# opensensor/thingino-accel

Hardware: AMD Instinct MI355X
Metric: images/sec yolov5s_int8 640x640 batch256 (higher is better)
Workload: dtype int8

## Files before the change

thingino-accel_amd/csrc/hip/conv_i8.hip:

```cpp
#include "conv_i8_common.hpp"

#ifndef I8M_ABL
#define I8M_ABL 0
#endif
template <int BPX, int BN, int STAGES, int KS = 1, int NW = 4>
__global__ __launch_bounds__(NW * 64) void conv_i8_mfma(const mhip_conv_i8_t p, const long total_pix, const int k64,
                                                         const int8_t *__restrict__ zeros, const unsigned noc,
                                                         const unsigned nblk, const int lg_inc, const unsigned kw_magic,
                                                         const fastdiv_t dhw, const fastdiv_t dow, const int bufmode,
                                                         const unsigned in_bytes) {
    ANAT_BEGIN();
    const bool POW2 = lg_inc >= 0;
    const bool masked = p.kh * p.kw <= 32;
    constexpr int SLICE = (BPX + BN) * BK;
    constexpr int STAGE = KS * SLICE;
    constexpr int NWN = BN == 128 ? 2 : 1;
    constexpr int NWM = NW / NWN;
    constexpr int WPX = BPX / NWM / 16;
    constexpr int WOC = BN / NWN / 16;
    constexpr int XROWS = BPX / NW;
    constexpr int XI = XROWS / 16;
    constexpr int LW = (BN / 16 + NW - 1) / NW;
    constexpr int L = XI + LW;
    static_assert(XI >= 1 && XROWS % 16 == 0, "every wave fetches whole 16-row pieces of the pixel tile");
// ... 1039 lines not shown
    if (v.patch) return conv_i8_launch_patch(p, k64, v.patch);
    const int bn = p->oc_pad % 128 == 0 ? 128 : (p->oc_pad % 64 == 0 ? 64 : 32);
    const bool b16 = v.persist && v.stages == 2 && bn16_ok(p);
    if (v.bpx == 256) {
        if (bn == 128) return launch_variant_t<256, 128>(p, total_pix, k64, v);
        if (bn == 64) return launch_variant_t<256, 64>(p, total_pix, k64, v);
        if (b16) return launch_variant_t<256, 16>(p, total_pix, k64, v);
        return launch_variant_t<256, 32>(p, total_pix, k64, v);
    }
    if (bn == 128) return launch_variant_t<128, 128>(p, total_pix, k64, v);
    if (bn == 64) return launch_variant_t<128, 64>(p, total_pix, k64, v);
    if (b16) return launch_variant_t<128, 16>(p, total_pix, k64, v);
    return launch_variant_t<128, 32>(p, total_pix, k64, v);
}

template <int BPX, int BN>
static int launch_pair_t(const mhip_conv_i8_t *a, const mhip_conv_i8_t *b, long total_pix, int k64, int lg, unsigned magic,
                         int wres) {
    if (a->nseg > 1) return -2;
    return launch_persist_t<BPX, BN, 2, true, false, true>(a, total_pix, k64, lg, magic, b, wres);
}
extern "C" int mhip_conv_i8_pair(const mhip_conv_i8_t *a, const mhip_conv_i8_t *b) {
    if (!a || !b || !tune().persist || tune().variant) return -2;
    if (a->in != b->in || a->in_stride != b->in_stride || a->frames != b->frames || a->in_h != b->in_h || a->in_w != b->in_w ||
        a->in_c != b->in_c || a->out_h != b->out_h || a->out_w != b->out_w || a->kh != b->kh || a->kw != b->kw ||
        a->stride_h != b->stride_h || a->stride_w != b->stride_w || a->pad_top != b->pad_top || a->pad_left != b->pad_left ||
        a->row_pad != b->row_pad || a->nseg != b->nseg || a->seg_up != b->seg_up || !a->lut || !b->lut || a->add || b->add ||
        a->out_nchw || b->out_nchw)
        return -2;
    for (int i = 0; i < a->nseg; i++)
        if (a->seg_in[i] != b->seg_in[i] || a->seg_c[i] != b->seg_c[i] || a->seg_stride[i] != b->seg_stride[i]) return -2;
    if ((a->in_c % 16) != 0 || mhip_conv_i8_small_c(a->in_c, a->kw, a->out_c) || mhip_conv_i8_small_c(b->in_c, b->kw, b->out_c))
        return -2;
    if (a->nseg > 1 && (!seg_valid(a) || !seg_valid(b))) return -2;
    if (!persist_eligible(a) || !persist_eligible(b)) return -2;
    const int bn = a->oc_pad % 128 == 0 ? 128 : (a->oc_pad % 64 == 0 ? 64 : 32);
    const int bnb = b->oc_pad % 128 == 0 ? 128 : (b->oc_pad % 64 == 0 ? 64 : 32);
    if (bn != bnb || !mhip_zero_page()) return -2;
    const long total_pix = (long)a->frames * a->out_h * a->out_w;
    const int k64 = (a->kh * a->row_pad + BK - 1) / BK * BK, nks = k64 / BK;
    if (total_pix <= 0 || total_pix > 0x7fffffffL) return -2;
    int lg = 0;
    while ((1 << lg) < a->in_c) lg++;
    const unsigned magic = ((65536u + (unsigned)a->kw - 1u) / (unsigned)a->kw);
    const variant_t dv = default_variant(a, nks);
    const int bpx = dv.bpx ? dv.bpx : 128, wres = dv.persist && dv.wres && (tune().wres & 2);
    const bool b16 = bn16_ok(a) && bn16_ok(b);
    if (bpx == 256) {
        if (bn == 128) return launch_pair_t<256, 128>(a, b, total_pix, k64, lg, magic, wres);
        if (bn == 64) return launch_pair_t<256, 64>(a, b, total_pix, k64, lg, magic, wres);
        if (b16) return launch_pair_t<256, 16>(a, b, total_pix, k64, lg, magic, wres);
        return launch_pair_t<256, 32>(a, b, total_pix, k64, lg, magic, wres);
    }
    if (bn == 128) return launch_pair_t<128, 128>(a, b, total_pix, k64, lg, magic, wres);
    if (bn == 64) return launch_pair_t<128, 64>(a, b, total_pix, k64, lg, magic, wres);
    if (b16) return launch_pair_t<128, 16>(a, b, total_pix, k64, lg, magic, wres);
    return launch_pair_t<128, 32>(a, b, total_pix, k64, lg, magic, wres);
}

extern "C" int mhip_conv_i8_seg_ok(const mhip_conv_i8_t *p) {
    return p && (p->in_c % 16) == 0 && !mhip_conv_i8_small_c(p->in_c, p->kw, p->out_c) && seg_valid(p) && persist_eligible(p);
}

extern "C" int mhip_conv_i8_variants(const mhip_conv_i8_t *p, int *codes, int max) {
    if (!p || (p->in_c % 16) != 0 || mhip_conv_i8_small_c(p->in_c, p->kw, p->out_c)) return 0;
    const int k64 = (p->kh * p->row_pad + BK - 1) / BK * BK, nks = k64 / BK;
    int n = 0;
    if (p->pre_w) {
        const int first = conv_i8_pre_tile_rows(p);
        for (int th : {first, 16, 8, 4})
            if (th && n < max && conv_i8_patch_ok(p, th, nullptr)) {
                const int code = th == 16 ? 10 : (th == 8 ? 9 : 11);
                bool seen = false;
                for (int i = 0; i < n; i++) seen |= codes[i] == code;
                if (!seen) codes[n++] = code;
            }
        return n;
    }
    if (p->post_w) {
        for (int th : {16, 8, 4})
            if (n < max && conv_i8_patch_ok(p, th, nullptr)) codes[n++] = th == 16 ? 10 : (th == 8 ? 9 : 11);
        return n;
    }
    if (p->nseg > 1) {
        const int bn = p->oc_pad % 128 == 0 ? 128 : (p->oc_pad % 64 == 0 ? 64 : 32);
        const variant_t dv = default_variant(p, nks);
        const int dflt = dv.persist && dv.wres ? (dv.bpx == 256 ? 15 : 14) : (dv.bpx == 256 ? 4 : 2);
        if (n < max) codes[n++] = dflt;
        if (n < max && dflt != 2) codes[n++] = 2;
        if (n < max && dflt != 4) codes[n++] = 4;
        if (n < max && dflt != 14 && LUTB + 2 * (size_t)128 * BK + (size_t)nks * bn * BK <= 80 * 1024) codes[n++] = 14;
        if (n < max && dflt != 15 && LUTB + 2 * (size_t)256 * BK + (size_t)nks * bn * BK <= 80 * 1024) codes[n++] = 15;
        return n;
    }
    const int dflt = variant_code(default_variant(p, nks));
    if (n < max) codes[n++] = dflt;
    for (int code = 1; code <= NVARIANTS; code++) {
        const variant_t v = variant_of(code);
        if (code == dflt) continue;
        if (v.patch && !conv_i8_patch_ok(p, v.patch, nullptr)) continue;
        if (v.persist && !persist_eligible(p)) continue;
        if (v.ks2 && ((nks & 1) || nks < 4 || p->oc_pad % 64 != 0)) continue;
        if (v.w8 && (p->oc_pad % 128 != 0 || nks < 3)) continue;
        if (v.persist < 0) continue;
        if (v.r128 && !r128_ok(p)) continue;
        if (v.rows && !conv_i8_rows_ok(p)) continue;
        if (v.wres) {
            const int bn = p->oc_pad % 128 == 0 ? 128 : (p->oc_pad % 64 == 0 ? 64 : 32);
            if (LUTB + 2 * (size_t)v.bpx * BK + (size_t)nks * bn * BK > 80 * 1024) continue;
        }
        if (!v.persist && v.stages == 3 && nks <= 2) continue;
        if (n < max) codes[n++] = code;
    }
    return n;
}

template <int BN>
static int launch_generic(const mhip_conv_i8_t *p, long total_pix, int k64) {
    dim3 grid((unsigned)((total_pix + BP - 1) / BP), (unsigned)(p->oc_pad / BN));
    hipLaunchKernelGGL((conv_i8_generic<BN>), grid, dim3(NTHREADS), 0, mhip_stream_native(), *p, total_pix, k64,
                       make_fastdiv((unsigned)(p->out_h * p->out_w)));
    return mhip_check(hipGetLastError(), "conv_i8_generic launch");
}

extern "C" int mhip_conv_i8(const mhip_conv_i8_t *p) {
    if (!p || !p->in || (!p->out && !(p->post_w && p->post_out)) || !p->w) return -1;
    if (p->out_pix_stride < 0 || p->out_ch_off < 0 || (p->out_nchw && (p->out_pix_stride || p->out_ch_off)) ||
        (p->out_pix_stride && p->out_pix_stride < p->out_ch_off + p->out_c))
        return -1;
    if (p->frames <= 0 || p->in_h <= 0 || p->in_w <= 0 || p->in_c <= 0 || p->out_h <= 0 || p->out_w <= 0 ||
        p->out_c <= 0 || p->kh <= 0 || p->kw <= 0 || p->stride_h < 0 || p->stride_w < 0)
        return -1;
    int row_pad, oc_pad;
    mhip_conv_i8_pack_geom(p->in_c, p->kw, p->out_c, &row_pad, &oc_pad, nullptr);
    if (row_pad != p->row_pad || oc_pad != p->oc_pad) return -1;
    if (p->add && (!p->safe || p->out_nchw || ((p->out_c | p->out_pix_stride | p->out_ch_off) & 15) || (p->in_c % 16) != 0 ||
                   mhip_conv_i8_small_c(p->in_c, p->kw, p->out_c) || p->nseg > 1))
        return -1;
    const long total_pix = (long)p->frames * p->out_h * p->out_w;
    const int k64 = (p->kh * p->row_pad + BK - 1) / BK * BK;
    if (total_pix <= 0 || total_pix > 0x7fffffffL || (total_pix + BP - 1) / BP * (oc_pad / 32) > 0x7fffffffL) return -1;
    if (p->in_planar) {
        if (p->in_planar > 4 || p->in_c != 4 || p->in_w < 4 || p->stride_h < 1 || p->stride_w < 1 || p->add || p->nseg > 1 ||
            !mhip_conv_i8_small_c(p->in_c, p->kw, p->out_c))
            return -2;
        return conv_i8_try_smallc(p, k64);
    }
    if (mhip_conv_i8_small_c(p->in_c, p->kw, p->out_c)) {
        if (p->stride_h >= 1 && p->stride_w >= 1) {
            int rc = conv_i8_try_rgb(p, k64);
            if (rc == -2) rc = conv_i8_try_smallc(p, k64);
            if (rc != -2) return rc;
        }
        if (p->add || p->nseg > 1) return -1;
        if (oc_pad % 64 == 0) return launch_generic<64>(p, total_pix, k64);
        return launch_generic<32>(p, total_pix, k64);
    }
    if (p->pre_w) {
        if (!mhip_zero_page() || !mhip_conv_i8_pre_ok(p)) return -1;
        int th = conv_i8_pre_tile_rows(p);
        const int code = p->variant ? p->variant : tune().variant;
        if (code >= 9 && code <= 11) {
            const int want = code == 10 ? 16 : (code == 9 ? 8 : 4);
            if (conv_i8_patch_ok(p, want, nullptr)) th = want;
        } else if (tune().small_batch && conv_i8_patch_ok(p, 4, nullptr) &&
                   ((long)p->frames * p->out_h * p->out_w + 255) / 256 * ((p->oc_pad + 127) / 128) < 256) {
            th = 4;
        }
        return conv_i8_launch_patch(p, k64, th);
    }
    if (p->post_w) {
        if (!mhip_zero_page() || (p->in_c % 16) != 0 || !mhip_conv_i8_post_ok(p)) return -1;
        int th = conv_i8_post_tile_rows(p);
        const int code = p->variant ? p->variant : tune().variant;
        if (code >= 9 && code <= 11) {
            const int want = code == 10 ? 16 : (code == 9 ? 8 : 4);
            if (conv_i8_patch_ok(p, want, nullptr)) th = want;
        } else if (tune().small_batch && conv_i8_patch_ok(p, 4, nullptr) &&
                   ((long)p->frames * p->out_h * p->out_w + 255) / 256 * ((p->oc_pad + 127) / 128) < tune().few_wgs) {
            th = 4;
        }
        return conv_i8_launch_patch(p, k64, th);
    }
    if ((p->in_c % 16) == 0) {
        if (!mhip_zero_page()) return -1;
        const int nks = k64 / BK;
        if (p->variant < 0 || p->variant > NVARIANTS) return -1;
        int code = p->variant;
        if (p->nseg > 1) {
            if (!seg_valid(p) || !persist_eligible(p)) return -1;
            if (!code && tune().variant) {
                int codes[NVARIANTS];
                const int n = mhip_conv_i8_variants(p, codes, NVARIANTS);
                for (int i = 0; i < n; i++)
                    if (codes[i] == tune().variant) code = codes[i];
            }
            variant_t v = variant_of(code == 4 || code == 14 || code == 15 ? code : 2);
            if (!code) {
                const variant_t dv = default_variant(p, nks);
                v.bpx = dv.bpx ? dv.bpx : 128;
                v.wres = dv.persist && dv.wres;
            }
            return launch_variant(p, total_pix, k64, v);
        }
        if (!code && tune().variant) {
            int codes[NVARIANTS];
            const int n = mhip_conv_i8_variants(p, codes, NVARIANTS);
            for (int i = 0; i < n; i++)
                if (codes[i] == tune().variant) code = codes[i];
        }
        return launch_variant(p, total_pix, k64, code ? variant_of(code) : default_variant(p, nks));
    }
    if (oc_pad % 64 == 0) return launch_generic<64>(p, total_pix, k64);
    return launch_generic<32>(p, total_pix, k64);
}
```

thingino-accel_amd/csrc/hip/conv_i8_common.hpp:

```cpp
#pragma once
#include <hip/hip_runtime.h>
#include <stdint.h>
#include <stdlib.h>
#include <string.h>
#include <type_traits>

#include "../mhip.h"

extern "C" hipStream_t mhip_stream_native(void);
extern "C" int mhip_check(hipError_t e, const char *what);
extern "C" const void *mhip_zero_page(void);

typedef int v4i __attribute__((ext_vector_type(4)));
typedef int v2i __attribute__((ext_vector_type(2)));

#ifdef ANATOMY
struct anat_rec_t {
    unsigned key, wg, hwid, xcc;
    unsigned long long t[4];
};
static __device__ anat_rec_t *g_anat_buf;
static __device__ unsigned g_anat_cap;
#define ANAT_SETTER(NAME)                                                                                                    \
    extern "C" int NAME(void *buf, unsigned cap) {                                                                          \
// ... 55 lines not shown
    r = r > 127 ? 127 : r;
    return r;
}

__device__ __forceinline__ int requant_safe(int acc, float cs, int lo, int hi) {
    const float scaled = (float)acc * cs;
    const float half = __int_as_float((__float_as_int(scaled) & (int)0x80000000) | 0x3f000000);
    const int r = (int)(scaled + half);
    int m;
    asm("v_med3_i32 %0, %1, %2, %3" : "=v"(m) : "v"(r), "v"(lo), "v"(hi));
    return m;
}
template <int NV>
__device__ __forceinline__ void wait_lds_values(int (&v)[NV]) {
    static_assert(NV == 4 || NV == 8 || NV == 16, "values per lane");
    if constexpr (NV == 16)
        asm volatile("s_waitcnt lgkmcnt(0)"
                     : "+v"(v[0]), "+v"(v[1]), "+v"(v[2]), "+v"(v[3]), "+v"(v[4]), "+v"(v[5]), "+v"(v[6]), "+v"(v[7]), "+v"(v[8]), "+v"(v[9]),
                       "+v"(v[10]), "+v"(v[11]), "+v"(v[12]), "+v"(v[13]), "+v"(v[14]), "+v"(v[15]));
    else if constexpr (NV == 8)
        asm volatile("s_waitcnt lgkmcnt(0)" : "+v"(v[0]), "+v"(v[1]), "+v"(v[2]), "+v"(v[3]), "+v"(v[4]), "+v"(v[5]), "+v"(v[6]), "+v"(v[7]));
    else
        asm volatile("s_waitcnt lgkmcnt(0)" : "+v"(v[0]), "+v"(v[1]), "+v"(v[2]), "+v"(v[3]));
}

__device__ __forceinline__ uint32_t pack4(int q0, int q1, int q2, int q3) {
    const uint32_t a = __builtin_amdgcn_perm((uint32_t)q1, (uint32_t)q0, 0x0c0c0400u);
    const uint32_t b = __builtin_amdgcn_perm((uint32_t)q3, (uint32_t)q2, 0x0c0c0400u);
    return (b << 16) | a;
}
__device__ __forceinline__ void lut4_at0(int q0, int q1, int q2, int q3, int &v0, int &v1, int &v2, int &v3) {
    asm volatile("ds_read_i8 %0, %4 offset:128\n\tds_read_i8 %1, %5 offset:128\n\t"
                 "ds_read_i8 %2, %6 offset:128\n\tds_read_i8 %3, %7 offset:128"
                 : "=&v"(v0), "=&v"(v1), "=&v"(v2), "=&v"(v3)
                 : "v"(q0), "v"(q1), "v"(q2), "v"(q3)
                 : "memory");
}
__device__ __forceinline__ void lds_base_must_be_zero(const void *dynamic_lds) {
    __builtin_amdgcn_s_setprio(3);
    unsigned a = (unsigned)(size_t)(const __attribute__((address_space(3))) void *)dynamic_lds;
    asm volatile("" : "+s"(a));
    if (a != 0u) __builtin_trap();
}
struct add_args_t {
    float s_conv, s_other, inv;
};
__device__ __forceinline__ int add_one(int v, uint32_t xword, int k, const add_args_t &g, int lo8, int hi8) {
    const int x = __builtin_amdgcn_sbfe((int)xword, 8 * k, 8);
    const float y = (float)v * g.s_conv + (float)x * g.s_other;
    const float t = y * g.inv;
    const int r = (int)(t + 0.5f);
    int m;
    asm("v_med3_i32 %0, %1, %2, %3" : "=v"(m) : "v"(r), "v"(lo8), "v"(hi8));
    return m;
}
__device__ __forceinline__ void lut4_fast(int q0, int q1, int q2, int q3, int &v0, int &v1, int &v2, int &v3) {
    asm volatile("ds_read_i8 %0, %4 offset:256\n\tds_read_i8 %1, %5 offset:256\n\t"
                 "ds_read_i8 %2, %6 offset:256\n\tds_read_i8 %3, %7 offset:256"
                 : "=&v"(v0), "=&v"(v1), "=&v"(v2), "=&v"(v3)
                 : "v"(q0), "v"(q1), "v"(q2), "v"(q3)
                 : "memory");
}
template <int NV>
__device__ __forceinline__ void requant_pack_pre(const int (&a)[NV], float cs, uint32_t (&pk)[NV / 4]) {
    const float cs2 = cs * 2.0f;
    const int klo = -256, khi = 255;
    int q[NV], v[NV];
#pragma unroll
    for (int i = 0; i < NV; i++) {
        const int k = (int)((float)a[i] * cs2);
        asm("v_med3_i32 %0, %1, %2, %3" : "=v"(q[i]) : "v"(k), "v"(klo), "v"(khi));
    }
#pragma unroll
    for (int g = 0; g < NV / 4; g++)
        asm volatile("ds_read_i8 %0, %4 offset:768\n\tds_read_i8 %1, %5 offset:768\n\t"
                     "ds_read_i8 %2, %6 offset:768\n\tds_read_i8 %3, %7 offset:768"
                     : "=&v"(v[4 * g]), "=&v"(v[4 * g + 1]), "=&v"(v[4 * g + 2]), "=&v"(v[4 * g + 3])
                     : "v"(q[4 * g]), "v"(q[4 * g + 1]), "v"(q[4 * g + 2]), "v"(q[4 * g + 3])
                     : "memory");
    wait_lds_values<NV>(v);
#pragma unroll
    for (int g = 0; g < NV / 4; g++) pk[g] = pack4(v[4 * g], v[4 * g + 1], v[4 * g + 2], v[4 * g + 3]);
}
template <int NV, bool HAS_LUT, bool SAFE, bool LUT0, bool ADD = false, bool FAST = false>
__device__ __forceinline__ void requant_pack(const int (&a)[NV], float cs, int lo, const uint8_t *lut128, uint32_t (&pk)[NV / 4],
                                             const uint32_t *xw = nullptr, const add_args_t *ga = nullptr) {
    int q[NV];
    const int hi = 127;
    if (FAST && HAS_LUT && LUT0 && SAFE) {
        const float cs2 = cs * 2.0f;
        const int klo = -256, khi = 255;
        int v[NV];
#pragma unroll
        for (int i = 0; i < NV; i++) {
            const int k = (int)((float)a[i] * cs2);
            asm("v_med3_i32 %0, %1, %2, %3" : "=v"(q[i]) : "v"(k), "v"(klo), "v"(khi));
        }
#pragma unroll
        for (int g = 0; g < NV / 4; g++)
            lut4_fast(q[4 * g], q[4 * g + 1], q[4 * g + 2], q[4 * g + 3], v[4 * g], v[4 * g + 1], v[4 * g + 2], v[4 * g + 3]);
        wait_lds_values<NV>(v);
        if (ADD) {
            const int lo8 = -128;
#pragma unroll
            for (int i = 0; i < NV; i++) v[i] = add_one(v[i], xw[i >> 2], i & 3, *ga, lo8, hi);
        }
#pragma unroll
        for (int g = 0; g < NV / 4; g++) pk[g] = pack4(v[4 * g], v[4 * g + 1], v[4 * g + 2], v[4 * g + 3]);
        return;
    }
#pragma unroll
    for (int i = 0; i < NV; i++) q[i] = SAFE ? requant_safe(a[i], cs, lo, hi) : requant<false>(a[i], cs, lo);
    if (HAS_LUT && LUT0) {
        int v[NV];
#pragma unroll
        for (int g = 0; g < NV / 4; g++)
            lut4_at0(q[4 * g], q[4 * g + 1], q[4 * g + 2], q[4 * g + 3], v[4 * g], v[4 * g + 1], v[4 * g + 2], v[4 * g + 3]);
        wait_lds_values<NV>(v);
        if (ADD) {
            const int lo8 = -128;
#pragma unroll
            for (int i = 0; i < NV; i++) v[i] = add_one(v[i], xw[i >> 2], i & 3, *ga, lo8, hi);
        }
#pragma unroll
        for (int g = 0; g < NV / 4; g++) pk[g] = pack4(v[4 * g], v[4 * g + 1], v[4 * g + 2], v[4 * g + 3]);
    } else {
        if (HAS_LUT) {
#pragma unroll
            for (int i = 0; i < NV; i++) q[i] = (int8_t)lut128[q[i]];
        }
        if (ADD) {
            const int lo8 = -128;
#pragma unroll
            for (int i = 0; i < NV; i++) q[i] = add_one(q[i], xw[i >> 2], i & 3, *ga, lo8, hi);
        }
#pragma unroll
        for (int g = 0; g < NV / 4; g++) pk[g] = pack4(q[4 * g], q[4 * g + 1], q[4 * g + 2], q[4 * g + 3]);
    }
}

struct fastdiv_t {
    unsigned m, s1, s2;
};
__device__ __forceinline__ unsigned fdiv(unsigned n, const fastdiv_t d) {
    const unsigned q = __umulhi(d.m, n);
    return (q + ((n - q) >> d.s1)) >> d.s2;
}
static fastdiv_t make_fastdiv(unsigned d) {
    fastdiv_t r;
    unsigned l = 0;
    while ((1ull << l) < d) l++;
    r.m = (unsigned)(((1ull << 32) * ((1ull << l) - d)) / d + 1);
    r.s1 = l < 1 ? l : 1;
    r.s2 = l > 0 ? l - 1 : 0;
    return r;
}

template <int N>
__device__ __forceinline__ void wait_vmcnt() {
    asm volatile("s_waitcnt vmcnt(%0)" ::"n"(N) : "memory");
}

__device__ __forceinline__ void glds16(const void *gsrc, void *lds_wave_base) {
    __builtin_amdgcn_global_load_lds((const __attribute__((address_space(1))) void *)gsrc,
                                     (__attribute__((address_space(3))) void *)lds_wave_base, 16, 0, 0);
}
// ... 98 lines not shown
            } else {
                const int rem = ncols - c * 16;
                int o = 0;
                if (rem & 8) { __builtin_memcpy(d, s, 8); o = 8; }
                if (rem & 4) { __builtin_memcpy(d + o, s + o, 4); o += 4; }
                if (rem & 2) { __builtin_memcpy(d + o, s + o, 2); o += 2; }
                if (rem & 1) d[o] = s[o];
            }
        }
    } else {
        for (int id = tid; id < BPX * BN; id += (int)blockDim.x) {
            const int c = id / BPX, row = id - c * BPX;
            const long off = rowoff[row];
            if (off < 0 || c >= ncols) continue;
            p.out[off + (size_t)(oc0 + c) * hw] = tile[row * ROW + c];
        }
    }
}

template <int BPX, int BN, int WPX, int WOC, bool LUT0 = false>
__device__ __forceinline__ void epilogue(const mhip_conv_i8_t &p, v4i (&acc)[WOC][WPX], int8_t *tile, const uint8_t *slut,
                                         const long *rowoff, int oc0, int pxw, int ocw, int hw) {
    const bool direct = !p.out_nchw && ((p.out_c | p.out_pix_stride | p.out_ch_off) & 15) == 0;
#define EPI(L, S, D) epilogue_t<BPX, BN, WPX, WOC, L, S, D, LUT0>(p, acc, tile, slut, rowoff, oc0, pxw, ocw, hw)
    if (direct) {
        if (p.lut) { if (p.safe) EPI(true, true, true); else EPI(true, false, true); }
        else { if (p.safe) EPI(false, true, true); else EPI(false, false, true); }
    } else {
        if (p.lut) { if (p.safe) EPI(true, true, false); else EPI(true, false, false); }
        else { if (p.safe) EPI(false, true, false); else EPI(false, false, false); }
    }
#undef EPI
}

template <int WPX, int WOC>
__device__ __forceinline__ void init_acc(const mhip_conv_i8_t &p, v4i (&acc)[WOC][WPX], int ocbase) {
    const int lane = threadIdx.x & 63;
#pragma unroll
    for (int s = 0; s < WOC; s++) {
        const v4i b = p.bias ? *(const v4i *)(p.bias + ocbase + s * 16 + (lane >> 4) * 4) : (v4i){0, 0, 0, 0};
#pragma unroll
        for (int t = 0; t < WPX; t++) acc[s][t] = b;
    }
}


struct tune_t {
    int init;
    int persist;
    int persist_stages;
    int persist_maxk;
    int persist_slots;
    int stages;
    int bpx;
    int variant;
    int bufmode;
    int small_batch;
    int rgb_direct;
    int wres;
    int few_wgs;
    int rows;
    int patch_ring;
    int patch_lds_kb;
};
const tune_t &conv_i8_tune_state();

extern "C" int mhip_conv_i8_small_c(int in_c, int kw, int out_c);

static inline long in_extent_bytes(const mhip_conv_i8_t *p) {
    return (long)(p->frames - 1) * (long)p->in_stride + (long)p->in_h * p->in_w * p->in_c;
}
static inline long persist_out_bytes(const mhip_conv_i8_t *p) {
    const long pstride = p->out_pix_stride ? p->out_pix_stride : p->out_c;
    return (long)(p->frames - 1) * (long)p->out_stride + (long)p->out_h * p->out_w * pstride;
}
static inline bool conv_i8_direct_rows(const mhip_conv_i8_t *p) {
    return !p->out_nchw && ((p->out_c | p->out_pix_stride | p->out_ch_off) & 15) == 0;
}

bool conv_i8_patch_ok(const mhip_conv_i8_t *p, int th, int *ring);
int conv_i8_launch_patch(const mhip_conv_i8_t *p, int k64, int th);
int conv_i8_pre_tile_rows(const mhip_conv_i8_t *p);
int conv_i8_post_tile_rows(const mhip_conv_i8_t *p);
bool conv_i8_rows_ok(const mhip_conv_i8_t *p);
int conv_i8_launch_rows(const mhip_conv_i8_t *p);
int conv_i8_try_rgb(const mhip_conv_i8_t *p, int k64);
int conv_i8_try_smallc(const mhip_conv_i8_t *p, int k64);
```

thingino-accel_amd/csrc/hip/conv_i8_patch.hip:

```cpp
#include "conv_i8_common.hpp"
#include <stdio.h>

#ifdef PATCH_STAMPS
__device__ unsigned long long patch_stamp_sums[8];
extern "C" int mhip_patch_stamps(unsigned long long *out, int reset) {
    if (out && hipMemcpyFromSymbol(out, HIP_SYMBOL(patch_stamp_sums), sizeof(patch_stamp_sums)) != hipSuccess) return -1;
    if (reset) {
        unsigned long long z[8] = {0};
        if (hipMemcpyToSymbol(HIP_SYMBOL(patch_stamp_sums), z, sizeof(z)) != hipSuccess) return -1;
    }
    return 0;
}
#define STAMP(t)                                                                          \
    do {                                                                                  \
        __builtin_amdgcn_sched_barrier(0);                                                \
        asm volatile("s_memtime %0\n\ts_waitcnt lgkmcnt(0)" : "=s"(t)::"memory");        \
        __builtin_amdgcn_sched_barrier(0);                                                \
    } while (0)
#else
#define STAMP(t) do { } while (0)
#endif
#define PT_TW 16
#define PT_NIMAX 10

template <int LO, int HI>
__device__ __forceinline__ void wait_vmcnt_tree(int n) {
    if constexpr (LO == HI) {
        wait_vmcnt<LO>();
    } else {
        constexpr int MID = (LO + HI + 1) / 2;
        if (n >= MID) wait_vmcnt_tree<MID, HI>(n);
        else wait_vmcnt_tree<LO, MID - 1>(n);
    }
}
template <int HI>
__device__ __forceinline__ void wait_vmcnt_upto(int n) {
    wait_vmcnt_tree<0, HI>(n > HI ? HI : n);
}
__device__ __forceinline__ void barrier_lds() {
    asm volatile("s_waitcnt lgkmcnt(0)\n\ts_barrier" ::: "memory");
}

template <int TH, int BN, bool HAS_LUT, bool PRE = false, bool POST = false>
__global__ __launch_bounds__(NTHREADS) void conv_i8_patch(const mhip_conv_i8_t p, const int k64, const int tiles_x,
                                                          const int tiles_y, const unsigned ntiles_all, const int PH,
                                                          const int PW, const int PWP, const int PWH, const int nblk,
                                                          const int8_t *__restrict__ zeros, const fastdiv_t dtx,
                                                          const fastdiv_t dty, const fastdiv_t dpwp, const unsigned out_bytes,
                                                          const int ring, const int xmap, const unsigned in_bytes) {
    ANAT_BEGIN();
    constexpr int WPX = TH / 4;
    constexpr int WOC = BN / 16;
    constexpr int NST = WPX;
    extern __shared__ __attribute__((aligned(16))) int8_t dynlds[];
    uint8_t *slut = (uint8_t *)dynlds;
    lds_base_must_be_zero(dynlds);
    const int nks = k64 / BK;
    constexpr int NPO = 2 * BN;
    constexpr int LB = LUTB + ((PRE || POST) ? 512 : 0);
    int *dutab = (int *)(dynlds + LB);
    int8_t *wl = dynlds + LB + ((nks * 16 + 255) & ~255);
    const int patch_bytes = nblk * 1024;
    int8_t *w1l = wl + nks * BN * BK;
    int8_t *pwl = w1l;
    const int *pbl = (const int *)(pwl + NPO * NPO);
    int8_t *patch0 = w1l + (PRE ? p.in_c * BK : 0) + (POST ? NPO * NPO + NPO * 4 : 0);
    int8_t *tpatch = patch0 + ring * patch_bytes;

    const int tid = threadIdx.x, lane = tid & 63;
    const int wv = __builtin_amdgcn_readfirstlane(tid >> 6);
    const int oc0 = blockIdx.y * BN;
    const int C = p.in_c, lgc = 31 - __builtin_clz((unsigned)C), cpp = C >> 4, lgcpp = lgc - 4;
    const int s = p.stride_w;
    const unsigned M = C >= 128 ? 6u : (C >= 64 ? 2u : 0u);

    v4i bias[WOC];
#pragma unroll
    for (int q = 0; q < WOC; q++) bias[q] = p.bias ? *(const v4i *)(p.bias + oc0 + q * 16 + (lane >> 4) * 4) : (v4i){0, 0, 0, 0};
    constexpr int W1MAX = 4;
    v4i pbias[PRE ? W1MAX : 1];
    if (PRE) {
#pragma unroll
        for (int q = 0; q < W1MAX; q++) pbias[q] = q < (C >> 4) ? *(const v4i *)(p.pre_bias + q * 16 + (lane >> 4) * 4) : (v4i){0, 0, 0, 0};
    }
    if (HAS_LUT) {
        if (p.lut2) { if (tid < 128) ((uint32_t *)slut)[tid] = ((const uint32_t *)p.lut2)[tid]; }
        else if (tid < 64) ((uint32_t *)slut)[tid] = ((const uint32_t *)p.lut)[tid];
    }
    if (PRE && tid >= 128) ((uint32_t *)slut)[tid] = ((const uint32_t *)p.pre_lut2)[tid - 128];
    if (POST) {
        if (tid >= 128) ((uint32_t *)slut)[tid] = ((const uint32_t *)p.post_lut2)[tid - 128];
        if (tid < NPO) ((int *)(pwl + NPO * NPO))[tid] = ((const int *)(p.post_w + NPO * NPO))[tid];
    }
    const int rowbytes = p.kw * C, kbytes = p.kh * rowbytes;
    for (int i = tid; i < nks * 4; i += NTHREADS) {
        const int kb = i * 16;
        int du = 0;
        if (kb < kbytes) {
            const int ky = kb / rowbytes, rem = kb - ky * rowbytes, kx = rem >> lgc, cc = (rem & (C - 1)) >> 4;
            const int dp = ky * PWP + (s == 2 ? (kx >> 1) + (kx & 1) * PWH : kx);
            du = dp * cpp + cc;
        }
        dutab[i] = du;
    }
    __syncthreads();
    {
        const int schunk = (lane & 3) ^ (((lane >> 4) & 1) << 1);
        for (int i = wv; i < nks * (BN / 16); i += 4) {
            const int ks = i / (BN / 16), g = i - ks * (BN / 16);
            glds16(p.w + (size_t)(oc0 + g * 16 + (lane >> 2)) * k64 + ks * BK + schunk * 16, wl + (ks * BN + g * 16) * BK);
        }
        if (PRE)
            for (int g = wv; g < C / 16; g += 4) glds16(p.pre_w + (size_t)(g * 16 + (lane >> 2)) * BK + schunk * 16, w1l + g * 16 * BK);
        if (POST)
            for (int i = wv; i < NPO * NPO / 1024; i += 4) glds16(p.post_w + i * 1024 + lane * 16, pwl + i * 1024);
    }
    int uoff[PT_NIMAX], upos[PT_NIMAX];
#pragma unroll
    for (int n = 0; n < PT_NIMAX; n++) {
        uoff[n] = 0;
        upos[n] = -1;
        if (n * 4 + wv < nblk) {
            const unsigned phys = (unsigned)((n * 4 + wv) * 64 + lane);
            const unsigned U = phys ^ ((phys >> 3) & M);
            const unsigned pp = U >> lgcpp, cc = U & (unsigned)(cpp - 1);
            const unsigned py = fdiv(pp, dpwp), col = pp - py * (unsigned)PWP;
            const int px = s == 2 ? ((int)col < PWH ? 2 * (int)col : 2 * ((int)col - PWH) + 1) : (int)col;
            if ((int)py < PH && px < PW) {
                uoff[n] = ((int)py * p.in_w + px) * C + (int)cc * 16;
                upos[n] = ((int)py << 16) | px;
            }
        }
    }
    const int npw = nblk > wv ? (nblk - wv + 3) >> 2 : 0;
    const unsigned xcd = blockIdx.x & 7u;
    const unsigned xstart = xmap ? (unsigned)(((unsigned long long)ntiles_all * xcd) >> 3) : 0u;
    const unsigned xend = xmap ? (unsigned)(((unsigned long long)ntiles_all * (xcd + 1u)) >> 3) : 0u;
    const unsigned ntiles = xmap ? (xend - xstart) * 8u + xcd : ntiles_all;
    auto tile_xy = [&](unsigned t, int &tx, int &ty, unsigned &f) {
        const unsigned j = xmap ? xstart + (t >> 3) : t, q = fdiv(j, dtx);
        tx = (int)(j - q * (unsigned)tiles_x);
        f = fdiv(q, dty);
        ty = (int)(q - f * (unsigned)tiles_y);
    };
    const __amdgpu_buffer_rsrc_t xrs = __builtin_amdgcn_make_buffer_rsrc((void *)p.in, 0, (int)in_bytes, 0x00020000);
    auto issue_patch = [&](unsigned t, int8_t *dst) {
#ifdef PATCH_ABL
        return;
#endif
        int tx, ty;
        unsigned f;
        tile_xy(t, tx, ty, f);
        const int iy0 = ty * TH * s - p.pad_top, ix0 = tx * PT_TW * s - p.pad_left;
        if (in_bytes != 0u && iy0 >= 0 && ix0 >= 0 && iy0 + PH <= p.in_h && ix0 + PW <= p.in_w) {
            const int sbase = (int)(f * (unsigned)p.in_stride) + (iy0 * p.in_w + ix0) * C;
#pragma unroll
            for (int n = 0; n < PT_NIMAX; n++)
                if (n * 4 + wv < nblk) blds16(xrs, uoff[n], sbase, dst + (n * 4 + wv) * 1024);
            return;
        }
        const int8_t *base = p.in + (size_t)f * p.in_stride + ((long)iy0 * p.in_w + ix0) * C;
#pragma unroll
        for (int n = 0; n < PT_NIMAX; n++)
            if (n * 4 + wv < nblk) {
                const int py = upos[n] >> 16, px = upos[n] & 0xffff;
                const bool ok = upos[n] >= 0 && (unsigned)(iy0 + py) < (unsigned)p.in_h && (unsigned)(ix0 + px) < (unsigned)p.in_w;
                glds16(ok ? base + uoff[n] : zeros, dst + (n * 4 + wv) * 1024);
            }
    };

    const __amdgpu_buffer_rsrc_t orsrc = __builtin_amdgcn_make_buffer_rsrc(POST ? p.post_out : p.out, 0, (int)out_bytes, 0x00020000);
    const bool has_add = p.add != nullptr;
    constexpr int RROW = WOC == 4 ? 1024 : 512;
    constexpr int NRI = WOC == 4 ? WPX : 2 * WPX;
    int8_t *rstage = patch0 + (ring + (PRE ? 1 : 0)) * patch_bytes + wv * (WPX * RROW);
    const int frow = lane & 15, fchunk = lane >> 4;
    const int chan = (lane >> 4) * (4 * WOC);
    const int NR = has_add || POST ? NRI : 0;
    const int ntail = POST ? (has_add ? NRI : 0) + WPX * (NPO / 64) : NST;
    const int ppstride = p.post_out_pix_stride ? p.post_out_pix_stride : NPO;
    auto issue_rows = [&](const int8_t *base, size_t fstride, int tx, int ty, unsigned f) {
#pragma unroll
        for (int u = 0; u < WPX; u++) {
            const int oy = ty * TH + wv * WPX + u, ox = tx * PT_TW + frow;
            const int8_t *src = oy < p.out_h && ox < p.out_w ? base + (size_t)f * fstride + ((size_t)(oy * p.out_w + ox) * BN + (size_t)chan) : zeros;
            if (WOC == 4) {
                glds16(src, rstage + u * RROW);
            } else {
                __builtin_amdgcn_global_load_lds((const __attribute__((address_space(1))) void *)src,
                                                 (__attribute__((address_space(3))) void *)(rstage + u * RROW), 4, 0, 0);
                __builtin_amdgcn_global_load_lds((const __attribute__((address_space(1))) void *)(src + 4),
                                                 (__attribute__((address_space(3))) void *)(rstage + u * RROW + 256), 4, 0, 0);
            }
        }
    };
    const int pstride = p.out_pix_stride ? p.out_pix_stride : p.out_c;
    const int lo = p.relu ? 0 : -128;
    const uint8_t *lut128 = slut + 128;
    int ubase[WPX];
#pragma unroll
    for (int u = 0; u < WPX; u++) ubase[u] = ((wv * WPX + u) * s * PWP + frow) * cpp;

    const unsigned G = gridDim.x;
    const int D = ring - 1;
    unsigned t = blockIdx.x;
    int yg0 = 0, yg1 = 0, yg2 = 0;
    {
        int issued = 0;
        for (int d = 0; d < D; d++)
            if (t + (unsigned)d * G < ntiles) {
                issue_patch(t + (unsigned)d * G, patch0 + d * patch_bytes);
                issued++;
            }
        yg0 = issued > 1 ? (issued - 1) * npw : 0;
        yg1 = issued > 2 ? (issued - 2) * npw : 0;
        yg2 = 0;
    }
#ifdef PATCH_STAMPS
    unsigned long long st0 = 0, st1 = 0, st2 = 0, st3 = 0, st4 = 0, sum_wait = 0, sum_issue = 0, sum_k = 0, sum_epi = 0, sum_tiles = 0;
#endif
    int cur = 0;
    int pn_last = 0;
    bool first = true;
    ANAT_NOW(1);
    for (; t < ntiles; t += G) {
        STAMP(st0);
        int tx, ty;
        unsigned f;
        tile_xy(t, tx, ty, f);
        int voffs[WPX];
        uint32_t xw[WPX][WOC];
#pragma unroll
        for (int u = 0; u < WPX; u++) {
            const int oy = ty * TH + wv * WPX + u, ox = tx * PT_TW + frow;
            const unsigned off = f * (unsigned)p.out_stride + (unsigned)(oy * p.out_w + ox) * (unsigned)pstride +
                                 (unsigned)(p.out_ch_off + oc0 + chan);
            const bool ok = oy < p.out_h && ox < p.out_w && oc0 + chan < p.out_c;
            voffs[u] = ok ? (int)off : -1;
#pragma unroll
            for (int q = 0; q < WOC; q++) xw[u][q] = 0;
        }
        if (POST) {
#pragma unroll
            for (int u = 0; u < WPX; u++) {
                const int oy = ty * TH + wv * WPX + u, ox = tx * PT_TW + frow;
                const unsigned off = f * (unsigned)p.post_out_stride + (unsigned)(oy * p.out_w + ox) * (unsigned)ppstride +
                                     (unsigned)(p.post_out_ch_off + (lane >> 4) * (NPO / 4));
                voffs[u] = oy < p.out_h && ox < p.out_w ? (int)off : -1;
            }
            if (has_add) issue_rows(p.add, p.out_stride, tx, ty, f);
            else issue_rows(p.post_in, p.post_in_stride, tx, ty, f);
        } else if (has_add) {
#pragma unroll
            for (int u = 0; u < WPX; u++) {
                const int8_t *src = voffs[u] >= 0 ? p.add + (unsigned)voffs[u] : zeros;
                if (WOC == 4) {
                    glds16(src, rstage + u * RROW);
                } else {
                    __builtin_amdgcn_global_load_lds((const __attribute__((address_space(1))) void *)src,
                                                     (__attribute__((address_space(3))) void *)(rstage + u * RROW), 4, 0, 0);
                    __builtin_amdgcn_global_load_lds((const __attribute__((address_space(1))) void *)(src + 4),
                                                     (__attribute__((address_space(3))) void *)(rstage + u * RROW + 256), 4, 0, 0);
                }
            }
        }
        if (D > 0) {
            wait_vmcnt_upto<63>(yg0 + NR);
            barrier_lds();
            STAMP(st1);
            const unsigned tn = t + (unsigned)D * G;
            int pn = 0;
            if (tn < ntiles) {
                int slot = cur + D;
                slot = slot >= ring ? slot - ring : slot;
                issue_patch(tn, patch0 + slot * patch_bytes);
                pn = npw;
            }
            const int after = NR + pn + ntail;
            yg0 = yg1 + after;
            yg1 = yg2 + after;
            yg2 = ntail;
            if (D == 1) yg0 = ntail;
            if (D == 2) yg1 = ntail;
            pn_last = pn;
        } else {
            if (!first) barrier_lds();
            issue_patch(t, patch0);
            wait_vmcnt<0>();
            barrier_lds();
        }
        first = false;
        STAMP(st2);
        const int8_t *patch = patch0 + cur * patch_bytes;
        if (PRE) {
            const int WOC1 = C >> 4;
            const int P = PH * PWP, nsub = (P + 15) >> 4;
            const int iy0 = ty * TH * s - p.pad_top, ix0 = tx * PT_TW * s - p.pad_left;
            for (int sub = wv; sub < nsub; sub += 4) {
                int pp = sub * 16 + frow;
                const bool live = pp < P;
                pp = live ? pp : P - 1;
                const unsigned Ur = (unsigned)(pp * cpp + (fchunk & (cpp - 1)));
                const v4i xb1 = *(const v4i *)(patch + ((Ur ^ ((Ur >> 3) & M)) << 4));
                const unsigned py = fdiv((unsigned)pp, dpwp), px = (unsigned)pp - py * (unsigned)PWP;
                const bool inimg = live && (int)py < PH && (int)px < PW && (unsigned)(iy0 + (int)py) < (unsigned)p.in_h &&
                                   (unsigned)(ix0 + (int)px) < (unsigned)p.in_w;
                uint32_t pk1[W1MAX];
                if (WOC1 == 4) {
                    int a1[16];
#pragma unroll
                    for (int q = 0; q < 4; q++) {
                        const v4i wa = *(const v4i *)(w1l + lds_off(q * 16 + frow, fchunk));
                        const v4i r = __builtin_amdgcn_mfma_i32_16x16x64_i8(wa, xb1, pbias[PRE ? q : 0], 0, 0, 0);
#pragma unroll
                        for (int e = 0; e < 4; e++) a1[q * 4 + e] = r[e];
                    }
                    uint32_t pk4[4];
                    requant_pack_pre<16>(a1, p.pre_cs, pk4);
#pragma unroll
                    for (int e = 0; e < 4; e++) pk1[e] = inimg ? pk4[e] : 0u;
                    const unsigned Uw = (unsigned)(pp * cpp + (lane >> 4));
                    if (live) *(v4i *)(tpatch + ((Uw ^ ((Uw >> 3) & M)) << 4)) = (v4i){(int)pk1[0], (int)pk1[1], (int)pk1[2], (int)pk1[3]};
                } else {
                    int a1[8];
#pragma unroll
                    for (int q = 0; q < 2; q++) {
                        const v4i wa = *(const v4i *)(w1l + lds_off(q * 16 + frow, fchunk));
                        const v4i r = __builtin_amdgcn_mfma_i32_16x16x64_i8(wa, xb1, pbias[PRE ? q : 0], 0, 0, 0);
#pragma unroll
                        for (int e = 0; e < 4; e++) a1[q * 4 + e] = r[e];
                    }
                    uint32_t pk2[2];
                    requant_pack_pre<8>(a1, p.pre_cs, pk2);
                    const int g4 = lane >> 4;
                    const unsigned Uw = (unsigned)(pp * cpp + (g4 >> 1));
                    if (live)
                        *(uint2 *)(tpatch + ((Uw ^ ((Uw >> 3) & M)) << 4) + (g4 & 1) * 8) = make_uint2(inimg ? pk2[0] : 0u, inimg ? pk2[1] : 0u);
                }
            }
            barrier_lds();
            patch = tpatch;
        }
        v4i acc[WOC][WPX];
        v4i xa[WPX], wa[WOC], xb[WPX], wb[WOC];
        auto load_frags = [&](int ks, int du, v4i (&xf)[WPX], v4i (&wf)[WOC]) {
#pragma unroll
            for (int u = 0; u < WPX; u++) {
                const unsigned U = (unsigned)(ubase[u] + du);
                xf[u] = *(const v4i *)(patch + ((U ^ ((U >> 3) & M)) << 4));
            }
            const int8_t *ws = wl + ks * BN * BK;
#pragma unroll
            for (int q = 0; q < WOC; q++) wf[q] = *(const v4i *)(ws + lds_off(q * 16 + frow, fchunk));
        };
        auto mfma_step = [&](const v4i (&xf)[WPX], const v4i (&wf)[WOC]) {
#pragma unroll
            for (int q = 0; q < WOC; q++)
#pragma unroll
                for (int u = 0; u < WPX; u++) acc[q][u] = __builtin_amdgcn_mfma_i32_16x16x64_i8(wf[q], xf[u], acc[q][u], 0, 0, 0);
        };
        const int last = nks - 1;
        auto clampk = [&](int k) { return k < last ? k : last; };
        load_frags(0, dutab[fchunk], xa, wa);
        load_frags(clampk(1), dutab[clampk(1) * 4 + fchunk], xb, wb);
        int du_n = dutab[clampk(2) * 4 + fchunk];
#pragma unroll
        for (int q = 0; q < WOC; q++)
#pragma unroll
            for (int u = 0; u < WPX; u++) acc[q][u] = __builtin_amdgcn_mfma_i32_16x16x64_i8(wa[q], xa[u], bias[q], 0, 0, 0);
        int ks = 1;
        for (; ks + 1 < nks; ks += 2) {
            load_frags(ks + 1, du_n, xa, wa);
            du_n = dutab[clampk(ks + 2) * 4 + fchunk];
            __builtin_amdgcn_sched_barrier(0);
            mfma_step(xb, wb);
            __builtin_amdgcn_sched_barrier(0);
            load_frags(clampk(ks + 2), du_n, xb, wb);
            du_n = dutab[clampk(ks + 3) * 4 + fchunk];
            __builtin_amdgcn_sched_barrier(0);
            mfma_step(xa, wa);
            __builtin_amdgcn_sched_barrier(0);
        }
        if (ks < nks) mfma_step(xb, wb);
        STAMP(st3);
        if (D > 0) cur = cur + 1 == ring ? 0 : cur + 1;
        if (has_add) {
            if (D > 0) wait_vmcnt_upto<15>(pn_last);
#pragma unroll
            for (int u = 0; u < WPX; u++) {
                if (WOC == 4) {
                    const v4i r = *(const v4i *)(rstage + u * RROW + lane * 16);
                    xw[u][0] = (uint32_t)r[0]; xw[u][1] = (uint32_t)r[1]; xw[u][WOC > 2 ? 2 : 0] = (uint32_t)r[2]; xw[u][WOC > 3 ? 3 : 0] = (uint32_t)r[3];
                } else {
                    xw[u][0] = *(const uint32_t *)(rstage + u * RROW + lane * 4);
                    xw[u][WOC > 1 ? 1 : 0] = *(const uint32_t *)(rstage + u * RROW + 256 + lane * 4);
                }
            }
        }
        uint32_t pku[POST ? WPX : 1][WOC];
        if (POST && has_add) {
#pragma unroll
            for (int u = 0; u < WPX; u++) {
                if constexpr (WOC == 4) asm volatile("s_waitcnt lgkmcnt(0)" : "+v"(xw[u][0]), "+v"(xw[u][1]), "+v"(xw[u][2]), "+v"(xw[u][3])::"memory");
                else asm volatile("s_waitcnt lgkmcnt(0)" : "+v"(xw[u][0]), "+v"(xw[u][1])::"memory");
            }
            issue_rows(p.post_in, p.post_in_stride, tx, ty, f);
        }
#pragma unroll
        for (int u = 0; u < WPX; u++) {
            uint32_t pk[WOC];
            int a[WOC * 4];
#pragma unroll
            for (int q = 0; q < WOC; q++)
#pragma unroll
                for (int r = 0; r < 4; r++) a[q * 4 + r] = acc[q][u][r];
            const bool fast = HAS_LUT && p.lut2 != nullptr;
            if (has_add) {
                const add_args_t ga = {p.add_s_conv, p.add_s_other, p.add_inv};
                if (fast) requant_pack<WOC * 4, HAS_LUT, true, true, true, true>(a, p.cs, lo, lut128, pk, xw[u], &ga);
                else requant_pack<WOC * 4, HAS_LUT, true, true, true>(a, p.cs, lo, lut128, pk, xw[u], &ga);
            } else {
                if (fast) requant_pack<WOC * 4, HAS_LUT, true, true, false, true>(a, p.cs, lo, lut128, pk);
                else requant_pack<WOC * 4, HAS_LUT, true, true>(a, p.cs, lo, lut128, pk);
            }
            if (POST) {
#pragma unroll
                for (int q = 0; q < WOC; q++) pku[POST ? u : 0][q] = pk[q];
                continue;
            }
            const int voff = voffs[u];
            if (WOC == 4)
                __builtin_amdgcn_raw_buffer_store_b128((v4i){(int)pk[0], (int)pk[1], (int)pk[2], (int)pk[3]}, orsrc, voff, 0, 0);
            else if (WOC == 2)
                __builtin_amdgcn_raw_buffer_store_b64((v2i){(int)pk[0], (int)pk[WOC > 1 ? 1 : 0]}, orsrc, voff, 0, 0);
        }
        if (POST) {
            if (has_add) wait_vmcnt<0>();
            else if (D > 0) wait_vmcnt_upto<15>(pn_last);
#pragma unroll
            for (int u = 0; u < WPX; u++) {
                v4i b0, b1 = {0, 0, 0, 0};
                if (WOC == 4) {
                    b0 = (v4i){(int)pku[POST ? u : 0][0], (int)pku[POST ? u : 0][1], (int)pku[POST ? u : 0][WOC > 2 ? 2 : 0], (int)pku[POST ? u : 0][WOC > 3 ? 3 : 0]};
                    b1 = *(const v4i *)(rstage + u * RROW + lane * 16);
                } else {
                    b0 = (v4i){(int)pku[POST ? u : 0][0], (int)pku[POST ? u : 0][WOC > 1 ? 1 : 0], *(const int *)(rstage + u * RROW + lane * 4),
                               *(const int *)(rstage + u * RROW + 256 + lane * 4)};
                }
#pragma unroll
                for (int h = 0; h < NPO / 64; h++) {
                    int a[16];
#pragma unroll
                    for (int s4 = 0; s4 < 4; s4++) {
                        const int row = (h * 4 + s4) * 16;
                        v4i c = *(const v4i *)(pbl + row + fchunk * 4);
                        c = __builtin_amdgcn_mfma_i32_16x16x64_i8(*(const v4i *)(pwl + lds_off(row + frow, fchunk)), b0, c, 0, 0, 0);
                        if (WOC == 4) c = __builtin_amdgcn_mfma_i32_16x16x64_i8(*(const v4i *)(pwl + NPO * BK + lds_off(row + frow, fchunk)), b1, c, 0, 0, 0);
#pragma unroll
                        for (int e = 0; e < 4; e++) a[s4 * 4 + e] = c[e];
                    }
                    uint32_t pk4[4];
                    requant_pack_pre<16>(a, p.post_cs, pk4);
                    const int voff = voffs[u] >= 0 ? voffs[u] + h * 16 : -1;
                    __builtin_amdgcn_raw_buffer_store_b128((v4i){(int)pk4[0], (int)pk4[1], (int)pk4[2], (int)pk4[3]}, orsrc, voff, 0, 0);
                }
            }
        }
#ifdef PATCH_STAMPS
        STAMP(st4);
        if (D == 0) st1 = st2;
        sum_wait += st1 - st0; sum_issue += st2 - st1; sum_k += st3 - st2; sum_epi += st4 - st3; sum_tiles += 1;
#endif
    }
    ANAT_NOW(2);
    ANAT_END(p);
#ifdef PATCH_STAMPS
    if (lane == 0) {
        atomicAdd(&patch_stamp_sums[0], sum_wait); atomicAdd(&patch_stamp_sums[1], sum_issue); atomicAdd(&patch_stamp_sums[2], sum_k);
        atomicAdd(&patch_stamp_sums[3], sum_epi); atomicAdd(&patch_stamp_sums[4], sum_tiles);
    }
#endif
}

ANAT_SETTER(mhip_anatomy_set_patch)
struct patch_geom_t {
    int bn, tiles_x, tiles_y, PH, PW, PWP, PWH, nblk, nks, ring;
    size_t lds;
};
static inline const tune_t &tune() { return conv_i8_tune_state(); }
static size_t patch_lds_budget(int bn) {
    const int kb = tune().patch_lds_kb;
    if (kb >= 16 && kb <= 160 && kb != 80) return (size_t)kb * 1024;
    return (size_t)(bn == 32 ? 53 : 80) * 1024;
}
static bool patch_geom(const mhip_conv_i8_t *p, int th, patch_geom_t *g) {
    const bool direct = conv_i8_direct_rows(p);
    const int C = p->in_c, s = p->stride_w;
    static const bool no_c16 = getenv("MARS_HIP_PATCH_NO_C16") != nullptr;
    if (!direct || !p->safe || (C != 16 && C != 32 && C != 64 && C != 128) || (C == 16 && (no_c16 || p->pre_w)) || (s != 1 && s != 2) || p->stride_h != s ||
        p->kh > 7 || p->kw > 7 || p->kh * p->kw < 2 || p->row_pad != p->kw * C || persist_out_bytes(p) > 0x7fffffffL)
        return false;
    const int k64 = (p->kh * p->row_pad + BK - 1) / BK * BK;
    g->nks = k64 / BK;
    g->bn = p->oc_pad % 64 == 0 ? 64 : 32;
    g->tiles_x = (p->out_w + PT_TW - 1) / PT_TW;
    g->tiles_y = (p->out_h + th - 1) / th;
    if ((double)p->out_h * p->out_w < (C == 128 ? 0.80 : 0.85) * (double)g->tiles_x * PT_TW * g->tiles_y * th) return false;
    g->PH = (th - 1) * s + p->kh;
    g->PW = (PT_TW - 1) * s + p->kw;
    g->PWH = s == 2 ? (g->PW + 1) / 2 : 0;
    g->PWP = s == 2 ? 2 * g->PWH : g->PW;
    const long units = (long)g->PH * g->PWP * (C / 16);
    g->nblk = (int)((units + 63) / 64);
    if (g->nblk > 4 * PT_NIMAX) return false;
    const bool pre = p->pre_w != nullptr;
    if (pre && (s != 1 || (C != 32 && C != 64) || !p->pre_bias || !p->pre_lut2 || !p->lut2)) return false;
    const bool post = p->post_w != nullptr;
    if (post) {
        const long ppstride = p->post_out_pix_stride ? p->post_out_pix_stride : 2 * g->bn;
        if (pre || s != 1 || p->out_c != g->bn || p->oc_pad != g->bn || p->out_pix_stride || p->out_ch_off || !p->lut2 || !p->post_lut2 || !p->post_in ||
            !p->post_out || ((p->post_out_pix_stride | p->post_out_ch_off) & 15) || p->post_out_pix_stride < 0 || p->post_out_ch_off < 0 ||
            ppstride < p->post_out_ch_off + 2 * g->bn ||
            (long)(p->frames - 1) * (long)p->post_out_stride + (long)p->out_h * p->out_w * ppstride > 0x7fffffffL)
            return false;
    }
    const size_t pb = (size_t)g->nblk * 1024;
    const size_t radd = p->add || post ? (size_t)4 * (th / 4) * (g->bn == 64 ? 1024 : 512) : 0;
    const size_t fixed = LUTB + (pre ? 512 + (size_t)C * BK + pb : 0) + (post ? 512 + (size_t)4 * g->bn * g->bn + (size_t)8 * g->bn : 0) +
                         (((size_t)g->nks * 16 + 255) & ~(size_t)255) + (size_t)g->nks * g->bn * BK + radd;
    const size_t budget = patch_lds_budget(g->bn);
    if (fixed + pb > budget) return false;
    const int fit = (int)((budget - fixed) / pb);
    const int cap = tune().patch_ring > 0 ? (tune().patch_ring > 4 ? 4 : tune().patch_ring) : 2;
    int ring = fit < cap ? fit : cap;
    g->ring = ring;
    g->lds = fixed + (size_t)ring * pb;
    if ((long)g->tiles_x * g->tiles_y * p->frames > 0x7fffffffL) return false;
    return true;
}

static inline long post_out_bytes(const mhip_conv_i8_t *p) {
    const long ppstride = p->post_out_pix_stride ? p->post_out_pix_stride : 2 * p->out_c;
    return (long)(p->frames - 1) * (long)p->post_out_stride + (long)p->out_h * p->out_w * ppstride;
}
template <int TH, int BN, bool HAS_LUT, bool PRE = false, bool POST = false>
static int launch_patch_t(const mhip_conv_i8_t *p, int k64, const patch_geom_t &g) {
    auto kern = conv_i8_patch<TH, BN, HAS_LUT, PRE, POST>;
    static int cus = 0;
    static size_t slots_lds[8];
    static int slots_n[8], nslots = 0;
    if (!cus) {
        int dev = 0;
        hipDeviceProp_t prop;
        if (hipFuncSetAttribute((const void *)kern, hipFuncAttributeMaxDynamicSharedMemorySize, 160 * 1024) != hipSuccess ||
            hipGetDevice(&dev) != hipSuccess || hipGetDeviceProperties(&prop, dev) != hipSuccess)
            return mhip_check(hipErrorUnknown, "conv_i8_patch occupancy query");
        cus = prop.multiProcessorCount;
    }
    int slots = 0;
    for (int i = 0; i < nslots; i++)
        if (slots_lds[i] == g.lds) slots = slots_n[i];
    if (!slots) {
        int occ = 0;
        if (hipOccupancyMaxActiveBlocksPerMultiprocessor(&occ, kern, NTHREADS, g.lds) != hipSuccess)
            return mhip_check(hipErrorUnknown, "conv_i8_patch occupancy query");
        slots = (occ > 0 ? occ : 1) * cus;
        if (nslots < 8) { slots_lds[nslots] = g.lds; slots_n[nslots++] = slots; }
    }
    const unsigned ntiles = (unsigned)((long)g.tiles_x * g.tiles_y * p->frames);
    const unsigned noc = (unsigned)(p->oc_pad / BN);
    unsigned gx = (unsigned)(tune().persist_slots > 0 ? tune().persist_slots : slots) / noc;
    if (gx < 1) gx = 1;
    if (gx > ntiles) gx = ntiles;
    const int xmap = gx >= 8 && ntiles < 0x0fffffffu;
    if (xmap) gx &= ~7u;
    {
        static const char *dbg = getenv("MARS_HIP_PATCH_DEBUG");
        static size_t last_lds = 0;
        static int last_ring = 0;
        if (dbg && (last_lds != g.lds || last_ring != g.ring)) {
            fprintf(stderr, "Mars: conv_i8_patch<%d,%d> ring %d, patch %d KB, LDS %zu B, %d workgroups per CU, grid %u x %u\n", TH, BN, g.ring,
                    g.nblk, g.lds, slots / cus, gx, noc);
            last_lds = g.lds;
            last_ring = g.ring;
        }
    }
    hipLaunchKernelGGL(kern, dim3(gx, noc), dim3(NTHREADS), g.lds, mhip_stream_native(), *p, k64,
                       g.tiles_x, g.tiles_y, ntiles, g.PH, g.PW, g.PWP, g.PWH, g.nblk, (const int8_t *)mhip_zero_page(),
                       make_fastdiv((unsigned)g.tiles_x), make_fastdiv((unsigned)g.tiles_y), make_fastdiv((unsigned)g.PWP),
                       (unsigned)(POST ? post_out_bytes(p) : persist_out_bytes(p)), g.ring, xmap,
                       in_extent_bytes(p) <= 0x7fffffffL ? (unsigned)in_extent_bytes(p) : 0u);
    return mhip_check(hipGetLastError(), "conv_i8_patch launch");
}

bool conv_i8_patch_ok(const mhip_conv_i8_t *p, int th, int *ring) {
    patch_geom_t g;
    if (!patch_geom(p, th, &g)) return false;
    if (ring) *ring = g.ring;
    return true;
}

int conv_i8_launch_patch(const mhip_conv_i8_t *p, int k64, int th) {
    patch_geom_t g;
    if (!patch_geom(p, th, &g)) return -1;
#define PATCH(T, B)                                                                       \
    (p->post_w ? launch_patch_t<T, B, true, false, true>(p, k64, g)                       \
     : p->pre_w ? launch_patch_t<T, B, true, true>(p, k64, g)                             \
                : (p->lut ? launch_patch_t<T, B, true>(p, k64, g) : launch_patch_t<T, B, false>(p, k64, g)))
    if (th == 16) return g.bn == 64 ? PATCH(16, 64) : PATCH(16, 32);
    if (th == 8) return g.bn == 64 ? PATCH(8, 64) : PATCH(8, 32);
    return g.bn == 64 ? PATCH(4, 64) : PATCH(4, 32);
#undef PATCH
}

int conv_i8_pre_tile_rows(const mhip_conv_i8_t *p) {
    patch_geom_t g;
    for (int th : {16, 8, 4})
        if (patch_geom(p, th, &g) && (th == 4 || g.ring >= 2)) return th;
    return 0;
}
extern "C" int mhip_conv_i8_pre_ok(const mhip_conv_i8_t *p) {
    if (!p || !p->pre_w || p->nseg > 1 || p->out_nchw) return 0;
    return conv_i8_pre_tile_rows(p) != 0;
}

int conv_i8_post_tile_rows(const mhip_conv_i8_t *p) {
    patch_geom_t g;
    for (int th : {16, 8, 4})
        if (patch_geom(p, th, &g)) return th;
    return 0;
}
extern "C" int mhip_conv_i8_post_ok(const mhip_conv_i8_t *p) {
    if (!p || !p->post_w || p->pre_w || p->nseg > 1 || p->out_nchw) return 0;
    return conv_i8_post_tile_rows(p) != 0;
}
extern "C" int mhip_conv_i8_post_k(int c, int k) {
    if (c == 64) return k;
    return k < 32 ? (k >> 3) * 16 + (k & 7) : ((k - 32) >> 3) * 16 + 8 + (k & 7);
}
extern "C" int mhip_conv_i8_post_row(int c, int oc) {
    const int per = c / 2, g = oc / per, rem = oc - g * per;
    return (rem >> 2) * 16 + g * 4 + (rem & 3);
}
extern "C" size_t mhip_conv_i8_post_pack(int c, const int8_t *packed, const int32_t *bias, int8_t *out) {
    if (c != 32 && c != 64) return 0;
    const int n = 2 * c;
    const size_t bytes = (size_t)n * n + (size_t)n * 4;
    if (!packed || !out) return bytes;
    memset(out, 0, bytes);
    for (int oc = 0; oc < n; oc++) {
        const int R = mhip_conv_i8_post_row(c, oc), src = mhip_conv_i8_oc_row(oc, n);
        for (int k = 0; k < n; k++) {
            const int pos = mhip_conv_i8_post_k(c, k), ks = pos >> 6, chunk = (pos & 63) >> 4;
            out[(size_t)(ks * n + R) * BK + (((chunk ^ ((R >> 1) & 2))) << 4) + (pos & 15)] = packed[(size_t)src * n + k];
        }
        ((int32_t *)(out + (size_t)n * n))[R] = bias ? bias[src] : 0;
    }
    return bytes;
}
```

thingino-accel_amd/csrc/host/mars_internal.h:

```cpp
#ifndef MARS_INTERNAL_H
#define MARS_INTERNAL_H

#include <stddef.h>
#include <stdint.h>

#include "../mhip.h"
#include "mars_hip.h"
#include "mars_runtime.h"

enum {
    OP_CONV_I8 = 0,
    OP_CONV_F32,
    OP_RELU_BYTES,
    OP_LUT_I8,
    OP_BINARY_I8,
    OP_SIGMOID_F32,
    OP_BINARY_F32,
    OP_RELU_F32,
    OP_BN,
    OP_MAXPOOL,
    OP_CONCAT_SLICE,
    OP_UPSAMPLE,
    OP_UPSAMPLE_Q, OP_MAXPOOL_Q,
    OP_CONCAT_Q,
    OP_CONV_F32_VHEAD,
    OP_FAIL,
};

#define NO_OFF ((size_t)-1)
#define MARS_MAX_IO 4
#define MARS_MAX_MODEL_TUNE 16

typedef struct {
    size_t bytes;
    size_t extent;
    size_t stride;
    uint8_t *dev;
    int is_weight;
    int needed;
    int io_in, io_out;
    uint8_t *host;
    uint8_t *dense_dev;
    int pix_c, pix_stride;
    int rec_c, rec_hw;
    int nhwc_c, nhwc_hw;
    size_t zero_from;
    int partial;
    int nhwc_pitch;
    int tail_read;
} mtensor_t;

typedef struct {
    int kind, layer, err;
    int t_in[4], n_in, t_out;
    int in_h, in_w, in_c, out_h, out_w, out_c, kh, kw, sh, sw, pt, pl;
    int nchw, relu, is_mul, is_f32, leaky, safe;
    size_t in_byte_off, out_byte_off;
    int k_limit;
    int vc_n, vc_t[3], vc_run, vc_shift;
    int rows_only;
    int out_nchw;
    int silu_f32;
    int f32_exact;
    int variant;
    int add_t; float add_s_conv, add_s_other, add_inv;
    int nseg, seg_t[4], seg_c[4], seg_up;
    int chain_n, chain_out[3];
    int pair_next;
    int row_pad, oc_pad, c_pad;
    int ch_off, scale_h, scale_w, bn_n;
    int out_pix_stride, out_ch_off;
    int store_c;
    float cs, f0, f1, f2;
    size_t n;
    size_t w_off, b_off, lut_off, s_off;
    int pre;
    size_t pre_w_off, pre_b_off, pre_lut2_off;
    float pre_cs;
    int post_next;
    size_t post_w_off;
    size_t w2_off;
    int w2_rows;
    int w2_planes;
    size_t w3_off;
    int w3_stem;
    int in_rec, out_rec;
    size_t lut2_off;
    size_t w_blob_off[2];
    double macs, bytes;
    int prof_kind;
    float last_ms;
    void *ev0, *ev1;
    int prof_rec;
    void *ev_start;
} mars_op_t;

typedef struct {
    int fusion;
    unsigned no_fuse_lut : 1, no_nhwc_internal : 1, no_vconcat_q : 1, no_pair_f32 : 1, no_rec : 1, no_zero_tail : 1, no_vconcat_f32 : 1,
        no_rowpad : 1, no_post : 1;
    size_t rec_limit;
    size_t vconcat_limit;
    size_t bottleneck_limit;
} plan_switches_t;

typedef struct mars_model_ext {
    mars_model_t pub;
    plan_switches_t sw;
    int batch, profiling, deferred;
    int plan_err;
    int no_vconcat;
    int no_download;
    int no_bottleneck;
    int no_post;
    int rec_frames;
    int rec_skipped;
    size_t rec_max_frames;
    mtensor_t *mt;
    mars_op_t *ops;
    int n_ops, cap_ops;
    uint8_t *arena_host;
    size_t arena_size, arena_cap;
    uint8_t *arena_dev;
    size_t blob_mirror_bytes;
    uint8_t *act_dev;
    size_t act_bytes;
    uint8_t *scratch_dev;
    size_t scratch_per_frame;
    int scratch_t, scratch_cpad, scratch_f0, scratch_n;
    void *det_dev;
    int *det_counts_dev;
    float *det_lut_dev;
    int det_cap;
    float det_lut_scale[4];
    int det_lut_n;
    int det_lut_mono[4];
    float *heads_lut_dev;
    float heads_lut_scale[4];
    int heads_lut_n;
    float *dfl_lut_dev;
    float dfl_lut_scale[4][2];
    int dfl_lut_n;
    void *ev_graph_done, *ev_tail_done;
    int tail_pending;
    int frame0, run_frames;
    void *ev_fork, *ev_join[3];
    void *ev_chunk[2][8];
    void *graph_exec;
    unsigned graph_gen;
    int ran_plain;
    void *pipe;
    struct { char key[28]; int value, saved; } tune[MARS_MAX_MODEL_TUNE];
    int n_tune, tune_depth;
    int plan_f32_mode;
    unsigned char *layer_noop;
    void *roi_dev;
    int roi_cap_slots, roi_cap_frames;
    int roi_slots;
    struct mars_model_ext *roi_from;
    void *cls_dev;
    size_t cls_bytes, cls_sums_off, cls_top_off;
    int cls_frames, cls_c, cls_top_k;
    void *ev_label_done;
    int label_pending;
    void *label_dev;
    int label_cap, label_frames;
    void *match_dev;
    size_t match_bytes, match_top_off, match_row_off;
    int match_frames, match_top_k;
    void *ident_dev;
    int ident_cap, ident_frames;
    void *track_dev;
    int track_cap, track_frames;
    void *seg_dev;
    size_t seg_bytes, seg_rec_off, seg_word_off;
    int seg_frames, seg_max, seg_ph, seg_pw;
    void *ev_seg[2];
    void *pose_dev;
    size_t pose_bytes, pose_rec_off, pose_kpt_off;
    int pose_frames, pose_max, pose_k;
    float pose_lut_scale[4];
    int pose_lut_n;
    void *ev_pose[2];
    void *obb_dev;
    size_t obb_bytes, obb_cnt_off, obb_out_off;
    int obb_frames;
    float obb_lut_scale[4];
    int obb_lut_n;
    void *ev_obb[2];
    struct mars_model_ext *live_next;
} mars_model_ext_t;


#define MARS_INTERNAL __attribute__((visibility("hidden")))
#define ALIGN_UP(x, a) (((x) + (size_t)(a) - 1) & ~((size_t)(a) - 1))
#define NO_TENSOR 0xFFFFFFFFu
#define MAX_DIM_PRODUCT ((size_t)1 << 40)
#define ARENA_MAX ((size_t)1 << 40)
#define MAX_CHANNELS 65536
MARS_INTERNAL int mars_verbose(void);
#define VLOG(...) do { if (mars_verbose()) fprintf(stderr, "Mars: " __VA_ARGS__); } while (0)
MARS_INTERNAL void drop_graph(mars_model_ext_t *m);
MARS_INTERNAL mars_model_ext_t *mars_live_models(void);
MARS_INTERNAL void plan_switches_read(plan_switches_t *sw, int at_load);
MARS_INTERNAL mars_error_t build_plan(mars_model_ext_t *m);
MARS_INTERNAL mars_error_t upload_params(mars_model_ext_t *m);
MARS_INTERNAL mars_error_t alloc_batch(mars_model_ext_t *m, int n);
MARS_INTERNAL size_t elem_size(uint32_t dtype);
MARS_INTERNAL size_t shape_numel(const mars_tensor_t *d);
MARS_INTERNAL size_t reference_buffer_size(const mars_model_ext_t *m);
MARS_INTERNAL size_t arena_reserve(mars_model_ext_t *m, size_t bytes);
MARS_INTERNAL void blob_read(const mars_model_ext_t *m, size_t off, size_t n, void *dst);
MARS_INTERNAL int op_reads(const mars_op_t *o, int t);
MARS_INTERNAL int op_writes(const mars_op_t *o, int t);
MARS_INTERNAL size_t planned_stride(const mtensor_t *t);
MARS_INTERNAL void conv_i8_geometry(const mars_op_t *op, int frames, mhip_conv_i8_t *p);
MARS_INTERNAL int conv_i8_pre_fits(const mars_op_t *op, int frames, size_t in_stride, size_t out_stride);
MARS_INTERNAL int conv_i8_post_fits(const mars_model_ext_t *m, const mars_op_t *a, const mars_op_t *b, int frames);
MARS_INTERNAL void plan_layer(mars_model_ext_t *m, int li);
MARS_INTERNAL void fold_silu(mars_model_ext_t *m, int f32);
MARS_INTERNAL void fuse_lut(mars_model_ext_t *m);
MARS_INTERNAL void nhwc_internal(mars_model_ext_t *m);
MARS_INTERNAL void fold_add(mars_model_ext_t *m, int f32);
MARS_INTERNAL void virtual_concat(mars_model_ext_t *m);
MARS_INTERNAL void elide_concat(mars_model_ext_t *m);
MARS_INTERNAL void trim_concat(mars_model_ext_t *m);
MARS_INTERNAL void fuse_pool_chains(mars_model_ext_t *m);
MARS_INTERNAL void pair_convs(mars_model_ext_t *m);
MARS_INTERNAL void fuse_bottleneck(mars_model_ext_t *m);
MARS_INTERNAL void fuse_post(mars_model_ext_t *m);
MARS_INTERNAL void pad_output_rows(mars_model_ext_t *m);
MARS_INTERNAL void virtual_concat_q(mars_model_ext_t *m);
MARS_INTERNAL void f32_policy(mars_model_ext_t *m);
MARS_INTERNAL void zero_tail_f32(mars_model_ext_t *m);
MARS_INTERNAL void pair_convs_f32(mars_model_ext_t *m);
MARS_INTERNAL void rec_pairs(mars_model_ext_t *m);
MARS_INTERNAL void virtual_concat_f32(mars_model_ext_t *m);
MARS_INTERNAL void plan_check(mars_model_ext_t *m);
MARS_INTERNAL void conv_i8_params(const mars_model_ext_t *m, const mars_op_t *op, mhip_conv_i8_t *p);
MARS_INTERNAL int mars_preproc_prepare(int w, int h, int tw, int th);
MARS_INTERNAL int mars_preproc_prepare_nv12(int w, int h, int tw, int th, int frames);

MARS_INTERNAL void mars_roi_release(mars_model_ext_t *m);

MARS_INTERNAL void mars_cls_release(mars_model_ext_t *m);

MARS_INTERNAL void mars_match_release(mars_model_ext_t *m);

MARS_INTERNAL void mars_track_release(mars_model_ext_t *m);

MARS_INTERNAL void mars_seg_release(mars_model_ext_t *m);

MARS_INTERNAL void mars_pose_release(mars_model_ext_t *m);

MARS_INTERNAL void mars_obb_release(mars_model_ext_t *m);

MARS_INTERNAL int mars_tensor_chw(const mars_tensor_t *d, int *c, int *h, int *w);
MARS_INTERNAL int mars_locate_i8(const mars_model_ext_t *m, int T, int ch, int hh, int ww, int any_writer, int *buf, int *off, int *pix_step, int *ch_step);
MARS_INTERNAL mars_error_t mars_own_det_buffers(mars_model_ext_t *m);
MARS_INTERNAL mars_error_t mars_tail_on_aux(mars_model_ext_t *m, int (*launch)(struct mars_model_ext *, const void *, void *, int *), const void *cfg);

mars_error_t mars_detect_prepare(mars_model_ext_t *m, const int *output_indices, int n_outputs);
int mars_detect_launch(mars_model_ext_t *m, const int *output_indices, int n_outputs, float nms_thresh, void *dets_dev,
                       int *counts_dev);

typedef struct {
    int n, ti[4], stride[4], nc[4], h[4], w[4], pix_step[4], ch_step[4];
    float anchors[4][3][2];
    float conf, nms;
    int map, px, py;
    float rx, ry;
    int internal;
} mars_heads_cfg_t;
MARS_INTERNAL int mars_find_heads(const mars_model_ext_t *m, int *tensor_ids, int *strides, int *num_classes, int cap);
MARS_INTERNAL mars_error_t mars_heads_resolve(mars_model_ext_t *m, const mars_yolo_heads_t *h, mars_heads_cfg_t *c);
MARS_INTERNAL mars_error_t mars_heads_prepare(mars_model_ext_t *m, const mars_heads_cfg_t *c);
MARS_INTERNAL int mars_heads_launch(mars_model_ext_t *m, const mars_heads_cfg_t *c, void *dets_dev, int *counts_dev);

typedef struct {
    int n, reg_max, stride[4], nc[4], h[4], w[4];
    int box_t[4], cls_t[4], box_buf[4], cls_buf[4], box_off[4], cls_off[4];
    int box_pix_step[4], box_ch_step[4], cls_pix_step[4], cls_ch_step[4];
    float box_scale[4], cls_scale[4];
    float conf, nms;
    int map, px, py;
    float rx, ry;
    int internal;
    int *cand_pred, *kept_pred;
    void *premap;
} mars_dfl_cfg_t;
MARS_INTERNAL int mars_find_dfl_heads(const mars_model_ext_t *m, int *box_ids, int *cls_ids, int *strides, int *num_classes, int *reg_max, int cap);
MARS_INTERNAL mars_error_t mars_dfl_resolve(mars_model_ext_t *m, const mars_yolo_dfl_heads_t *h, mars_dfl_cfg_t *c);
MARS_INTERNAL mars_error_t mars_dfl_prepare(mars_model_ext_t *m, const mars_dfl_cfg_t *c);
MARS_INTERNAL int mars_dfl_launch(mars_model_ext_t *m, const mars_dfl_cfg_t *c, void *dets_dev, int *counts_dev);

int32_t mars_trunc_x86(float x);
void mars_pack_conv_i8(const int8_t *w, size_t avail, int nchw, int out_c, int in_c, int kh, int kw,
                       int c_pad, int row_pad, int oc_pad, int8_t *dst);

#endif
```

thingino-accel_amd/csrc/host/mars_model.c:

```c
#include <math.h>
#include <stdio.h>
#include <stdlib.h>
#include <string.h>
#include <sys/types.h>
#include <time.h>

#include "mars_internal.h"
#include "nna.h"


int mars_verbose(void) {
    static int v = -1;
    if (v < 0) v = getenv("MARS_VERBOSE") ? 1 : 0;
    return v;
}

void plan_switches_read(plan_switches_t *sw, int at_load) {
    const char *e;
    if (at_load) sw->fusion = (e = getenv("MARS_HIP_FUSION")) ? atoi(e) : 1;
    sw->no_fuse_lut = getenv("MARS_HIP_NO_FUSE_LUT") != NULL;
    sw->no_nhwc_internal = getenv("MARS_HIP_NO_NHWC_INTERNAL") != NULL;
    sw->no_vconcat_q = getenv("MARS_HIP_NO_VCONCAT_Q") != NULL;
    sw->no_pair_f32 = getenv("MARS_HIP_NO_PAIR_F32") != NULL;
    sw->no_rec = getenv("MARS_HIP_NO_REC") != NULL;
    sw->no_zero_tail = getenv("MARS_HIP_NO_ZERO_TAIL") != NULL;
    sw->no_vconcat_f32 = getenv("MARS_HIP_NO_VCONCAT_F32") != NULL;
    sw->no_rowpad = getenv("MARS_HIP_NO_ROWPAD") != NULL;
    sw->no_post = getenv("MARS_HIP_NO_POST") != NULL;
    sw->rec_limit = (e = getenv("MARS_HIP_REC_LIMIT")) ? (size_t)strtoull(e, NULL, 0) : (size_t)0xfffffff0u;
    sw->vconcat_limit = (e = getenv("MARS_HIP_VCONCAT_LIMIT")) ? (size_t)strtoull(e, NULL, 0) : (size_t)0x7fffffffu;
    sw->bottleneck_limit = (e = getenv("MARS_HIP_BOTTLENECK_LIMIT")) ? (size_t)strtoull(e, NULL, 0) : 0;
}

void drop_graph(mars_model_ext_t *m) {
    if (m->graph_exec) {
        mhip_sync();
        mhip_graph_destroy(m->graph_exec);
    }
    m->graph_exec = NULL;
    m->ran_plain = 0;
}

static const char *const k_err[] = {
    "OK", "Invalid magic number", "Version mismatch", "Memory allocation failed",
    "Invalid file format", "NNA initialization failed", "Layer execution failed",
    "Invalid tensor", "Invalid layer",
};

const char *mars_get_error_string(mars_error_t err) {
    int i = -(int)err;
    if (i >= 0 && i < (int)(sizeof(k_err) / sizeof(k_err[0]))) return k_err[i];
    return "Unknown error";
}

static void free_device_state(mars_model_ext_t *m) {
    drop_graph(m);
    if (m->act_dev) mhip_free(m->act_dev);
    if (m->scratch_dev) mhip_free(m->scratch_dev);
    m->act_dev = m->scratch_dev = NULL;
    for (uint32_t i = 0; m->mt && i < m->pub.header.num_tensors; i++) {
        if (m->mt[i].host) mhip_host_free(m->mt[i].host);
        m->mt[i].host = NULL;
        if (m->mt[i].dense_dev) mhip_free(m->mt[i].dense_dev);
        m->mt[i].dense_dev = NULL;
        if (!m->mt[i].is_weight) m->mt[i].dev = NULL;
    }
    if (m->det_dev) mhip_free(m->det_dev);
    if (m->det_counts_dev) mhip_free(m->det_counts_dev);
    m->det_dev = NULL;
    m->det_counts_dev = NULL;
    m->det_cap = 0;
    m->tail_pending = 0;
    mars_roi_release(m);
    mars_cls_release(m);
    mars_track_release(m);
    mars_seg_release(m);
    mars_pose_release(m);
    mars_obb_release(m);
}

static void free_ops(mars_model_ext_t *m) {
    drop_graph(m);
    for (int i = 0; i < m->n_ops; i++) {
        if (m->ops[i].ev0) mhip_event_destroy(m->ops[i].ev0);
        if (m->ops[i].ev1) mhip_event_destroy(m->ops[i].ev1);
    }
    free(m->ops);
    m->ops = NULL;
    m->n_ops = m->cap_ops = 0;
}

static mars_model_ext_t *g_live_models = NULL;
mars_model_ext_t *mars_live_models(void) { return g_live_models; }

void mars_free(mars_model_t *model) {
    if (!model) return;
    mars_model_ext_t *m = (mars_model_ext_t *)model;
    for (mars_model_ext_t **pp = &g_live_models; *pp; pp = &(*pp)->live_next)
        if (*pp == m) { *pp = m->live_next; break; }
    for (mars_model_ext_t *x = g_live_models; x; x = x->live_next)
        if (x->roi_from == m) x->roi_from = NULL;
    if (m->pipe) mars_hip_pipe_close(model);
    if (mhip_ready()) mhip_sync();
    free_device_state(m);
    free_ops(m);
    if (m->arena_dev) mhip_free(m->arena_dev);
    if (m->det_lut_dev) mhip_free(m->det_lut_dev);
    if (m->heads_lut_dev) mhip_free(m->heads_lut_dev);
    if (m->dfl_lut_dev) mhip_free(m->dfl_lut_dev);
    if (m->ev_graph_done) mhip_event_destroy(m->ev_graph_done);
    if (m->ev_tail_done) mhip_event_destroy(m->ev_tail_done);
    if (m->ev_label_done) mhip_event_destroy(m->ev_label_done);
    if (m->ev_fork) mhip_event_destroy(m->ev_fork);
    for (int k = 0; k < 3; k++)
        if (m->ev_join[k]) mhip_event_destroy(m->ev_join[k]);
    for (int k = 0; k < 2; k++)
        for (int c = 0; c < 8; c++)
            if (m->ev_chunk[k][c]) mhip_event_destroy(m->ev_chunk[k][c]);
    free(m->arena_host);
    free(m->layer_noop);
    free(m->mt);
    free(m->pub.weights);
    free(m->pub.layers);
    free(m->pub.tensors);
    free(m);
}

mars_error_t build_plan(mars_model_ext_t *m) {
    const uint32_t nt = m->pub.header.num_tensors, nl = m->pub.header.num_layers;
    plan_switches_read(&m->sw, 0);
    free_ops(m);
    m->arena_size = 0;
    if (m->arena_host) memset(m->arena_host, 0, m->arena_cap);
    m->scratch_per_frame = 0;
    m->plan_err = MARS_OK;
    m->plan_f32_mode = mhip_conv_f32_mode(-1);
    m->blob_mirror_bytes = m->pub.weights_size;
    for (uint32_t i = 0; i < nt; i++) {
        m->mt[i].extent = m->mt[i].bytes;
        m->mt[i].pix_c = m->mt[i].pix_stride = 0;
        m->mt[i].needed = (m->mt[i].io_in || m->mt[i].io_out) ? 1 : 0;
    }
    for (uint32_t i = 0; i < nl && m->plan_err == MARS_OK; i++) {
        const int n0 = m->n_ops;
        plan_layer(m, (int)i);
        m->layer_noop[i] = m->n_ops == n0;
    }
    if (m->plan_err != MARS_OK) return (mars_error_t)m->plan_err;
    if (m->sw.fusion >= 1) {
        fold_silu(m, 0);
        fuse_lut(m);
        fold_silu(m, 1);
        nhwc_internal(m);
        fold_add(m, 0);
        fold_add(m, 1);
        if (!m->no_vconcat) virtual_concat(m);
        elide_concat(m);
        trim_concat(m);
        fuse_pool_chains(m);
        pair_convs(m);
        if (m->sw.fusion >= 2 && !m->no_bottleneck) fuse_bottleneck(m);
        fuse_post(m);
        pad_output_rows(m);
        virtual_concat_q(m);
    } else {
        nhwc_internal(m);
    }
    f32_policy(m);
    zero_tail_f32(m);
    if (m->sw.fusion >= 1) pair_convs_f32(m);
    rec_pairs(m);
    virtual_concat_f32(m);
    if (m->plan_err == MARS_OK) plan_check(m);
    return (mars_error_t)m->plan_err;
}

mars_error_t upload_params(mars_model_ext_t *m) {
    size_t mirror_off = arena_reserve(m, m->blob_mirror_bytes + 64);
    if (mirror_off == NO_OFF) return MARS_ERR_ALLOC_FAILED;
    if (!m->deferred) blob_read(m, 0, m->blob_mirror_bytes, m->arena_host + mirror_off);
    if (m->arena_dev) mhip_free(m->arena_dev);
    m->arena_dev = (uint8_t *)mhip_malloc(m->arena_size);
    if (!m->arena_dev) return MARS_ERR_ALLOC_FAILED;
    if (mhip_h2d_async(m->arena_dev, m->arena_host, m->arena_size) || mhip_sync()) return MARS_ERR_NNA_INIT_FAILED;
    for (uint32_t i = 0; i < m->pub.header.num_tensors; i++) {
        if (!m->mt[i].is_weight) continue;
        m->mt[i].dev = m->arena_dev + mirror_off + (size_t)m->pub.tensors[i].desc.data_offset;
        m->mt[i].stride = 0;
        m->pub.tensors[i].paddr = m->mt[i].dev;
    }
    m->pub.ddr_paddr = m->arena_dev;
    m->pub.ddr_size = m->arena_size;
    return MARS_OK;
}

mars_error_t alloc_batch(mars_model_ext_t *m, int n) {
    const uint32_t nt = m->pub.header.num_tensors;
    if (m->pipe) mars_hip_pipe_close(&m->pub);
    if (mhip_sync()) return MARS_ERR_LAYER_FAILED;
    plan_switches_read(&m->sw, 0);
    const size_t vlim = m->sw.vconcat_limit, blim = m->sw.bottleneck_limit;
    const int rec_replan = (size_t)n > m->rec_max_frames || (m->rec_skipped && n < m->rec_frames);
    m->rec_frames = n;
    if (m->no_vconcat || m->no_bottleneck || m->no_post || rec_replan) {
        m->no_vconcat = m->no_bottleneck = m->no_post = 0;
        mars_error_t e = build_plan(m);
        if (e == MARS_OK) e = upload_params(m);
        if (e != MARS_OK) return e;
    }
    if (!m->no_vconcat)
        for (int i = 0; i < m->n_ops; i++) {
            const mars_op_t *op = &m->ops[i];
            if (op->kind != OP_CONV_I8 || op->nseg < 2 || op->t_out < 0) continue;
            if (planned_stride(&m->mt[op->t_out]) * (size_t)n > vlim) {
                m->no_vconcat = 1;
                mars_error_t e = build_plan(m);
                if (e == MARS_OK) e = upload_params(m);
                if (e != MARS_OK) return e;
                break;
            }
        }
    if (m->sw.fusion >= 2 && !m->no_bottleneck)
        for (int i = 0; i < m->n_ops; i++) {
            const mars_op_t *op = &m->ops[i];
            if (op->kind != OP_CONV_I8 || !op->pre || op->t_out < 0) continue;
            const size_t in_stride = op->t_in[0] >= 0 ? planned_stride(&m->mt[op->t_in[0]]) : 0;
            if (!conv_i8_pre_fits(op, n, in_stride, planned_stride(&m->mt[op->t_out])) || (blim && (size_t)n > blim)) {
                m->no_bottleneck = 1;
                mars_error_t e = build_plan(m);
                if (e == MARS_OK) e = upload_params(m);
                if (e != MARS_OK) return e;
                break;
            }
        }
    if (!m->no_post)
        for (int i = 0; i + 1 < m->n_ops; i++) {
            const mars_op_t *op = &m->ops[i];
            if (op->kind != OP_CONV_I8 || !op->post_next) continue;
            if (!conv_i8_post_fits(m, op, op + 1, n)) {
                m->no_post = 1;
                mars_error_t e = build_plan(m);
                if (e == MARS_OK) e = upload_params(m);
                if (e != MARS_OK) return e;
                break;
            }
        }
    free_device_state(m);
    size_t per_frame = 0;
    for (uint32_t i = 0; i < nt; i++) {
        mtensor_t *t = &m->mt[i];
        if (t->is_weight || !t->needed) continue;
        t->stride = planned_stride(t);
        per_frame += t->stride;
    }
    m->act_bytes = per_frame * (size_t)n;
    m->act_dev = (uint8_t *)mhip_malloc(m->act_bytes + 512);
    if (!m->act_dev) return MARS_ERR_ALLOC_FAILED;
    if (mhip_memset_async(m->act_dev, 0, m->act_bytes + 256)) return MARS_ERR_ALLOC_FAILED;
    size_t off = 256;
    for (uint32_t i = 0; i < nt; i++) {
        mtensor_t *t = &m->mt[i];
        mars_runtime_tensor_t *rt = &m->pub.tensors[i];
        if (t->is_weight) continue;
        rt->vaddr = NULL; rt->paddr = NULL; rt->alloc_size = 0;
        if (!t->needed) continue;
        t->dev = m->act_dev + off;
        off += t->stride * (size_t)n;
        rt->paddr = t->dev;
        rt->alloc_size = t->stride * (size_t)n;
        if (t->io_in || t->io_out) {
            const size_t hb = t->bytes * (size_t)n, ref = reference_buffer_size(m);
            size_t cap = hb > ref ? hb : ref;
            if (ref > ((size_t)8 << 20)) cap = hb;
            t->host = (uint8_t *)mhip_host_alloc(cap ? cap : 64);
            if (!t->host) return MARS_ERR_ALLOC_FAILED;
            memset(t->host, 0, cap);
            rt->vaddr = t->host;
            rt->alloc_size = n == 1 && cap >= ref ? ref : hb;
        }
        if (t->pix_stride) {
            t->dense_dev = (uint8_t *)mhip_malloc(t->bytes * (size_t)n);
            if (!t->dense_dev) return MARS_ERR_ALLOC_FAILED;
        }
    }
    if (m->scratch_per_frame) {
        m->scratch_dev = (uint8_t *)mhip_malloc(ALIGN_UP(m->scratch_per_frame, 256) * (size_t)n + 256);
        if (!m->scratch_dev) return MARS_ERR_ALLOC_FAILED;
    }
    m->batch = n;
    m->frame0 = 0;
    m->run_frames = n;
    return mhip_sync() ? MARS_ERR_ALLOC_FAILED : MARS_OK;
}

static mars_error_t load_host(const void *data, size_t size, unsigned flags, mars_model_ext_t **out_m) {
    if (!data || !out_m || size < sizeof(mars_header_t)) return MARS_ERR_INVALID_FILE;
    const uint8_t *p = (const uint8_t *)data;
    mars_header_t h;
    memcpy(&h, p, sizeof(h));
    if (h.magic != MARS_MAGIC) {
        VLOG("Invalid magic 0x%08x (expected 0x%08x)\n", h.magic, MARS_MAGIC);
        return MARS_ERR_INVALID_MAGIC;
    }
    if (h.version_major != MARS_VERSION_MAJOR) return MARS_ERR_VERSION_MISMATCH;
    if (h.num_tensors > 65536 || h.num_layers > 65536 || h.num_inputs > 4 || h.num_outputs > 4) return MARS_ERR_INVALID_FILE;
    const size_t tables = sizeof(h) + (size_t)h.num_tensors * sizeof(mars_tensor_t) + (size_t)h.num_layers * sizeof(mars_layer_t);
    if (tables > size) return MARS_ERR_INVALID_FILE;
    const int deferred = (flags & MARS_HIP_LOAD_DEFER_WEIGHTS) != 0;
    if (!deferred && h.weights_size > 0 && (h.weights_offset > size || h.weights_size > size - h.weights_offset))
        return MARS_ERR_INVALID_FILE;
    if (h.weights_size > ((uint64_t)1 << 36)) return MARS_ERR_INVALID_FILE;

    mars_model_ext_t *m = (mars_model_ext_t *)calloc(1, sizeof(*m));
    if (!m) return MARS_ERR_ALLOC_FAILED;
    m->pub.header = h;
    plan_switches_read(&m->sw, 1);
    m->deferred = deferred;
    m->pub.tensors = (mars_runtime_tensor_t *)calloc(h.num_tensors ? h.num_tensors : 1, sizeof(mars_runtime_tensor_t));
    m->pub.layers = (mars_runtime_layer_t *)calloc(h.num_layers ? h.num_layers : 1, sizeof(mars_runtime_layer_t));
    m->mt = (mtensor_t *)calloc(h.num_tensors ? h.num_tensors : 1, sizeof(mtensor_t));
    m->layer_noop = (unsigned char *)calloc(h.num_layers ? h.num_layers : 1, 1);
    if (!m->pub.tensors || !m->pub.layers || !m->mt || !m->layer_noop) { mars_free(&m->pub); return MARS_ERR_ALLOC_FAILED; }
    const uint8_t *q = p + sizeof(h);
    for (uint32_t i = 0; i < h.num_tensors; i++, q += sizeof(mars_tensor_t)) memcpy(&m->pub.tensors[i].desc, q, sizeof(mars_tensor_t));
    for (uint32_t i = 0; i < h.num_layers; i++, q += sizeof(mars_layer_t)) memcpy(&m->pub.layers[i].desc, q, sizeof(mars_layer_t));

    m->pub.weights_size = (size_t)h.weights_size;
    if (h.weights_size) {
        m->pub.weights = calloc(1, (size_t)h.weights_size);
        if (!m->pub.weights) { mars_free(&m->pub); return MARS_ERR_ALLOC_FAILED; }
        if (!deferred) memcpy(m->pub.weights, p + h.weights_offset, (size_t)h.weights_size);
    }
    m->pub.ddr_base = m->pub.weights;
    for (uint32_t i = 0; i < h.num_tensors; i++) {
        mars_runtime_tensor_t *rt = &m->pub.tensors[i];
        if (rt->desc.ndims > MARS_MAX_DIMS) { mars_free(&m->pub); return MARS_ERR_INVALID_FILE; }
        m->mt[i].bytes = shape_numel(&rt->desc) * elem_size(rt->desc.dtype);
        if (rt->desc.data_size > 0) {
            if (rt->desc.data_offset > h.weights_size) { mars_free(&m->pub); return MARS_ERR_INVALID_FILE; }
            m->mt[i].is_weight = 1;
            rt->vaddr = (uint8_t *)m->pub.weights + rt->desc.data_offset;
            rt->alloc_size = (size_t)rt->desc.data_size;
        }
    }
    for (uint32_t i = 0; i < h.num_inputs; i++) {
        uint32_t id = h.input_tensor_ids[i];
        if (id < h.num_tensors && !m->mt[id].is_weight) m->mt[id].io_in = (int)i + 1;
    }
    for (uint32_t i = 0; i < h.num_outputs; i++) {
        uint32_t id = h.output_tensor_ids[i];
        if (id < h.num_tensors && !m->mt[id].is_weight) m->mt[id].io_out = (int)i + 1;
    }

    mars_error_t err = build_plan(m);
    if (err != MARS_OK) { mars_free(&m->pub); return err; }
    VLOG("%u layers -> %d launches, parameter arena %zu bytes\n", h.num_layers, m->n_ops, m->arena_size);
    *out_m = m;
    return MARS_OK;
}

mars_error_t mars_hip_load_memory_ex(const void *data, size_t size, unsigned flags, mars_model_t **out_model) {
    if (!out_model) return MARS_ERR_INVALID_FILE;
    mars_model_ext_t *m = NULL;
    mars_error_t err = load_host(data, size, flags, &m);
    if (err != MARS_OK) return err;
    if (!nna_is_ready() || !mhip_ready()) {
        fprintf(stderr, "Mars: no initialised MI355X device (call nna_init first); refusing to load\n");
        mars_free(&m->pub);
        return MARS_ERR_NNA_INIT_FAILED;
    }
    err = upload_params(m);
    if (err == MARS_OK) err = alloc_batch(m, 1);
    if (err != MARS_OK) { mars_free(&m->pub); return err; }
    m->live_next = g_live_models;
    g_live_models = m;
    *out_model = &m->pub;
    return MARS_OK;
}

static int describe_op_full(const mars_op_t *o, char *line, size_t cap, int k) {
#define ADD(...) k += snprintf(line + k, cap - (size_t)k, __VA_ARGS__)
    ADD(" | err %d in %dx%dx%d out %dx%dx%d k %dx%d s %dx%d p %d,%d", o->err, o->in_h, o->in_w, o->in_c, o->out_h, o->out_w, o->out_c, o->kh, o->kw, o->sh, o->sw, o->pt, o->pl);
    ADD(" nchw %d out_nchw %d relu %d is_mul %d is_f32 %d leaky %d safe %d silu %d f32_exact %d variant %d", o->nchw, o->out_nchw, o->relu, o->is_mul, o->is_f32, o->leaky,
        o->safe, o->silu_f32, o->f32_exact, o->variant);
    ADD(" row_pad %d oc_pad %d c_pad %d store_c %d ch_off %d out_ch_off %d out_pix_stride %d in_byte_off %zu out_byte_off %zu scale %dx%d bn_n %d n %zu", o->row_pad,
        o->oc_pad, o->c_pad, o->store_c, o->ch_off, o->out_ch_off, o->out_pix_stride, o->in_byte_off, o->out_byte_off, o->scale_h, o->scale_w, o->bn_n, o->n);
    ADD(" k_limit %d rows_only %d pair_next %d in_rec %d out_rec %d vc %d,%d,%d:", o->k_limit, o->rows_only, o->pair_next, o->in_rec, o->out_rec, o->vc_n, o->vc_run, o->vc_shift);
    for (int q = 0; q < o->vc_n && q < 3; q++) ADD(" %d", o->vc_t[q]);
    ADD(" add %d %a %a %a seg %d up %d:", o->add_t, (double)o->add_s_conv, (double)o->add_s_other, (double)o->add_inv, o->nseg, o->seg_up);
    for (int q = 0; q < o->nseg && q < 4; q++) ADD(" %d/%d", o->seg_t[q], o->seg_c[q]);
    ADD(" chain %d:", o->chain_n);
    for (int q = 0; q < o->chain_n && q < 3; q++) ADD(" %d", o->chain_out[q]);
    ADD(" cs %a f %a %a %a", (double)o->cs, (double)o->f0, (double)o->f1, (double)o->f2);
    ADD(" w_off %zd b_off %zd lut_off %zd lut2_off %zd s_off %zd w2_off %zd rows %d planes %d w3_off %zd stem %d blob %zd %zd", (ssize_t)o->w_off, (ssize_t)o->b_off,
        (ssize_t)o->lut_off, (ssize_t)o->lut2_off, (ssize_t)o->s_off, (ssize_t)o->w2_off, o->w2_rows, o->w2_planes, (ssize_t)o->w3_off, o->w3_stem, (ssize_t)o->w_blob_off[0],
        (ssize_t)o->w_blob_off[1]);
    ADD(" post_next %d", o->post_next);
    if (o->post_next) ADD(" %zd", (ssize_t)o->post_w_off);
    ADD(" pre %d", o->pre);
    if (o->pre) ADD(" %zd %zd %zd %a", (ssize_t)o->pre_w_off, (ssize_t)o->pre_b_off, (ssize_t)o->pre_lut2_off, (double)o->pre_cs);
    ADD(" macs %a bytes %a prof_kind %d", o->macs, o->bytes, o->prof_kind);
#undef ADD
    return k;
}

size_t mars_hip_describe_plan(const void *data, size_t size, unsigned flags, char *out, size_t cap) {
    static const char *const kinds[] = {"conv_i8", "conv_f32", "relu_bytes", "lut_i8", "binary_i8", "sigmoid_f32", "binary_f32", "relu_f32", "bn",
                                        "maxpool", "concat_slice", "upsample", "upsample_q", "maxpool_q", "concat_q", "conv_f32_vhead", "fail"};
    mars_model_ext_t *m = NULL;
    const int full = (flags & MARS_HIP_DESCRIBE_FULL) != 0;
    if (load_host(data, size, flags & ~MARS_HIP_DESCRIBE_FULL, &m) != MARS_OK) return 0;
    size_t n = 0;
    char line[4096];
#define EMIT() do { const size_t l = strlen(line); if (out && n < cap) memcpy(out + n, line, n + l <= cap ? l : cap - n); n += l; } while (0)
    for (int i = 0; i < m->n_ops; i++) {
        const mars_op_t *o = &m->ops[i];
        int k = snprintf(line, sizeof line, "op %d layer %d %s in", i, o->layer, o->kind >= 0 && o->kind <= OP_FAIL ? kinds[o->kind] : "?");
        for (int q = 0; q < o->n_in && q < 4; q++) k += snprintf(line + k, sizeof line - (size_t)k, " %d", o->t_in[q]);
        k += snprintf(line + k, sizeof line - (size_t)k, " out %d", o->t_out);
#define FLAG(cond, ...) if (cond) k += snprintf(line + k, sizeof line - (size_t)k, __VA_ARGS__)
        FLAG(o->kind == OP_CONV_I8 || o->kind == OP_CONV_F32 || o->kind == OP_CONV_F32_VHEAD, " k%dx%d s%d c%d->%d", o->kh, o->kw, o->sw, o->in_c, o->out_c);
        FLAG(o->nchw, " relayout"); FLAG(o->out_nchw, " planar_store"); FLAG(o->lut_off != NO_OFF, " lut"); FLAG(o->add_t, " add=%d", o->add_t - 1);
        FLAG(o->nseg, " seg=%d", o->nseg); FLAG(o->pair_next, " pair_next"); FLAG(o->post_next, " post_next"); FLAG(o->pre, " pre"); FLAG(o->silu_f32, " silu");
        FLAG(o->k_limit, " k_limit=%d", o->k_limit); FLAG(o->in_rec, " in_rec=%d", o->in_rec); FLAG(o->out_rec, " out_rec");
        FLAG(o->vc_shift, " view=-%d", o->vc_shift); FLAG(o->vc_n, " vcat=%dx%d", o->vc_n, o->vc_run);
        FLAG(o->rows_only, " rows_only=%d", o->rows_only); FLAG(o->out_byte_off, " out_off=%zu", o->out_byte_off); FLAG(o->chain_n, " chain=%d", o->chain_n);
        FLAG(o->out_pix_stride, " pix_stride=%d", o->out_pix_stride); FLAG(o->kind == OP_FAIL, " err=%d", o->err);
#undef FLAG
        if (full) k = describe_op_full(o, line, sizeof line, k);
        snprintf(line + k, sizeof line - (size_t)k, "\n");
        EMIT();
    }
    for (uint32_t t = 0; t < m->pub.header.num_tensors; t++) {
        const mtensor_t *mt = &m->mt[t];
        const int listed = mt->nhwc_c || mt->partial || mt->zero_from || mt->rec_c || mt->pix_stride;
        if (!listed && !(full && mt->needed)) continue;
        int k = listed ? snprintf(line, sizeof line, "tensor %u nhwc_c %d pitch %d partial %d zero_from %zu rec_c %d pix_stride %d", t, mt->nhwc_c, mt->nhwc_pitch,
                                  mt->partial, mt->zero_from, mt->rec_c, mt->pix_stride)
                       : snprintf(line, sizeof line, "+tensor %u", t);
        if (full)
            k += snprintf(line + k, sizeof line - (size_t)k, " | bytes %zu extent %zu needed %d tail_read %d weight %d io %d,%d pix_c %d rec_hw %d nhwc_hw %d", mt->bytes,
                          mt->extent, mt->needed, mt->tail_read, mt->is_weight, mt->io_in, mt->io_out, mt->pix_c, mt->rec_hw, mt->nhwc_hw);
        snprintf(line + k, sizeof line - (size_t)k, "\n");
        EMIT();
    }
    if (full) {
        const plan_switches_t *w = &m->sw;
        snprintf(line, sizeof line, "+plan n_ops %d arena_size %zu scratch_per_frame %zu blob_mirror_bytes %zu rec_max_frames %zu rec_skipped %d f32_mode %d | fusion %d"
                 " no_fuse_lut %d no_nhwc_internal %d no_vconcat_q %d no_pair_f32 %d no_rec %d no_zero_tail %d no_vconcat_f32 %d no_rowpad %d no_post %d rec_limit %zu"
                 " vconcat_limit %zu bottleneck_limit %zu\n", m->n_ops, m->arena_size, m->scratch_per_frame, m->blob_mirror_bytes, m->rec_max_frames, m->rec_skipped,
                 m->plan_f32_mode, w->fusion, w->no_fuse_lut, w->no_nhwc_internal, w->no_vconcat_q, w->no_pair_f32, w->no_rec, w->no_zero_tail, w->no_vconcat_f32,
                 w->no_rowpad, w->no_post, w->rec_limit, w->vconcat_limit, w->bottleneck_limit);
        EMIT();
    }
#undef EMIT
    if (out && cap) out[n < cap ? n : cap - 1] = 0;
    mars_free(&m->pub);
    return n;
}

int mars_yolo_find_heads(const void *data, size_t size, int *tensor_ids, int *strides, int *num_classes, int cap) {
    mars_model_ext_t *m = NULL;
    if (load_host(data, size, 0, &m) != MARS_OK) return -1;
    const int n = mars_find_heads(m, tensor_ids, strides, num_classes, cap);
    mars_free(&m->pub);
    return n;
}

int mars_yolo_find_dfl_heads(const void *data, size_t size, int *box_ids, int *cls_ids, int *strides, int *num_classes, int *reg_max, int cap) {
    mars_model_ext_t *m = NULL;
    if (load_host(data, size, 0, &m) != MARS_OK) return -1;
    const int n = mars_find_dfl_heads(m, box_ids, cls_ids, strides, num_classes, reg_max, cap);
    mars_free(&m->pub);
    return n;
}

mars_error_t mars_load_memory(const void *data, size_t size, mars_model_t **model) {
    return mars_hip_load_memory_ex(data, size, 0, model);
}

mars_error_t mars_load_file(const char *path, mars_model_t **model) {
    if (!path || !model) return MARS_ERR_INVALID_FILE;
    FILE *fp = fopen(path, "rb");
    if (!fp) {
        fprintf(stderr, "Mars: Cannot open %s\n", path);
        return MARS_ERR_INVALID_FILE;
    }
    fseek(fp, 0, SEEK_END);
    long size = ftell(fp);
    fseek(fp, 0, SEEK_SET);
    if (size <= 0) { fclose(fp); return MARS_ERR_INVALID_FILE; }
    void *buf = malloc((size_t)size);
    if (!buf) { fclose(fp); return MARS_ERR_ALLOC_FAILED; }
    if (fread(buf, 1, (size_t)size, fp) != (size_t)size) { free(buf); fclose(fp); return MARS_ERR_INVALID_FILE; }
    fclose(fp);
    mars_error_t err = mars_load_memory(buf, (size_t)size, model);
    free(buf);
    return err;
}

mars_runtime_tensor_t *mars_get_input(mars_model_t *model, int index) {
    if (!model || index < 0 || (uint32_t)index >= model->header.num_inputs) return NULL;
    uint32_t tid = model->header.input_tensor_ids[index];
    if (tid >= model->header.num_tensors) return NULL;
    return &model->tensors[tid];
}

mars_runtime_tensor_t *mars_get_output(mars_model_t *model, int index) {
    if (!model || index < 0 || (uint32_t)index >= model->header.num_outputs) return NULL;
    uint32_t tid = model->header.output_tensor_ids[index];
    if (tid >= model->header.num_tensors) return NULL;
    return &model->tensors[tid];
}

int mars_get_num_inputs(mars_model_t *model) { return model ? (int)model->header.num_inputs : 0; }
int mars_get_num_outputs(mars_model_t *model) { return model ? (int)model->header.num_outputs : 0; }

void mars_print_summary(mars_model_t *model) {
    if (!model) return;
    mars_model_ext_t *m = (mars_model_ext_t *)model;
    printf("\nMars model summary (MI355X)\n");
    printf("Layers: %u\n", model->header.num_layers);
    printf("Tensors: %u\n", model->header.num_tensors);
    printf("Inputs: %u\n", model->header.num_inputs);
    printf("Outputs: %u\n", model->header.num_outputs);
    printf("Weights: %zu bytes\n", model->weights_size);
    printf("Launches per run: %d, batch %d, activations %zu bytes, parameters %zu bytes\n\n", m->n_ops, m->batch,
           m->act_bytes, m->arena_size);
}
```

thingino-accel_amd/csrc/host/mars_plan.c:

```c
#include <math.h>
#include <stdio.h>
#include <stdlib.h>
#include <string.h>
#include <time.h>

#include "mars_internal.h"
#include "nna.h"

int32_t mars_trunc_x86(float x) {
    if (x >= -2147483648.0f && x < 2147483648.0f) return (int32_t)x;
    return INT32_MIN;
}
static int sat8(int32_t v) { return v > 127 ? 127 : (v < -128 ? -128 : v); }
static int q_half_up(float v) { return sat8(mars_trunc_x86(v + 0.5f)); }

size_t elem_size(uint32_t dtype) {
    switch (dtype) {
        case MARS_DTYPE_FLOAT32: case MARS_DTYPE_INT32: return 4;
        case MARS_DTYPE_INT16: return 2;
        default: return 1;
    }
}

size_t shape_numel(const mars_tensor_t *d) {
// ... 524 lines not shown
    for (int i = 0; i < m->n_ops; i++) {
        const mars_op_t *o = &m->ops[i];
        for (int k = 0; k < o->n_in; k++)
            if (o->t_in[k] >= 0) c[o->t_in[k]]++;
        if (o->t_out >= 0) c[nt + (size_t)o->t_out]++;
        for (int k = 0; k < o->chain_n; k++)
            if (o->chain_out[k] >= 0 && o->chain_out[k] != o->t_out) c[nt + (size_t)o->chain_out[k]]++;
    }
    *readers = c;
    *writers = c + nt;
    return 1;
}

static int writer_before(const mars_model_ext_t *m, int t, int before) {
    for (int k = before - 1; k >= 0; k--)
        if (m->ops[k].t_out == t) return k;
    return -1;
}

enum { USE_READ = 1, USE_WRITE = 2 };
static int touched_between(const mars_model_ext_t *m, int lo, int hi, int t, int how) {
    for (int k = lo < 0 ? 0 : lo; k < hi && k < m->n_ops; k++)
        if (((how & USE_READ) && op_reads(&m->ops[k], t)) || ((how & USE_WRITE) && op_writes(&m->ops[k], t))) return 1;
    return 0;
}
static int touched_by_other(const mars_model_ext_t *m, int t, int lo, int hi) {
    return touched_between(m, 0, lo, t, USE_READ | USE_WRITE) || touched_between(m, hi + 1, m->n_ops, t, USE_READ | USE_WRITE);
}

static void drop_dead_ops(mars_model_ext_t *m) {
    int w = 0;
    for (int i = 0; i < m->n_ops; i++)
        if (m->ops[i].kind != -1) m->ops[w++] = m->ops[i];
    m->n_ops = w;
}

size_t planned_stride(const mtensor_t *t) {
    size_t s = ALIGN_UP(t->extent > t->bytes ? t->extent : t->bytes, 256);
    return s ? s : 256;
}

static void lut2_from_lut(mars_model_ext_t *m, mars_op_t *c, const int8_t *tab) {
    if (!mhip_conv_i8_lut2_ok(c->cs)) return;
    int8_t tab2[512];
    for (int k = -256; k < 256; k++) {
        int r = k >= 0 ? (k + 1) >> 1 : -((1 - k) >> 1);
        const int lo = c->relu ? 0 : -128;
        r = r < lo ? lo : (r > 127 ? 127 : r);
        tab2[k + 256] = tab[r + 128];
    }
    c->lut2_off = arena_reserve(m, 512);
    if (c->lut2_off != NO_OFF) memcpy(m->arena_host + c->lut2_off, tab2, 512);
}

void conv_i8_geometry(const mars_op_t *op, int frames, mhip_conv_i8_t *p) {
    memset(p, 0, sizeof(*p));
    p->frames = frames;
    p->in_c = op->in_c; p->in_h = op->in_h; p->in_w = op->in_w;
    p->out_h = op->out_h; p->out_w = op->out_w; p->out_c = op->store_c ? op->store_c : op->out_c;
    p->kh = op->kh; p->kw = op->kw; p->stride_h = op->sh; p->stride_w = op->sw; p->pad_top = op->pt; p->pad_left = op->pl;
    p->row_pad = op->row_pad; p->oc_pad = op->oc_pad; p->safe = op->safe;
    p->out_pix_stride = op->out_pix_stride; p->out_ch_off = op->out_ch_off;
}
int conv_i8_pre_fits(const mars_op_t *op, int frames, size_t in_stride, size_t out_stride) {
    mhip_conv_i8_t p;
    conv_i8_geometry(op, frames, &p);
    p.in_stride = in_stride; p.out_stride = out_stride;
    p.pre_w = (const int8_t *)op; p.pre_bias = (const int32_t *)op; p.pre_lut2 = (const uint8_t *)op; p.lut2 = (const uint8_t *)op;
    p.lut = (const uint8_t *)op;
    return mhip_conv_i8_pre_ok(&p);
}

int conv_i8_post_fits(const mars_model_ext_t *m, const mars_op_t *a, const mars_op_t *b, int frames) {
    mhip_conv_i8_t p;
    if (a->t_in[0] < 0 || a->t_out < 0 || b->t_out < 0) return 0;
    conv_i8_geometry(a, frames, &p);
    p.in_stride = planned_stride(&m->mt[a->t_in[0]]); p.out_stride = planned_stride(&m->mt[a->t_out]);
    p.lut = p.lut2 = p.post_lut2 = (const uint8_t *)a;
    p.post_w = p.post_in = (const int8_t *)a; p.post_out = (int8_t *)m;
    if (a->add_t) p.add = (const int8_t *)a;
    p.post_out_stride = planned_stride(&m->mt[b->t_out]);
    p.post_out_pix_stride = b->out_pix_stride; p.post_out_ch_off = b->out_ch_off;
    return mhip_conv_i8_post_ok(&p);
}

static int match_silu(const mars_model_ext_t *m, int i, int f32, const int *readers, const int *writers, int q[3], int *fwd) {
    const mars_op_t *c = &m->ops[i], *s = c + 1, *mu = c + 2;
    if (c->kind != (f32 ? OP_CONV_F32 : OP_CONV_I8) || s->kind != (f32 ? OP_SIGMOID_F32 : OP_LUT_I8) || mu->kind != (f32 ? OP_BINARY_F32 : OP_BINARY_I8) || !mu->is_mul)
        return 0;
    if (!f32 && m->pub.layers[s->layer].desc.type != MARS_LAYER_SIGMOID) return 0;
    const int q1 = q[0] = c->t_out, q2 = q[1] = s->t_out, q3 = q[2] = mu->t_out;
    if (s->t_in[0] != q1 || q1 == q2 || q2 == q3 || q1 == q3) return 0;
    *fwd = mu->t_in[0] == q1 && mu->t_in[1] == q2;
    if (!*fwd && !(mu->t_in[0] == q2 && mu->t_in[1] == q1)) return 0;
    if (f32 ? q3 == c->t_in[0] || m->mt[q3].is_weight : op_reads(c, q3)) return 0;
    if (readers[q1] != 2 || readers[q2] != 1 || writers[q1] != 1 || writers[q2] != 1 || writers[q3] != 1) return 0;
    if (m->mt[q1].io_out || m->mt[q2].io_out || m->mt[q1].io_in || m->mt[q2].io_in) return 0;
    const size_t n1 = (size_t)c->out_h * c->out_w * c->out_c;
    return s->n == n1 && mu->n == n1;
}

void fold_silu(mars_model_ext_t *m, int f32) {
    int *readers, *writers;
    if (!use_counts(m, &readers, &writers)) return;
    for (int i = 0; i + 2 < m->n_ops; i++) {
        mars_op_t *c = &m->ops[i];
        int q[3], fwd;
        if (!match_silu(m, i, f32, readers, writers, q, &fwd)) continue;
        const size_t n1 = (size_t)c->out_h * c->out_w * c->out_c;
        if (f32) {
            c->silu_f32 = 1;
        } else {
            const mars_tensor_t *d1 = &m->pub.tensors[q[0]].desc, *d2 = &m->pub.tensors[q[1]].desc, *d3 = &m->pub.tensors[q[2]].desc;
            int8_t tab[256];
            for (int v = -128; v < 128; v++) {
                int sg = sigmoid_q(v, d1->scale, d2->scale);
                tab[v + 128] = (int8_t)(fwd ? binary_q(1, v, sg, d1->scale, d2->scale, d3->scale)
                                            : binary_q(1, sg, v, d2->scale, d1->scale, d3->scale));
            }
            c->lut_off = lut_i8(m, tab);
            lut2_from_lut(m, c, tab);
        }
        c->t_out = q[2];
        touch(m, q[2], n1 * (f32 ? 4 : 1));
        m->mt[q[0]].needed = 0;
        m->mt[q[1]].needed = 0;
        memmove(&m->ops[i + 1], &m->ops[i + 3], (size_t)(m->n_ops - i - 3) * sizeof(mars_op_t));
        m->n_ops -= 2;
    }
    free(readers);
}

void fuse_lut(mars_model_ext_t *m) {
    if (m->sw.no_fuse_lut) return;
    int *readers, *writers;
    if (!use_counts(m, &readers, &writers)) return;
    for (int i = 0; i + 1 < m->n_ops; i++) {
        mars_op_t *c = &m->ops[i], *s = &m->ops[i + 1];
        if (c->kind != OP_CONV_I8 || s->kind != OP_LUT_I8 || c->lut_off != NO_OFF || s->lut_off == NO_OFF) continue;
        const int q1 = c->t_out, q2 = s->t_out;
        if (q1 < 0 || q2 < 0 || s->t_in[0] != q1 || q1 == q2) continue;
        if (op_reads(c, q2)) continue;
        if (readers[q1] != 1 || writers[q1] != 1 || writers[q2] != 1 || m->mt[q1].io_out || m->mt[q1].io_in || m->mt[q1].is_weight || m->mt[q2].is_weight) continue;
        const size_t n1 = (size_t)c->out_h * c->out_w * c->out_c;
        if (s->n != n1 || m->mt[q2].bytes < n1) continue;
        if (m->pub.tensors[q1].desc.dtype != MARS_DTYPE_INT8 || m->pub.tensors[q2].desc.dtype != MARS_DTYPE_INT8) continue;
        c->lut_off = s->lut_off;
        lut2_from_lut(m, c, (const int8_t *)(m->arena_host + s->lut_off));
        c->t_out = q2;
        touch(m, q2, n1);
        m->mt[q1].needed = 0;
        memmove(&m->ops[i + 1], &m->ops[i + 2], (size_t)(m->n_ops - i - 2) * sizeof(mars_op_t));
        m->n_ops -= 1;
    }
    free(readers);
}

void elide_concat(mars_model_ext_t *m) {
    int *readers, *writers;
    if (!use_counts(m, &readers, &writers)) return;
    for (int i = 0; i < m->n_ops; i++) {
        mars_op_t *cs = &m->ops[i];
        if (cs->kind != OP_CONCAT_SLICE) continue;
        const int ti = cs->t_in[0], to = cs->t_out;
        const mtensor_t *mt = &m->mt[ti];
        if (mt->is_weight || mt->io_in || mt->io_out || readers[ti] != 1 || writers[ti] != 1) continue;
// ... 308 lines not shown
            if (!f32) { c->add_s_conv = s_conv; c->add_s_other = s_other; c->add_inv = inv; }
            c->t_in[c->n_in++] = X;
            c->bytes += (f32 ? 4.0 : 1.0) * (double)ad->n;
            m->mt[A].needed = 0;
            ad->kind = -1;
            readers[A] = 0;
            break;
        }
    }
    drop_dead_ops(m);
    free(readers);
}

void fuse_bottleneck(mars_model_ext_t *m) {
    int *readers, *writers;
    if (!use_counts(m, &readers, &writers)) return;
    for (int i = 0; i + 1 < m->n_ops; i++) {
        mars_op_t *a = &m->ops[i], *b = &m->ops[i + 1];
        if (a->kind != OP_CONV_I8 || b->kind != OP_CONV_I8 || a->pre || b->pre) continue;
        const int T = a->t_out;
        if (T < 0 || b->t_in[0] != T || readers[T] != 1 || m->mt[T].io_in || m->mt[T].io_out || m->mt[T].is_weight) continue;
        if (a->kh != 1 || a->kw != 1 || a->sh != 1 || a->sw != 1 || a->nchw || b->nchw || a->out_nchw || b->out_nchw || !a->safe || !b->safe || a->nseg || b->nseg ||
            a->add_t || a->n_in != 1 || a->out_pix_stride || a->relu || a->lut2_off == NO_OFF || b->lut2_off == NO_OFF ||
            a->in_c != a->out_c || a->out_c != b->in_c || (a->in_c != 32 && a->in_c != 64) || b->sh != 1 || b->sw != 1 ||
            a->in_h != b->in_h || a->in_w != b->in_w || a->b_off == NO_OFF || a->pair_next || b->pair_next ||
            (i > 0 && m->ops[i - 1].pair_next))
            continue;
        const int X = a->t_in[0];
        if (X < 0 || X == b->t_out || m->mt[X].is_weight) continue;
        if (!conv_i8_pre_fits(b, 1, 0, 0)) continue;
        b->pre = 1;
        b->pre_w_off = a->w_off; b->pre_b_off = a->b_off; b->pre_lut2_off = a->lut2_off; b->pre_cs = a->cs;
        b->t_in[0] = X;
        b->macs += a->macs;
        m->mt[T].needed = 0;
        readers[T] = 0;
        a->kind = -1;
    }
    drop_dead_ops(m);
    free(readers);
}

void fuse_post(mars_model_ext_t *m) {
    if (m->sw.no_post || m->no_post) return;
    int *readers, *writers;
    if (!use_counts(m, &readers, &writers)) return;
    for (int i = 0; i + 1 < m->n_ops; i++) {
        mars_op_t *a = &m->ops[i], *b = &m->ops[i + 1];
        if (a->kind != OP_CONV_I8 || b->kind != OP_CONV_I8 || a->pre || b->pre || a->post_next || b->post_next || a->pair_next || b->pair_next ||
            (i > 0 && (m->ops[i - 1].pair_next || m->ops[i - 1].post_next)))
            continue;
        const int c = a->out_c, T = a->t_out, O = b->t_out;
        if ((c != 32 && c != 64) || a->oc_pad != c || a->kh * a->kw < 2 || a->sh != 1 || a->sw != 1 || !a->safe || a->nchw || a->out_nchw || a->nseg ||
            a->out_pix_stride || a->out_ch_off || a->store_c || a->chain_n || a->in_byte_off || a->out_byte_off || a->lut_off == NO_OFF ||
            a->lut2_off == NO_OFF || a->n_in >= 4)
            continue;
        if (b->kh != 1 || b->kw != 1 || b->sh != 1 || b->sw != 1 || b->pt || b->pl || !b->safe || b->nchw || b->out_nchw || b->add_t || b->chain_n ||
            b->store_c || b->in_byte_off || b->lut_off == NO_OFF || b->lut2_off == NO_OFF || b->nseg != 2 || b->seg_up || b->seg_t[0] != T ||
            b->seg_c[0] != c || b->seg_c[1] != c || b->in_c != 2 * c || b->out_c != 2 * c || b->oc_pad != 2 * c || b->row_pad != 2 * c ||
            b->in_h != a->out_h || b->in_w != a->out_w || b->out_h != a->out_h || b->out_w != a->out_w)
            continue;
        const int Y = b->seg_t[1];
        if (T < 0 || O < 0 || Y < 0 || Y == T || O == T || O == Y || readers[T] != 1 || writers[T] != 1 || m->mt[T].io_in || m->mt[T].io_out ||
            m->mt[T].is_weight || m->mt[T].tail_read || m->mt[Y].is_weight || m->mt[Y].pix_stride ||
            m->mt[Y].bytes != (size_t)a->out_h * a->out_w * c || op_reads(a, O) || op_reads(a, Y))
            continue;
        if (!conv_i8_post_fits(m, a, b, 1)) continue;
        const size_t bytes = mhip_conv_i8_post_pack(c, NULL, NULL, NULL);
        const size_t off = arena_reserve(m, bytes);
        if (off == NO_OFF) break;
        mhip_conv_i8_post_pack(c, (const int8_t *)(m->arena_host + b->w_off), b->b_off != NO_OFF ? (const int32_t *)(m->arena_host + b->b_off) : NULL,
                               (int8_t *)(m->arena_host + off));
        a->post_next = 1;
        a->post_w_off = off;
        a->t_in[a->n_in++] = Y;
        m->mt[T].needed = 0;
        readers[T] = 0;
        readers[Y]++;
        i++;
    }
    free(readers);
}

void pad_output_rows(mars_model_ext_t *m) {
    for (uint32_t i = 0; i < m->pub.header.num_tensors; i++) m->mt[i].pix_c = m->mt[i].pix_stride = 0;
    if (m->sw.no_rowpad) return;
    for (int i = 0; i < m->n_ops; i++) {
        mars_op_t *o = &m->ops[i];
        if (o->kind != OP_CONV_I8 || o->out_nchw || o->out_pix_stride || o->out_ch_off || o->add_t || o->t_out < 0 ||
            (o->out_c & 15) == 0 || (o->in_c & 15) != 0)
            continue;
        mtensor_t *t = &m->mt[o->t_out];
        const int P = (o->out_c + 15) & ~15;
        const size_t px = (size_t)o->out_h * o->out_w;
        if (!t->io_out || t->io_in || P > o->oc_pad || t->bytes != px * (size_t)o->out_c || (px * P) % 256 != 0) continue;
        if (touched_by_other(m, o->t_out, i, i)) continue;
        o->out_pix_stride = P;
        o->store_c = P;
        t->pix_c = o->out_c;
        t->pix_stride = P;
        if (px * P > t->extent) t->extent = px * P;
    }
}

void virtual_concat(mars_model_ext_t *m) {
    const int nt = (int)m->pub.header.num_tensors;
    for (int T = 0; T < nt; T++) {
        const mtensor_t *mt = &m->mt[T];
        if (mt->is_weight || mt->io_in || mt->io_out) continue;
        int sl[4], ns = 0, bad = 0, first_reader = -1, last_reader = -1, last_slice = -1;
        for (int i = 0; i < m->n_ops && !bad; i++) {
            const mars_op_t *o = &m->ops[i];
            if (o->t_out == T) {
                if (o->kind != OP_CONCAT_SLICE || ns >= 4) bad = 1;
                else { sl[ns++] = i; last_slice = i; }
            }
            for (int k = 0; k < o->n_in; k++)
                if (o->t_in[k] == T) {
                    if (o->kind != OP_CONV_I8 || k != 0 || o->n_in != 1 || o->nchw || o->kh != 1 || o->kw != 1 || o->sh != 1 ||
                        o->sw != 1 || o->pt || o->pl || !o->safe || o->nseg || (o->out_c & 15) || o->in_h != o->out_h ||
                        o->in_w != o->out_w || (o->in_c & (o->in_c - 1)) != 0 || o->add_t)
                        bad = 1;
                    if (first_reader < 0) first_reader = i;
                    last_reader = i;
                }
        }
        if (bad || ns < 2 || first_reader < 0 || last_slice > first_reader) continue;
        for (int a = 0; a < ns; a++)
            for (int b = a + 1; b < ns; b++)
                if (m->ops[sl[b]].ch_off < m->ops[sl[a]].ch_off) { int t = sl[a]; sl[a] = sl[b]; sl[b] = t; }
        int c = 0;
        const mars_op_t *s0 = &m->ops[sl[0]];
        for (int a = 0; a < ns && !bad; a++) {
            const mars_op_t *o = &m->ops[sl[a]];
            if (o->ch_off != c || (o->in_c & 31) || o->out_h != s0->out_h || o->out_w != s0->out_w || o->out_c != s0->out_c ||
                o->t_in[0] == T || o->t_in[0] < 0)
                bad = 1;
            c += o->in_c;
            if (!bad && touched_between(m, sl[a] + 1, last_reader + 1, o->t_in[0], USE_WRITE)) bad = 1;
        }
        if (bad || c != s0->out_c) continue;
        for (int i = 0; i < m->n_ops && !bad; i++) {
            const mars_op_t *o = &m->ops[i];
            if (o->kind == OP_CONV_I8 && o->n_in == 1 && o->t_in[0] == T &&
                (o->in_c != c || (size_t)o->in_h * o->in_w != (size_t)s0->out_h * s0->out_w))
                bad = 1;
        }
        if (bad) continue;
        for (int i = 0; i < m->n_ops; i++) {
            mars_op_t *o = &m->ops[i];
            if (o->kind != OP_CONV_I8 || o->n_in != 1 || o->t_in[0] != T) continue;
            o->nseg = ns;
            o->n_in = ns;
            for (int a = 0; a < ns; a++) {
                o->seg_t[a] = o->t_in[a] = m->ops[sl[a]].t_in[0];
                o->seg_c[a] = m->ops[sl[a]].in_c;
            }
        }
        for (int a = 0; a < ns; a++) m->ops[sl[a]].kind = -1;
        m->mt[T].needed = 0;
        for (int a = 0; a < ns; a++) {
            const int S = m->ops[sl[a]].t_in[0];
            int up = -1, nread = 0, nwrite = 0, ok = 1;
            for (int i = 0; i < m->n_ops; i++) {
                const mars_op_t *o = &m->ops[i];
                if (o->kind == -1) continue;
// ... 305 lines not shown
        for (int q = 0; q < heads; q++) {
            const mars_op_t *x = &m->ops[r1 + q];
            wt_off[q] = arena_reserve(m, mhip_conv_f32_vcat_pack(x->out_c, x->in_c, (int)km + 1, NULL, NULL));
            if (wt_off[q] == NO_OFF) return;
            if (!m->deferred)
                mhip_conv_f32_vcat_pack(x->out_c, x->in_c, (int)km + 1, (const float *)(m->arena_host + x->w_off), (float *)(m->arena_host + wt_off[q]));
        }
        while (m->n_ops + heads > m->cap_ops) {
            const int cap = m->cap_ops * 2;
            mars_op_t *np = (mars_op_t *)realloc(m->ops, (size_t)cap * sizeof(mars_op_t));
            if (!np) { m->plan_err = MARS_ERR_ALLOC_FAILED; return; }
            m->ops = np; m->cap_ops = cap;
        }
        memmove(&m->ops[rl + 1 + heads], &m->ops[rl + 1], sizeof(mars_op_t) * (size_t)(m->n_ops - rl - 1));
        m->n_ops += heads;
        for (int q = 0; q < heads; q++) {
            mars_op_t *x = &m->ops[r1 + q], *h = &m->ops[rl + 1 + q];
            const double hw = (double)x->in_h * x->in_w;
            x->t_in[0] = TL;
            x->vc_shift = (int)sB;
            x->k_limit = (int)km;
            x->macs = hw * x->out_c * (double)km;
            x->bytes = (hw * (double)km + hw * x->out_c) * 4.0;
            *h = *x;
            h->kind = OP_CONV_F32_VHEAD;
            h->pair_next = 0; h->vc_shift = 0;
            h->k_limit = (int)km + 1;
            h->vc_n = N - 1; h->vc_run = Wb / 4;
            h->n_in = N;
            for (int k = 0; k < N - 1; k++) { h->vc_t[k] = firsts[k]; h->t_in[1 + k] = firsts[k]; }
            h->macs = (double)(sB / 4) * x->out_c * (double)(km + 1);
            h->bytes = ((double)(sB / 4) * (double)(km + 1) + (double)(sB / 4) * x->out_c) * 4.0;
            h->variant = 0;
            h->w3_off = wt_off[q]; h->w3_stem = 0;
            h->w2_off = NO_OFF; h->w2_planes = 0;
        }
        memmove(&m->ops[first_op], &m->ops[e + 1], sizeof(mars_op_t) * (size_t)(m->n_ops - e - 1));
        m->n_ops -= N;
        m->mt[T].needed = 0;
        m->mt[T].partial = 1;
        m->mt[T].zero_from = 0;
        i = first_op - 1;
    }
}

void f32_policy(mars_model_ext_t *m) {
    const int nt = (int)m->pub.header.num_tensors;
    unsigned char *hot = (unsigned char *)calloc((size_t)nt + 1, 1);
    if (!hot) {
        for (int i = 0; i < m->n_ops; i++) m->ops[i].f32_exact = 1;
        return;
    }
    for (int i = m->n_ops - 1; i >= 0; i--) {
        mars_op_t *o = &m->ops[i];
        int reach = 0;
        if (o->kind == OP_MAXPOOL && o->t_in[0] >= 0 && m->pub.tensors[o->t_in[0]].desc.dtype == MARS_DTYPE_FLOAT32) reach = 1;
        if (o->kind == OP_RELU_BYTES && o->t_out >= 0) {
            hot[o->t_out] = 1;
            continue;
        }
        if (o->t_out >= 0 && hot[o->t_out]) reach = 1;
        for (int k = 0; k < o->chain_n; k++)
            if (o->chain_out[k] >= 0 && hot[o->chain_out[k]]) reach = 1;
        if (!reach) continue;
        for (int k = 0; k < o->n_in; k++)
            if (o->t_in[k] >= 0) hot[o->t_in[k]] = 1;
        if (o->kind == OP_CONV_F32) o->f32_exact = 1;
    }
    free(hot);
}

void plan_check(mars_model_ext_t *m) {
    for (int i = 0; i < m->n_ops; i++) {
        const mars_op_t *o = &m->ops[i];
        const char *why = NULL;
        if (o->kind == -1) why = "a dead op is left";
        else if (o->n_in < 0 || o->n_in > 4 || o->nseg < 0 || o->nseg > 4 || o->chain_n < 0 || o->chain_n > 3 || o->vc_n < 0 || o->vc_n > 3) why = "an operand count is out of range";
        else if (o->add_t && !op_reads(o, o->add_t - 1)) why = "add_t is not among t_in";
        else if (o->chain_n && o->t_out != o->chain_out[o->chain_n - 1]) why = "t_out is not the chain's last stage";
        else if (o->pair_next && (i + 1 >= m->n_ops || m->ops[i + 1].kind != o->kind)) why = "pair_next without a mate of its kind";
        else if (o->post_next && (o->kind != OP_CONV_I8 || i + 1 >= m->n_ops || m->ops[i + 1].kind != OP_CONV_I8 || m->ops[i + 1].nseg != 2 ||
                                  m->ops[i + 1].seg_t[0] != o->t_out || !op_reads(o, m->ops[i + 1].seg_t[1])))
            why = "post_next without its 1x1 behind it, or y2 is not among t_in";
        for (int k = 0; !why && k < o->nseg; k++)
            if (!op_reads(o, o->seg_t[k])) why = "a seg_t is not among t_in";
        for (int k = 0; !why && k < o->vc_n; k++)
            if (!op_reads(o, o->vc_t[k])) why = "a vc_t is not among t_in";
        if (!why) continue;
        VLOG("plan_check: op %d (layer %d, kind %d): %s\n", i, o->layer, o->kind, why);
        m->plan_err = MARS_ERR_LAYER_FAILED;
        return;
    }
}
```

thingino-accel_amd/csrc/host/mars_run.c:

```c
#include <math.h>
#include <stdio.h>
#include <stdlib.h>
#include <string.h>
#include <time.h>

#include "mars_internal.h"
#include "nna.h"

static int g_graph_max_batch = 8;
static unsigned g_tune_gen = 1;
static int g_dual_min_batch = 64;
static int g_dual_ways = 2;
static uint8_t *tdev(const mars_model_ext_t *m, int ti) {
    if (ti < 0 || !m->mt[ti].dev) return NULL;
    return m->mt[ti].dev + (m->mt[ti].is_weight ? 0 : (size_t)m->frame0 * m->mt[ti].stride);
}
static size_t tstride(const mars_model_ext_t *m, int ti) { return ti >= 0 ? m->mt[ti].stride : 0; }

void conv_i8_params(const mars_model_ext_t *m, const mars_op_t *op, mhip_conv_i8_t *p) {
    uint8_t *A = m->arena_dev;
    conv_i8_geometry(op, m->run_frames, p);
    p->in = (const int8_t *)tdev(m, op->t_in[0]); p->in_stride = tstride(m, op->t_in[0]);
    p->out = (int8_t *)tdev(m, op->t_out); p->out_stride = tstride(m, op->t_out);
    if (p->in) p->in += op->in_byte_off;
    if (p->out) p->out += op->out_byte_off;
    p->w = (const int8_t *)(A + op->w_off);
    p->bias = op->b_off != NO_OFF ? (const int32_t *)(A + op->b_off) : NULL;
    p->lut = op->lut_off != NO_OFF ? A + op->lut_off : NULL;
    p->lut2 = op->lut_off != NO_OFF && op->lut2_off != NO_OFF ? A + op->lut2_off : NULL;
    p->w_rgb = op->w2_off != NO_OFF && !op->w2_rows ? (const int8_t *)(A + op->w2_off) : NULL;
    p->w_rows = op->w2_off != NO_OFF && op->w2_rows ? (const int8_t *)(A + op->w2_off) : NULL;
    if (op->pre) {
        p->pre_w = (const int8_t *)(A + op->pre_w_off);
        p->pre_bias = (const int32_t *)(A + op->pre_b_off);
        p->pre_lut2 = A + op->pre_lut2_off;
        p->pre_cs = op->pre_cs;
    }
    p->cs = op->cs; p->relu = op->relu; p->out_nchw = op->out_nchw;
    p->variant = op->variant;
    if (op->post_next && op->t_out >= 0) p->out_stride = planned_stride(&m->mt[op->t_out]);
    if (op->add_t && tstride(m, op->add_t - 1) == p->out_stride) {
        p->add = (const int8_t *)tdev(m, op->add_t - 1);
        p->add_s_conv = op->add_s_conv; p->add_s_other = op->add_s_other; p->add_inv = op->add_inv;
    }
    p->nseg = op->nseg;
    p->seg_up = op->seg_up;
    int c0 = 0;
    for (int k = 0; k < 4; k++) {
        p->seg_c0[k] = 0x7fffffff;
        if (k < op->nseg) {
            p->seg_in[k] = (const int8_t *)tdev(m, op->seg_t[k]);
            p->seg_stride[k] = tstride(m, op->seg_t[k]);
            p->seg_c[k] = op->seg_c[k];
            p->seg_c0[k] = c0;
            c0 += op->seg_c[k];
        }
    }
    if (op->nseg > 1) p->in = p->seg_in[0];
}

static void conv_i8_post_params(const mars_model_ext_t *m, const mars_op_t *op, const mars_op_t *cv3, mhip_conv_i8_t *p) {
    uint8_t *A = m->arena_dev;
    conv_i8_params(m, op, p);
    p->post_w = (const int8_t *)(A + op->post_w_off);
    p->post_lut2 = A + cv3->lut2_off;
    p->post_cs = cv3->cs;
    p->post_in = (const int8_t *)tdev(m, cv3->seg_t[1]); p->post_in_stride = tstride(m, cv3->seg_t[1]);
    p->post_out = (int8_t *)tdev(m, cv3->t_out); p->post_out_stride = tstride(m, cv3->t_out);
    if (p->post_out) p->post_out += cv3->out_byte_off;
    p->post_out_pix_stride = cv3->out_pix_stride; p->post_out_ch_off = cv3->out_ch_off;
}

static void conv_f32_params(mars_model_ext_t *m, mars_op_t *op, mhip_conv_f32_t *p) {
    const int B = m->run_frames;
    uint8_t *A = m->arena_dev;
    memset(p, 0, sizeof(*p));
    p->in = (const float *)tdev(m, op->t_in[0]); p->in_stride = tstride(m, op->t_in[0]);
    p->out = (float *)tdev(m, op->t_out); p->out_stride = tstride(m, op->t_out);
    p->w = (const float *)(A + op->w_off);
    p->w_split = op->w2_off != NO_OFF ? (const void *)(A + op->w2_off) : NULL;
    p->w_patch = op->w3_off != NO_OFF ? (const void *)(A + op->w3_off) : NULL;
    p->bias = op->b_off != NO_OFF ? (const float *)(A + op->b_off) : NULL;
    p->frames = B;
    p->in_h = op->in_h; p->in_w = op->in_w; p->in_c = op->in_c;
    p->out_h = op->out_h; p->out_w = op->out_w; p->out_c = op->out_c;
    p->kh = op->kh; p->kw = op->kw; p->stride_h = op->sh; p->stride_w = op->sw; p->pad_top = op->pt; p->pad_left = op->pl;
    p->silu = op->silu_f32;
    if (op->add_t) { p->add = (const float *)tdev(m, op->add_t - 1); p->add_stride = tstride(m, op->add_t - 1); }
    {
        const int mode = mhip_conv_f32_mode(-1);
        p->use_mfma = mode == 3 ? 3 : mode == 4 ? 2 : (mode == 2 || (mode == 1 && !op->f32_exact));
    }
    if (op->in_rec || op->out_rec) {
        p->in_rec = op->in_rec; p->out_rec = op->out_rec;
        p->use_mfma = 3;
    }
    {
        const int need = p->use_mfma == 2 ? 3 : p->use_mfma == 3 ? 2 : 0;
        if (need > op->w2_planes) p->w_split = NULL;
        if (p->use_mfma != 3) p->w_patch = NULL;
    }
    if (p->use_mfma >= 2) p->k_limit = op->k_limit;
    if (op->vc_shift && op->kind == OP_CONV_F32) {
        p->in = p->in ? (const float *)((const uint8_t *)p->in - op->vc_shift) : NULL;
        p->k_limit = op->k_limit;
        p->k_limit_required = 1;
        if (p->use_mfma < 2 || !p->w_split) p->in = NULL;
    }
}

static int launch_op(mars_model_ext_t *m, mars_op_t *op) {
    const int B = m->run_frames;
    uint8_t *A = m->arena_dev;
    switch (op->kind) {
        case OP_CONV_I8: {
            mhip_conv_i8_t p;
            conv_i8_params(m, op, &p);
            if (op->nchw && op->c_pad == 4 && op->in_c <= 4 && !op->add_t) {
                if (!getenv("MARS_HIP_NO_PLANAR_STEM")) {
                    mhip_conv_i8_t q = p;
                    q.in_c = op->c_pad;
                    q.in_planar = op->in_c;
                    const int rc = mhip_conv_i8(&q);
                    if (rc != -2) return rc;
                }
            }
            if (op->nchw) {
                const size_t ss = ALIGN_UP(m->scratch_per_frame, 256);
                int8_t *scratch = (int8_t *)m->scratch_dev + (size_t)m->frame0 * ss;
                if (!(m->scratch_t == op->t_in[0] && m->scratch_cpad == op->c_pad && m->scratch_f0 == m->frame0 && m->scratch_n == B)) {
                    int rc = mhip_nchw_to_nhwc_pad(p.in, p.in_stride, scratch, ss, B, op->in_c, op->in_h * op->in_w, op->c_pad);
                    if (rc) return rc;
                    m->scratch_t = op->t_in[0]; m->scratch_cpad = op->c_pad; m->scratch_f0 = m->frame0; m->scratch_n = B;
                }
                p.in = scratch; p.in_stride = ss; p.in_c = op->c_pad;
            }
            if (op->add_t && !p.add) return -1;
            return mhip_conv_i8(&p);
        }
        case OP_CONV_F32: {
            mhip_conv_f32_t p;
            conv_f32_params(m, op, &p);
            return mhip_conv_f32(&p);
        }
        case OP_CONV_F32_VHEAD: {
            mhip_conv_f32_t p;
            const float *first[3] = {NULL, NULL, NULL};
            size_t strides[3] = {0, 0, 0};
            conv_f32_params(m, op, &p);
            if (p.use_mfma < 2) return -1;
            p.k_limit = op->k_limit;
            for (int k = 0; k < op->vc_n && k < 3; k++) {
                first[k] = (const float *)tdev(m, op->vc_t[k]);
// ... 80 lines not shown
                                    op->out_h, op->out_w, op->scale_h, op->scale_w, op->out_pix_stride, op->out_ch_off);
        default: return -1;
    }
}

static mars_error_t enqueue_plan(mars_model_t *model);
static double now_us(void);
static int tune_raw(const char *key, int value, int *get);

static void tune_push(mars_model_ext_t *m) {
    if (m->tune_depth++ || !m->n_tune) return;
    for (int i = 0; i < m->n_tune; i++) {
        tune_raw(m->tune[i].key, 0, &m->tune[i].saved);
        tune_raw(m->tune[i].key, m->tune[i].value, NULL);
    }
}
static void tune_pop(mars_model_ext_t *m) {
    if (--m->tune_depth || !m->n_tune) return;
    for (int i = m->n_tune - 1; i >= 0; i--) tune_raw(m->tune[i].key, m->tune[i].saved, NULL);
}
static mars_error_t run_device_async(mars_model_t *model);
mars_error_t mars_hip_run_device_async(mars_model_t *model) {
    if (!model) return MARS_ERR_INVALID_FILE;
    tune_push((mars_model_ext_t *)model);
    mars_error_t e = run_device_async(model);
    tune_pop((mars_model_ext_t *)model);
    return e;
}

static mars_error_t run_device_async(mars_model_t *model) {
    mars_model_ext_t *m = (mars_model_ext_t *)model;
    if (!m->act_dev || !m->arena_dev) return MARS_ERR_NNA_INIT_FAILED;
    int graphable = g_graph_max_batch > 0 && m->batch <= g_graph_max_batch && !m->profiling && !m->pipe;
    for (int i = 0; i < m->n_ops && graphable; i++)
        if (m->ops[i].kind == OP_FAIL) graphable = 0;
    if (!graphable) return enqueue_plan(model);
    if (m->graph_exec && m->graph_gen != g_tune_gen) {
        drop_graph(m);
        m->ran_plain = 0;
    }
    if (!m->graph_exec) {
        if (!m->ran_plain) {
            mars_error_t e = enqueue_plan(model);
            if (e == MARS_OK) m->ran_plain = 1;
            return e;
        }
        if (m->tail_pending) {
            mhip_select_stream(0);
            if (mhip_stream_wait(0, m->ev_tail_done)) return MARS_ERR_LAYER_FAILED;
            m->tail_pending = 0;
        }
        if (mhip_graph_begin() == 0) {
            mars_error_t e = enqueue_plan(model);
            m->graph_exec = mhip_graph_end(e == MARS_OK);
            m->graph_gen = g_tune_gen;
            if (e != MARS_OK) { m->graph_exec = NULL; return e; }
        }
        VLOG("plan of %d launches at batch %d %s\n", m->n_ops, m->batch, m->graph_exec ? "captured into a HIP graph" : "could not be captured");
        if (!m->graph_exec) {
            g_graph_max_batch = 0;
            return enqueue_plan(model);
        }
    }
    if (m->tail_pending) {
        mhip_select_stream(0);
        if (mhip_stream_wait(0, m->ev_tail_done)) return MARS_ERR_LAYER_FAILED;
        m->tail_pending = 0;
    }
    if (mhip_graph_launch(m->graph_exec)) return MARS_ERR_LAYER_FAILED;
    for (uint32_t i = 0; i < model->header.num_layers; i++) model->layers[i].is_executed = true;
    return MARS_OK;
}

static mars_error_t enqueue_range(mars_model_ext_t *m, int sid, int wait_tail) {
    void *prof_last = NULL;
    mhip_select_stream(sid);
    m->scratch_t = -1;
    for (int i = 0; i < m->n_ops; i++) {
        mars_op_t *op = &m->ops[i];
        if (op->kind == OP_FAIL) {
            fprintf(stderr, "Mars: Layer %d execution failed\n", op->layer);
            return (mars_error_t)op->err;
        }
        mars_op_t *mate = (op->pair_next || op->post_next) && i + 1 < m->n_ops ? &m->ops[i + 1] : NULL;
        if (wait_tail && ((op->t_out >= 0 && (m->mt[op->t_out].io_out || m->mt[op->t_out].tail_read)) ||
                          (mate && mate->t_out >= 0 && (m->mt[mate->t_out].io_out || m->mt[mate->t_out].tail_read)))) {
            mhip_stream_wait(sid, m->ev_tail_done);
            wait_tail = 0;
        }
        if (m->profiling) {
            if (!op->ev1) op->ev1 = mhip_event_create();
            if (!prof_last) {
                if (!op->ev0) op->ev0 = mhip_event_create();
                mhip_event_record(op->ev0);
                prof_last = op->ev0;
            }
            op->ev_start = prof_last;
        }
        int rc;
        if (mate && op->post_next) {
            mhip_conv_i8_t pa;
            conv_i8_post_params(m, op, mate, &pa);
            rc = mhip_conv_i8(&pa);
            i++;
        } else if (mate && op->kind == OP_CONV_F32) {
            mhip_conv_f32_t pa, pb;
            conv_f32_params(m, op, &pa);
            conv_f32_params(m, mate, &pb);
            rc = mhip_conv_f32_pair(&pa, &pb);
            if (rc == -2) {
                rc = launch_op(m, op);
                if (!rc) rc = launch_op(m, mate);
            }
            i++;
        } else if (mate) {
            mhip_conv_i8_t pa, pb;
            conv_i8_params(m, op, &pa);
            conv_i8_params(m, mate, &pb);
            rc = mhip_conv_i8_pair(&pa, &pb);
            if (rc == -2) {
                rc = launch_op(m, op);
                if (!rc) rc = launch_op(m, mate);
            }
            i++;
        } else {
            rc = launch_op(m, op);
        }
        {
            const mars_op_t *w2[2] = {op, mate};
            for (int q = 0; q < 2; q++)
                if (w2[q] && op_writes(w2[q], m->scratch_t)) m->scratch_t = -1;
        }
        if (m->profiling) {
            const int nx = i + 1;
            const int end = m->profiling != 2 || nx >= m->n_ops || m->ops[nx].prof_kind != op->prof_kind;
            op->prof_rec = end;
            if (end) {
                mhip_event_record(op->ev1);
                prof_last = op->ev1;
            }
        }
        if (rc != 0) {
            fprintf(stderr, "Mars: Layer %d launch failed: %s\n", op->layer, mhip_last_error());
            return MARS_ERR_LAYER_FAILED;
        }
    }
    return MARS_OK;
}

static mars_error_t enqueue_plan(mars_model_t *model) {
    mars_model_ext_t *m = (mars_model_ext_t *)model;
    for (uint32_t i = 0; i < model->header.num_layers; i++) model->layers[i].is_executed = false;
    const int B = m->batch;
    int dual = g_dual_min_batch > 0 && B >= g_dual_min_batch && B >= 2 && !m->profiling &&
               !(g_graph_max_batch > 0 && B <= g_graph_max_batch);
    if (dual) {
        if (!m->ev_fork) m->ev_fork = mhip_event_create_sync();
        for (int k = 0; k < 3; k++) {
            if (!m->ev_join[k]) m->ev_join[k] = mhip_event_create_sync();
            if (!m->ev_join[k]) dual = 0;
        }
        if (!m->ev_fork) dual = 0;
    }
    mars_error_t e;
    if (!dual) {
        m->frame0 = 0; m->run_frames = B;
        e = enqueue_range(m, 0, m->tail_pending);
    } else {
        const int ways = g_dual_ways < B ? g_dual_ways : B;
        mhip_select_stream(0);
        int rc = mhip_event_record(m->ev_fork);
        for (int k = 1; k < ways && !rc; k++) rc = mhip_stream_wait(3 + k, m->ev_fork);
        if (rc) return MARS_ERR_LAYER_FAILED;
        e = MARS_OK;
        int f0 = 0;
        for (int k = 0; k < ways && e == MARS_OK; k++) {
            const int n = (B - f0 + (ways - k) - 1) / (ways - k);
            m->frame0 = f0; m->run_frames = n;
            e = enqueue_range(m, k ? 3 + k : 0, m->tail_pending);
            f0 += n;
        }
        for (int k = 1; k < ways; k++) {
            mhip_select_stream(3 + k);
            rc = mhip_event_record(m->ev_join[k - 1]);
            if (!rc) rc = mhip_stream_wait(0, m->ev_join[k - 1]);
            if (rc && e == MARS_OK) e = MARS_ERR_LAYER_FAILED;
        }
    }
    mhip_select_stream(0);
    m->frame0 = 0; m->run_frames = B;
    if (e != MARS_OK) return e;
    m->tail_pending = 0;
    for (uint32_t i = 0; i < model->header.num_layers; i++) model->layers[i].is_executed = true;
    return MARS_OK;
}

static double now_us(void) {
    struct timespec ts;
    clock_gettime(CLOCK_MONOTONIC, &ts);
    return ts.tv_sec * 1e6 + ts.tv_nsec * 1e-3;
}

mars_error_t mars_hip_run_device(mars_model_t *model) {
    double t0 = now_us();
    mars_error_t e = mars_hip_run_device_async(model);
    if (e != MARS_OK) { mhip_sync(); return e; }
    if (mhip_sync()) return MARS_ERR_LAYER_FAILED;
    mars_model_ext_t *m = (mars_model_ext_t *)model;
    if (m->profiling)
        for (int i = 0; i < m->n_ops; i++)
            m->ops[i].last_ms = (m->ops[i].prof_rec && m->ops[i].ev_start && m->ops[i].ev1) ? mhip_event_elapsed_ms(m->ops[i].ev_start, m->ops[i].ev1) : 0.f;
    model->total_inference_us += (uint64_t)(now_us() - t0);
    model->inference_count++;
// ... 174 lines not shown
        mhip_conv_f32_mode(value);
        return 0;
    }
    return get ? mhip_conv_i8_tune_get(key, get) : mhip_conv_i8_tune(key, value);
}

static mars_error_t replan_for_f32_mode(mars_model_ext_t *m) {
    if (m->deferred || !m->arena_dev) return MARS_OK;
    int has_f32 = 0;
    for (int i = 0; i < m->n_ops && !has_f32; i++) has_f32 = m->ops[i].kind == OP_CONV_F32;
    if (!has_f32) return MARS_OK;
    tune_push(m);
    const int mode = mhip_conv_f32_mode(-1);
    mars_error_t e = MARS_OK;
    if (mode != m->plan_f32_mode && (mode >= 3 || m->plan_f32_mode >= 3)) {
        mhip_sync();
        e = build_plan(m);
        if (e == MARS_OK) e = upload_params(m);
        if (e == MARS_OK) e = alloc_batch(m, m->batch > 0 ? m->batch : 1);
    }
    tune_pop(m);
    return e;
}

int mars_hip_set_tuning(const char *key, int value) {
    g_tune_gen++;
    int rc = tune_raw(key, value, NULL);
    if (rc == 0 && key && !strcmp(key, "f32_mfma"))
        for (mars_model_ext_t *m = mars_live_models(); m; m = m->live_next)
            if (replan_for_f32_mode(m) != MARS_OK) rc = -1;
    return rc;
}

int mars_hip_get_tuning(const char *key, int *value) { return value ? tune_raw(key, 0, value) : -1; }

int mars_hip_model_set_tuning(mars_model_t *model, const char *key, int value) {
    mars_model_ext_t *m = (mars_model_ext_t *)model;
    int cur;
    if (!m || !key || strlen(key) >= sizeof m->tune[0].key || tune_raw(key, 0, &cur)) return -1;
    if (tune_raw(key, value, NULL)) return -1;
    tune_raw(key, cur, NULL);
    int i = 0;
    while (i < m->n_tune && strcmp(m->tune[i].key, key)) i++;
    if (i == m->n_tune) {
        if (m->n_tune == MARS_MAX_MODEL_TUNE) return -1;
        strcpy(m->tune[m->n_tune++].key, key);
    }
    m->tune[i].value = value;
    drop_graph(m);
    if (!strcmp(key, "f32_mfma") && replan_for_f32_mode(m) != MARS_OK) return -1;
    return 0;
}

int mars_hip_model_get_tuning(mars_model_t *model, const char *key, int *value) {
    mars_model_ext_t *m = (mars_model_ext_t *)model;
    if (!m || !key || !value) return -1;
    for (int i = 0; i < m->n_tune; i++)
        if (!strcmp(m->tune[i].key, key)) { *value = m->tune[i].value; return 0; }
    return tune_raw(key, 0, value);
}

static mars_error_t autotune_model(mars_model_t *model, int reps);
mars_error_t mars_hip_autotune(mars_model_t *model, int reps) {
    if (!model) return MARS_ERR_INVALID_FILE;
    tune_push((mars_model_ext_t *)model);
    mars_error_t e = autotune_model(model, reps);
    tune_pop((mars_model_ext_t *)model);
    return e;
}
static mars_error_t autotune_model(mars_model_t *model, int reps) {
    mars_model_ext_t *m = (mars_model_ext_t *)model;
    if (!m->act_dev || !m->arena_dev) return MARS_ERR_NNA_INIT_FAILED;
    drop_graph(m);
    if (reps <= 0) reps = 3;
    void *e0 = mhip_event_create(), *e1 = mhip_event_create();
    if (!e0 || !e1) return MARS_ERR_ALLOC_FAILED;
    mars_error_t err = MARS_OK;
    if (mhip_sync()) err = MARS_ERR_LAYER_FAILED;
    for (int i = 0; i < m->n_ops && err == MARS_OK; i++) {
        mars_op_t *op = &m->ops[i];
        if (op->kind != OP_CONV_I8 || op->nchw) continue;
        if (op->pair_next || (i > 0 && m->ops[i - 1].pair_next)) continue;
        if (op->post_next || (i > 0 && m->ops[i - 1].post_next)) continue;
        mhip_conv_i8_t p;
        conv_i8_params(m, op, &p);
        int codes[32];
        const int n = mhip_conv_i8_variants(&p, codes, 32);
        if (getenv("MARS_VERBOSE") && atoi(getenv("MARS_VERBOSE")) > 1)
            fprintf(stderr, "Mars: autotune layer %d: %dx%dx%d -> %dx%dx%d k%dx%d s%d pixstride %d choff %d lut %d safe %d\n", op->layer,
                    p.in_h, p.in_w, p.in_c, p.out_h, p.out_w, p.out_c, p.kh, p.kw, p.stride_w, p.out_pix_stride, p.out_ch_off,
                    p.lut != NULL, p.safe);
        float best = 0.0f;
        int best_code = 0;
        for (int k = 0; k < n && err == MARS_OK; k++) {
            p.variant = codes[k];
            int rc = mhip_conv_i8(&p);
            if (!rc) rc = mhip_event_record(e0);
            for (int r = 0; r < reps && !rc; r++) rc = mhip_conv_i8(&p);
            if (!rc) rc = mhip_event_record(e1);
            if (rc || mhip_sync()) { err = MARS_ERR_LAYER_FAILED; break; }
            const float ms = mhip_event_elapsed_ms(e0, e1);
            if (getenv("MARS_VERBOSE") && atoi(getenv("MARS_VERBOSE")) > 1)
                fprintf(stderr, "Mars: autotune layer %d: candidate %d: %.1f us\n", op->layer, codes[k], ms * 1000.0f / reps);
            if (best_code == 0 || ms < best) { best = ms; best_code = codes[k]; }
        }
        if (err == MARS_OK && best_code) {
            if (getenv("MARS_VERBOSE"))
                fprintf(stderr, "Mars: autotune layer %d: variant %d (%.1f us) of %d candidates, default %d\n", op->layer,
                        best_code, best * 1000.0f / reps, n, n ? codes[0] : 0);
            op->variant = best_code;
        }
    }
    mhip_event_destroy(e0);
    mhip_event_destroy(e1);
    return err;
}

void *mars_hip_tensor_device(mars_model_t *model, int ti, size_t *frame_stride) {
    if (!model || ti < 0 || (uint32_t)ti >= model->header.num_tensors) return NULL;
    mars_model_ext_t *m = (mars_model_ext_t *)model;
    if (frame_stride) *frame_stride = m->mt[ti].stride;
    return m->mt[ti].dev;
}

size_t mars_hip_tensor_frame_bytes(const mars_model_t *model, int ti) {
    if (!model || ti < 0 || (uint32_t)ti >= model->header.num_tensors) return 0;
    return ((const mars_model_ext_t *)model)->mt[ti].bytes;
}

int mars_hip_tensor_row_pitch(mars_model_t *model, int ti, int *row_bytes) {
    if (!model || ti < 0 || (uint32_t)ti >= model->header.num_tensors) return 0;
    const mtensor_t *t = &((mars_model_ext_t *)model)->mt[ti];
    if (row_bytes) *row_bytes = t->pix_stride ? t->pix_c : 0;
    return t->pix_stride;
}

mars_error_t mars_hip_read_tensor(mars_model_t *model, int ti, int frame, void *dst, size_t bytes) {
    if (!model || !dst || ti < 0 || (uint32_t)ti >= model->header.num_tensors) return MARS_ERR_INVALID_TENSOR;
    mars_model_ext_t *m = (mars_model_ext_t *)model;
    mtensor_t *t = &m->mt[ti];
    if (!t->dev || frame < 0 || (!t->is_weight && frame >= m->batch)) return MARS_ERR_INVALID_TENSOR;
    if (!t->is_weight && bytes > t->stride) return MARS_ERR_INVALID_TENSOR;
    if (t->partial) return MARS_ERR_INVALID_TENSOR;
    if (t->is_weight) {
        const size_t off = (size_t)m->pub.tensors[ti].desc.data_offset;
        if (off > m->blob_mirror_bytes || bytes > m->blob_mirror_bytes - off) return MARS_ERR_INVALID_TENSOR;
        frame = 0;
    }
    if (mhip_sync()) return MARS_ERR_LAYER_FAILED;
    if (t->rec_c) {
        const size_t full = (size_t)t->rec_c * t->rec_hw * 4;
        uint8_t *raw = (uint8_t *)malloc(full);
        float *f = (float *)malloc(full);
        if (!raw || !f || bytes > full || mhip_d2h_async(raw, t->dev + (size_t)frame * t->stride, full) || mhip_sync()) {
            free(raw); free(f);
            return MARS_ERR_LAYER_FAILED;
        }
        for (int c = 0; c < t->rec_c; c++)
            for (int px = 0; px < t->rec_hw; px++) {
                const uint8_t *r = raw + ((size_t)(c >> 3) * t->rec_hw + px) * 32 + (size_t)(c & 7) * 2;
                uint16_t h, md;
                memcpy(&h, r, 2); memcpy(&md, r + 16, 2);
                const uint32_t hb = (uint32_t)h << 16, mb = (uint32_t)md << 16;
                float hf, mf;
                memcpy(&hf, &hb, 4); memcpy(&mf, &mb, 4);
                f[(size_t)c * t->rec_hw + px] = hf + mf;
// ... 120 lines not shown
```

thingino-accel_amd/csrc/mhip.h:

```cpp
#ifndef MHIP_H
#define MHIP_H

#include <stddef.h>
#include <stdint.h>

#ifdef __cplusplus
extern "C" {
#endif

int mhip_init(int device_hint);
void mhip_shutdown(void);
int mhip_ready(void);
int mhip_device_info(int *cu_count, int *lds_bytes, int *gfx_version, size_t *hbm_bytes);
void *mhip_stream(void);
int mhip_sync(void);
void mhip_select_aux(int on);
void mhip_select_stream(int which);
int mhip_stream_wait(int which, void *ev);
int mhip_event_sync(void *ev);
void *mhip_malloc(size_t bytes);
void mhip_free(void *p);
void *mhip_host_alloc(size_t bytes);
void mhip_host_free(void *p);
int mhip_memset_async(void *dst, int value, size_t bytes);
int mhip_h2d_async(void *dst, const void *src, size_t bytes);
int mhip_d2h_async(void *dst, const void *src, size_t bytes);
int mhip_d2d_async(void *dst, const void *src, size_t bytes);
int mhip_h2d_2d_async(void *dst, size_t dpitch, const void *src, size_t spitch, size_t row_bytes, size_t rows);
int mhip_d2h_2d_async(void *dst, size_t dpitch, const void *src, size_t spitch, size_t row_bytes, size_t rows);
void *mhip_event_create(void);
void *mhip_event_create_sync(void);
void mhip_event_destroy(void *ev);
int mhip_event_record(void *ev);
float mhip_event_elapsed_ms(void *start, void *stop);
const char *mhip_last_error(void);
int mhip_graph_begin(void);
void *mhip_graph_end(int ok);
int mhip_graph_launch(void *exec);
void mhip_graph_destroy(void *exec);

typedef struct {
    const int8_t *in;  size_t in_stride;
    int8_t *out;       size_t out_stride;
    const int8_t *w;
    const int32_t *bias;
    const uint8_t *lut;
    const uint8_t *lut2;
    const int8_t *pre_w;
    const int32_t *pre_bias;
    const uint8_t *pre_lut2;
    float pre_cs;
    const int8_t *w_rgb;
    const int8_t *w_rows;
    int frames;
    int in_h, in_w, in_c;
    int out_h, out_w, out_c;
    int kh, kw, stride_h, stride_w, pad_top, pad_left;
    int row_pad;
    int oc_pad;
    float cs;
    int relu;
    int out_nchw;
    int in_planar;
    int safe;
    int out_pix_stride;
    int out_ch_off;
    int variant;
    const int8_t *add;
    float add_s_conv, add_s_other, add_inv;
    int nseg;
    const int8_t *seg_in[4];
    size_t seg_stride[4];
    int seg_c[4], seg_c0[4];
    int seg_up;
    const int8_t *post_w;
    const uint8_t *post_lut2;
    float post_cs;
    const int8_t *post_in;  size_t post_in_stride;
    int8_t *post_out;       size_t post_out_stride;
    int post_out_pix_stride, post_out_ch_off;
} mhip_conv_i8_t;
int mhip_conv_i8_post_ok(const mhip_conv_i8_t *p);
size_t mhip_conv_i8_post_pack(int c, const int8_t *packed, const int32_t *bias, int8_t *out);
int mhip_conv_i8_post_k(int c, int k);
int mhip_conv_i8_post_row(int c, int oc);
int mhip_conv_i8_oc_row(int oc, int oc_pad);
int mhip_conv_i8_pre_ok(const mhip_conv_i8_t *p);
size_t mhip_conv_i8_rgb_pack(int in_c, int kh, int kw, int stride_h, int stride_w, int pad_left, int oc_pad, int k64,
                             const int8_t *packed, int8_t *out);
size_t mhip_conv_i8_rows_pack(int in_c, int kh, int kw, int stride_h, int stride_w, int oc_pad, int k64, int out_w,
                              const int8_t *packed, int8_t *out);
unsigned long mhip_conv_i8_rows_launches(void);
int mhip_conv_i8_is_safe(float cs);
int mhip_conv_i8_lut2_ok(float cs);
int mhip_conv_i8_tune(const char *key, int value);
int mhip_conv_i8_tune_get(const char *key, int *value);
int mhip_conv_i8_variants(const mhip_conv_i8_t *p, int *codes, int max);
int mhip_conv_i8_seg_ok(const mhip_conv_i8_t *p);
int mhip_conv_i8_pair(const mhip_conv_i8_t *a, const mhip_conv_i8_t *b);
int mhip_conv_i8_small_c(int in_c, int kw, int out_c);
void mhip_conv_i8_pack_geom(int in_c, int kw, int out_c, int *row_pad, int *oc_pad, int *c_eff);
int mhip_conv_i8(const mhip_conv_i8_t *p);

typedef struct {
    const float *in;  size_t in_stride;
    float *out;       size_t out_stride;
    const float *w;   const float *bias;
    const void *w_split;
    const void *w_patch;
    int frames;
    int in_h, in_w, in_c, out_h, out_w, out_c;
    int kh, kw, stride_h, stride_w, pad_top, pad_left;
    int silu;
    const float *add; size_t add_stride;
    int use_mfma;
    int k_limit;
    int k_limit_required;
    int in_rec, out_rec;
} mhip_conv_f32_t;
int mhip_conv_f32(const mhip_conv_f32_t *p);
size_t mhip_conv_f32_vcat_pack(int out_c, int in_c, int planes, const float *w, float *out);
int mhip_conv_f32_vcat_head(const mhip_conv_f32_t *p, const float *w_t, const float *const *first, const size_t *first_strides, int n_first, int run_floats);
int mhip_conv_f32_pair(const mhip_conv_f32_t *a, const mhip_conv_f32_t *b);
unsigned long mhip_conv_f32_pair_launches(void);
size_t mhip_conv_f32_split_pack(int out_c, int in_c, int kh, int kw, int stride_w, int planes, const float *w, void *out);
unsigned long mhip_conv_f32_split_launches(void);
int mhip_conv_f32_split_takes(int out_c, int in_c, int kh, int kw, int stride_h, int stride_w, int pad_left, int in_w, int out_w);
size_t mhip_conv_f32_patch_pack(int out_c, int in_c, int kh, int kw, int stride, int pad, int in_h, int in_w, int out_h, int out_w,
                                const float *w, void *out);
size_t mhip_conv_f32_patch_pack2(int out_c, int in_c, int kh, int kw, int stride, int pad, int in_h, int in_w, int out_h, int out_w,
                                 int rec, const float *w, void *out);
int mhip_conv_f32_patch_geom2(int out_c, int in_c, int kh, int kw, int stride, int pad, int in_h, int in_w, int out_h, int out_w,
                              int rec, int *outv, int cap);
unsigned long mhip_conv_f32_prec_launches(void);
unsigned long mhip_conv_f32_recin_launches(void);
int mhip_conv_f32_patch_rec_form(int out_c, int in_c, int kh, int kw, int stride, int pad, int in_h, int in_w, int out_h, int out_w);
int mhip_conv_f32_patch_geom(int out_c, int in_c, int kh, int kw, int stride, int pad, int in_h, int in_w, int out_h, int out_w,
                             int *outv, int cap);
unsigned long mhip_conv_f32_patch_launches(void);
size_t mhip_conv_f32_stem_pack(int out_c, int in_c, int kh, int kw, int stride, int pad, int in_h, int in_w, int out_h, int out_w,
                               const float *w, void *out);
unsigned long mhip_conv_f32_stem_launches(void);
int mhip_conv_f32_mode(int set);

int mhip_lut_i8(const int8_t *in, size_t in_stride, int8_t *out, size_t out_stride, int frames,
                size_t n, const uint8_t *lut_dev);
int mhip_relu_bytes(int8_t *buf, size_t stride, int frames, size_t n);
int mhip_binary_i8(int is_mul, const int8_t *a, size_t a_stride, const int8_t *b, size_t b_stride,
                   int8_t *out, size_t out_stride, int frames, size_t n, float sa, float sb, float inv_so,
                   int out_run, int out_pix_stride, int out_ch_off);
int mhip_sigmoid_f32(const float *in, size_t in_stride, float *out, size_t out_stride, int frames, size_t n);
int mhip_binary_f32(int op , const float *a, size_t a_stride, const float *b,
                    size_t b_stride, float *out, size_t out_stride, int frames, size_t n);
int mhip_relu_f32(const float *in, size_t in_stride, float *out, size_t out_stride, int frames,
                  size_t n, float alpha);
int mhip_batchnorm_i8(const int8_t *in, size_t in_stride, int8_t *out, size_t out_stride, int frames,
                      int n, int c, int hw, const float *s, const float *b, float in_scale, float out_scale);
int mhip_batchnorm_f32(const float *in, size_t in_stride, float *out, size_t out_stride, int frames,
                       int n, int c, int hw, const float *s, const float *b);

int mhip_maxpool_i8(const int8_t *in, size_t in_stride, int8_t *out, size_t out_stride, int frames,
                    int in_h, int in_w, int ch, int out_h, int out_w, int kh, int kw, int sh, int sw,
                    int out_pix_stride, int out_ch_off);
int mhip_pool_chain_i8(const int8_t *in, size_t in_stride, int8_t *const *outs, const size_t *out_strides, int n,
// ... 235 lines not shown
```

Measured before the change: 58480.

## Fuse a 3x3 conv with its two following 1x1 convs in the patch kernel

Adds a SPLIT mode to the patch conv kernel. When a 64-channel conv feeds exactly two 32-channel 1x1 convs, the kernel applies both 1x1s in registers with an extra MFMA over the requantized tile and writes the two outputs directly. The aim is to skip writing and re-reading the intermediate tensor and to remove two kernel launches per fused group. In exchange it uses more LDS for the packed 1x1 weights and the second LUT, which may lower occupancy. It also adds extra per-tile requant work and excludes fused layers from autotuning.

```diff
diff --git a/thingino-accel_amd/csrc/hip/conv_i8.hip b/thingino-accel_amd/csrc/hip/conv_i8.hip
--- a/thingino-accel_amd/csrc/hip/conv_i8.hip
+++ b/thingino-accel_amd/csrc/hip/conv_i8.hip
@@ -1145,6 +1145,11 @@
             if (n < max && conv_i8_patch_ok(p, th, nullptr)) codes[n++] = th == 16 ? 10 : (th == 8 ? 9 : 11);
         return n;
     }
+    if (p->split_w) {
+        for (int th : {16, 8, 4})
+            if (n < max && conv_i8_patch_ok(p, th, nullptr)) codes[n++] = th == 16 ? 10 : (th == 8 ? 9 : 11);
+        return n;
+    }
     if (p->nseg > 1) {
         const int bn = p->oc_pad % 128 == 0 ? 128 : (p->oc_pad % 64 == 0 ? 64 : 32);
         const variant_t dv = default_variant(p, nks);
@@ -1187,7 +1192,7 @@
 }
 
 extern "C" int mhip_conv_i8(const mhip_conv_i8_t *p) {
-    if (!p || !p->in || (!p->out && !(p->post_w && p->post_out)) || !p->w) return -1;
+    if (!p || !p->in || (!p->out && !(p->post_w && p->post_out) && !(p->split_w && p->split_out[0] && p->split_out[1])) || !p->w) return -1;
     if (p->out_pix_stride < 0 || p->out_ch_off < 0 || (p->out_nchw && (p->out_pix_stride || p->out_ch_off)) ||
         (p->out_pix_stride && p->out_pix_stride < p->out_ch_off + p->out_c))
         return -1;
@@ -1245,6 +1250,19 @@
         }
         return conv_i8_launch_patch(p, k64, th);
     }
+    if (p->split_w) {
+        if (!mhip_zero_page() || (p->in_c % 16) != 0 || !mhip_conv_i8_split_ok(p)) return -1;
+        int th = conv_i8_split_tile_rows(p);
+        const int code = p->variant ? p->variant : tune().variant;
+        if (code >= 9 && code <= 11) {
+            const int want = code == 10 ? 16 : (code == 9 ? 8 : 4);
+            if (conv_i8_patch_ok(p, want, nullptr)) th = want;
+        } else if (tune().small_batch && conv_i8_patch_ok(p, 4, nullptr) &&
+                   ((long)p->frames * p->out_h * p->out_w + 255) / 256 * ((p->oc_pad + 127) / 128) < tune().few_wgs) {
+            th = 4;
+        }
+        return conv_i8_launch_patch(p, k64, th);
+    }
     if ((p->in_c % 16) == 0) {
         if (!mhip_zero_page()) return -1;
         const int nks = k64 / BK;
diff --git a/thingino-accel_amd/csrc/hip/conv_i8_common.hpp b/thingino-accel_amd/csrc/hip/conv_i8_common.hpp
--- a/thingino-accel_amd/csrc/hip/conv_i8_common.hpp
+++ b/thingino-accel_amd/csrc/hip/conv_i8_common.hpp
@@ -161,6 +161,33 @@
 #pragma unroll
     for (int g = 0; g < NV / 4; g++) pk[g] = pack4(v[4 * g], v[4 * g + 1], v[4 * g + 2], v[4 * g + 3]);
 }
+__device__ __forceinline__ void requant_pack_two(const int (&a)[16], float cs0, float cs1, uint32_t (&pk)[4]) {
+    const float c0 = cs0 * 2.0f, c1 = cs1 * 2.0f;
+    const int klo = -256, khi = 255;
+    int q[16], v[16];
+#pragma unroll
+    for (int i = 0; i < 16; i++) {
+        const int k = (int)((float)a[i] * (i < 8 ? c0 : c1));
+        asm("v_med3_i32 %0, %1, %2, %3" : "=v"(q[i]) : "v"(k), "v"(klo), "v"(khi));
+    }
+#pragma unroll
+    for (int g = 0; g < 2; g++)
+        asm volatile("ds_read_i8 %0, %4 offset:768\n\tds_read_i8 %1, %5 offset:768\n\t"
+                     "ds_read_i8 %2, %6 offset:768\n\tds_read_i8 %3, %7 offset:768"
+                     : "=&v"(v[4 * g]), "=&v"(v[4 * g + 1]), "=&v"(v[4 * g + 2]), "=&v"(v[4 * g + 3])
+                     : "v"(q[4 * g]), "v"(q[4 * g + 1]), "v"(q[4 * g + 2]), "v"(q[4 * g + 3])
+                     : "memory");
+#pragma unroll
+    for (int g = 2; g < 4; g++)
+        asm volatile("ds_read_i8 %0, %4 offset:1280\n\tds_read_i8 %1, %5 offset:1280\n\t"
+                     "ds_read_i8 %2, %6 offset:1280\n\tds_read_i8 %3, %7 offset:1280"
+                     : "=&v"(v[4 * g]), "=&v"(v[4 * g + 1]), "=&v"(v[4 * g + 2]), "=&v"(v[4 * g + 3])
+                     : "v"(q[4 * g]), "v"(q[4 * g + 1]), "v"(q[4 * g + 2]), "v"(q[4 * g + 3])
+                     : "memory");
+    wait_lds_values<16>(v);
+#pragma unroll
+    for (int g = 0; g < 4; g++) pk[g] = pack4(v[4 * g], v[4 * g + 1], v[4 * g + 2], v[4 * g + 3]);
+}
 template <int NV, bool HAS_LUT, bool SAFE, bool LUT0, bool ADD = false, bool FAST = false>
 __device__ __forceinline__ void requant_pack(const int (&a)[NV], float cs, int lo, const uint8_t *lut128, uint32_t (&pk)[NV / 4],
                                              const uint32_t *xw = nullptr, const add_args_t *ga = nullptr) {
@@ -425,6 +452,7 @@
 int conv_i8_launch_patch(const mhip_conv_i8_t *p, int k64, int th);
 int conv_i8_pre_tile_rows(const mhip_conv_i8_t *p);
 int conv_i8_post_tile_rows(const mhip_conv_i8_t *p);
+int conv_i8_split_tile_rows(const mhip_conv_i8_t *p);
 bool conv_i8_rows_ok(const mhip_conv_i8_t *p);
 int conv_i8_launch_rows(const mhip_conv_i8_t *p);
 int conv_i8_try_rgb(const mhip_conv_i8_t *p, int k64);
diff --git a/thingino-accel_amd/csrc/hip/conv_i8_patch.hip b/thingino-accel_amd/csrc/hip/conv_i8_patch.hip
--- a/thingino-accel_amd/csrc/hip/conv_i8_patch.hip
+++ b/thingino-accel_amd/csrc/hip/conv_i8_patch.hip
@@ -41,7 +41,7 @@
     asm volatile("s_waitcnt lgkmcnt(0)\n\ts_barrier" ::: "memory");
 }
 
-template <int TH, int BN, bool HAS_LUT, bool PRE = false, bool POST = false>
+template <int TH, int BN, bool HAS_LUT, bool PRE = false, bool POST = false, bool SPLIT = false>
 __global__ __launch_bounds__(NTHREADS) void conv_i8_patch(const mhip_conv_i8_t p, const int k64, const int tiles_x,
                                                           const int tiles_y, const unsigned ntiles_all, const int PH,
                                                           const int PW, const int PWP, const int PWH, const int nblk,
@@ -57,14 +57,17 @@
     lds_base_must_be_zero(dynlds);
     const int nks = k64 / BK;
     constexpr int NPO = 2 * BN;
-    constexpr int LB = LUTB + ((PRE || POST) ? 512 : 0);
+    static_assert(!SPLIT || (BN == 64 && HAS_LUT && !PRE && !POST), "SPLIT: one 64-channel tile, no other stage");
+    constexpr int LB = LUTB + ((PRE || POST) ? 512 : 0) + (SPLIT ? 1024 : 0);
     int *dutab = (int *)(dynlds + LB);
     int8_t *wl = dynlds + LB + ((nks * 16 + 255) & ~255);
     const int patch_bytes = nblk * 1024;
     int8_t *w1l = wl + nks * BN * BK;
     int8_t *pwl = w1l;
     const int *pbl = (const int *)(pwl + NPO * NPO);
-    int8_t *patch0 = w1l + (PRE ? p.in_c * BK : 0) + (POST ? NPO * NPO + NPO * 4 : 0);
+    int8_t *swl = w1l;
+    const int *sbl = (const int *)(swl + 64 * BK);
+    int8_t *patch0 = w1l + (PRE ? p.in_c * BK : 0) + (POST ? NPO * NPO + NPO * 4 : 0) + (SPLIT ? 64 * BK + 64 * 4 : 0);
     int8_t *tpatch = patch0 + ring * patch_bytes;
 
     const int tid = threadIdx.x, lane = tid & 63;
@@ -91,6 +94,13 @@
     if (POST) {
         if (tid >= 128) ((uint32_t *)slut)[tid] = ((const uint32_t *)p.post_lut2)[tid - 128];
         if (tid < NPO) ((int *)(pwl + NPO * NPO))[tid] = ((const int *)(p.post_w + NPO * NPO))[tid];
+    }
+    if (SPLIT) {
+        if (tid >= 128) {
+            ((uint32_t *)slut)[tid] = ((const uint32_t *)p.split_lut2[0])[tid - 128];
+            ((uint32_t *)slut)[tid + 128] = ((const uint32_t *)p.split_lut2[1])[tid - 128];
+        }
+        if (tid < 64) ((int *)(swl + 64 * BK))[tid] = ((const int *)(p.split_w + 64 * BK))[tid];
     }
     const int rowbytes = p.kw * C, kbytes = p.kh * rowbytes;
     for (int i = tid; i < nks * 4; i += NTHREADS) {
@@ -114,6 +124,8 @@
             for (int g = wv; g < C / 16; g += 4) glds16(p.pre_w + (size_t)(g * 16 + (lane >> 2)) * BK + schunk * 16, w1l + g * 16 * BK);
         if (POST)
             for (int i = wv; i < NPO * NPO / 1024; i += 4) glds16(p.post_w + i * 1024 + lane * 16, pwl + i * 1024);
+        if (SPLIT)
+            glds16(p.split_w + wv * 1024 + lane * 16, swl + wv * 1024);
     }
     int uoff[PT_NIMAX], upos[PT_NIMAX];
 #pragma unroll
@@ -169,15 +181,17 @@
             }
     };
 
-    const __amdgpu_buffer_rsrc_t orsrc = __builtin_amdgcn_make_buffer_rsrc(POST ? p.post_out : p.out, 0, (int)out_bytes, 0x00020000);
-    const bool has_add = p.add != nullptr;
+    const __amdgpu_buffer_rsrc_t orsrc = __builtin_amdgcn_make_buffer_rsrc(SPLIT ? p.split_out[0] : (POST ? p.post_out : p.out), 0, (int)out_bytes, 0x00020000);
+    const unsigned out_bytes1 = SPLIT ? (unsigned)(p.frames - 1) * (unsigned)p.split_out_stride[1] + (unsigned)(p.out_h * p.out_w) * 32u : 0u;
+    const __amdgpu_buffer_rsrc_t orsrc1 = __builtin_amdgcn_make_buffer_rsrc(SPLIT ? p.split_out[1] : p.out, 0, (int)out_bytes1, 0x00020000);
+    const bool has_add = !SPLIT && p.add != nullptr;
     constexpr int RROW = WOC == 4 ? 1024 : 512;
     constexpr int NRI = WOC == 4 ? WPX : 2 * WPX;
     int8_t *rstage = patch0 + (ring + (PRE ? 1 : 0)) * patch_bytes + wv * (WPX * RROW);
     const int frow = lane & 15, fchunk = lane >> 4;
     const int chan = (lane >> 4) * (4 * WOC);
     const int NR = has_add || POST ? NRI : 0;
-    const int ntail = POST ? (has_add ? NRI : 0) + WPX * (NPO / 64) : NST;
+    const int ntail = POST ? (has_add ? NRI : 0) + WPX * (NPO / 64) : (SPLIT ? 2 * WPX : NST);
     const int ppstride = p.post_out_pix_stride ? p.post_out_pix_stride : NPO;
     auto issue_rows = [&](const int8_t *base, size_t fstride, int tx, int ty, unsigned f) {
 #pragma unroll
@@ -250,6 +264,12 @@
             }
             if (has_add) issue_rows(p.add, p.out_stride, tx, ty, f);
             else issue_rows(p.post_in, p.post_in_stride, tx, ty, f);
+        } else if (SPLIT) {
+#pragma unroll
+            for (int u = 0; u < WPX; u++) {
+                const int oy = ty * TH + wv * WPX + u, ox = tx * PT_TW + frow;
+                voffs[u] = oy < p.out_h && ox < p.out_w ? (oy * p.out_w + ox) * 32 + (lane >> 4) * 8 : -1;
+            }
         } else if (has_add) {
 #pragma unroll
             for (int u = 0; u < WPX; u++) {
@@ -397,7 +417,7 @@
                 }
             }
         }
-        uint32_t pku[POST ? WPX : 1][WOC];
+        uint32_t pku[POST || SPLIT ? WPX : 1][WOC];
         if (POST && has_add) {
 #pragma unroll
             for (int u = 0; u < WPX; u++) {
@@ -428,11 +448,45 @@
                 for (int q = 0; q < WOC; q++) pku[POST ? u : 0][q] = pk[q];
                 continue;
             }
+            if (SPLIT) {
+#pragma unroll
+                for (int q = 0; q < WOC; q++) pku[SPLIT ? u : 0][q] = pk[q];
+                continue;
+            }
             const int voff = voffs[u];
             if (WOC == 4)
                 __builtin_amdgcn_raw_buffer_store_b128((v4i){(int)pk[0], (int)pk[1], (int)pk[2], (int)pk[3]}, orsrc, voff, 0, 0);
             else if (WOC == 2)
                 __builtin_amdgcn_raw_buffer_store_b64((v2i){(int)pk[0], (int)pk[WOC > 1 ? 1 : 0]}, orsrc, voff, 0, 0);
+        }
+        if (SPLIT) {
+            v4i sw4[4], sb4[4];
+#pragma unroll
+            for (int r = 0; r < 4; r++) {
+                sw4[r] = *(const v4i *)(swl + lds_off(r * 16 + frow, fchunk));
+                sb4[r] = *(const v4i *)(sbl + r * 16 + fchunk * 4);
+            }
+            v4i sc[WPX][4];
+#pragma unroll
+            for (int u = 0; u < WPX; u++) {
+                const v4i b0 = {(int)pku[SPLIT ? u : 0][0], (int)pku[SPLIT ? u : 0][1], (int)pku[SPLIT ? u : 0][WOC > 2 ? 2 : 0], (int)pku[SPLIT ? u : 0][WOC > 3 ? 3 : 0]};
+#pragma unroll
+                for (int r = 0; r < 4; r++) sc[u][r] = __builtin_amdgcn_mfma_i32_16x16x64_i8(sw4[r], b0, sb4[r], 0, 0, 0);
+            }
+            const unsigned fo0 = f * (unsigned)p.split_out_stride[0], fo1 = f * (unsigned)p.split_out_stride[1];
+#pragma unroll
+            for (int u = 0; u < WPX; u++) {
+                int a2[16];
+#pragma unroll
+                for (int r = 0; r < 4; r++)
+#pragma unroll
+                    for (int e = 0; e < 4; e++) a2[r * 4 + e] = sc[u][r][e];
+                uint32_t pk4[4];
+                requant_pack_two(a2, p.split_cs[0], p.split_cs[1], pk4);
+                const int voff0 = voffs[u] >= 0 ? voffs[u] + (int)fo0 : -1, voff1 = voffs[u] >= 0 ? voffs[u] + (int)fo1 : -1;
+                __builtin_amdgcn_raw_buffer_store_b64((v2i){(int)pk4[0], (int)pk4[1]}, orsrc, voff0, 0, 0);
+                __builtin_amdgcn_raw_buffer_store_b64((v2i){(int)pk4[2], (int)pk4[3]}, orsrc1, voff1, 0, 0);
+            }
         }
         if (POST) {
             if (has_add) wait_vmcnt<0>();
@@ -524,9 +578,18 @@
             (long)(p->frames - 1) * (long)p->post_out_stride + (long)p->out_h * p->out_w * ppstride > 0x7fffffffL)
             return false;
     }
+    const bool split = p->split_w != nullptr;
+    if (split) {
+        if (pre || post || p->add || g->bn != 64 || p->out_c != 64 || p->oc_pad != 64 || p->out_pix_stride || p->out_ch_off || !p->lut2 || !p->split_lut2[0] ||
+            !p->split_lut2[1] || !p->split_out[0] || !p->split_out[1])
+            return false;
+        for (int i = 0; i < 2; i++)
+            if ((long)(p->frames - 1) * (long)p->split_out_stride[i] + (long)p->out_h * p->out_w * 32 > 0x7fffffffL) return false;
+    }
     const size_t pb = (size_t)g->nblk * 1024;
     const size_t radd = p->add || post ? (size_t)4 * (th / 4) * (g->bn == 64 ? 1024 : 512) : 0;
     const size_t fixed = LUTB + (pre ? 512 + (size_t)C * BK + pb : 0) + (post ? 512 + (size_t)4 * g->bn * g->bn + (size_t)8 * g->bn : 0) +
+                         (split ? 1024 + (size_t)64 * BK + 64 * 4 : 0) +
                          (((size_t)g->nks * 16 + 255) & ~(size_t)255) + (size_t)g->nks * g->bn * BK + radd;
     const size_t budget = patch_lds_budget(g->bn);
     if (fixed + pb > budget) return false;
@@ -543,9 +606,12 @@
     const long ppstride = p->post_out_pix_stride ? p->post_out_pix_stride : 2 * p->out_c;
     return (long)(p->frames - 1) * (long)p->post_out_stride + (long)p->out_h * p->out_w * ppstride;
 }
-template <int TH, int BN, bool HAS_LUT, bool PRE = false, bool POST = false>
+static inline long split_out_bytes(const mhip_conv_i8_t *p, int side) {
+    return (long)(p->frames - 1) * (long)p->split_out_stride[side] + (long)p->out_h * p->out_w * 32;
+}
+template <int TH, int BN, bool HAS_LUT, bool PRE = false, bool POST = false, bool SPLIT = false>
 static int launch_patch_t(const mhip_conv_i8_t *p, int k64, const patch_geom_t &g) {
-    auto kern = conv_i8_patch<TH, BN, HAS_LUT, PRE, POST>;
+    auto kern = conv_i8_patch<TH, BN, HAS_LUT, PRE, POST, SPLIT>;
     static int cus = 0;
     static size_t slots_lds[8];
     static int slots_n[8], nslots = 0;
@@ -588,7 +654,7 @@
     hipLaunchKernelGGL(kern, dim3(gx, noc), dim3(NTHREADS), g.lds, mhip_stream_native(), *p, k64,
                        g.tiles_x, g.tiles_y, ntiles, g.PH, g.PW, g.PWP, g.PWH, g.nblk, (const int8_t *)mhip_zero_page(),
                        make_fastdiv((unsigned)g.tiles_x), make_fastdiv((unsigned)g.tiles_y), make_fastdiv((unsigned)g.PWP),
-                       (unsigned)(POST ? post_out_bytes(p) : persist_out_bytes(p)), g.ring, xmap,
+                       (unsigned)(SPLIT ? split_out_bytes(p, 0) : (POST ? post_out_bytes(p) : persist_out_bytes(p))), g.ring, xmap,
                        in_extent_bytes(p) <= 0x7fffffffL ? (unsigned)in_extent_bytes(p) : 0u);
     return mhip_check(hipGetLastError(), "conv_i8_patch launch");
 }
@@ -607,6 +673,11 @@
     (p->post_w ? launch_patch_t<T, B, true, false, true>(p, k64, g)                       \
      : p->pre_w ? launch_patch_t<T, B, true, true>(p, k64, g)                             \
                 : (p->lut ? launch_patch_t<T, B, true>(p, k64, g) : launch_patch_t<T, B, false>(p, k64, g)))
+    if (p->split_w) {
+        if (th == 16) return launch_patch_t<16, 64, true, false, false, true>(p, k64, g);
+        if (th == 8) return launch_patch_t<8, 64, true, false, false, true>(p, k64, g);
+        return launch_patch_t<4, 64, true, false, false, true>(p, k64, g);
+    }
     if (th == 16) return g.bn == 64 ? PATCH(16, 64) : PATCH(16, 32);
     if (th == 8) return g.bn == 64 ? PATCH(8, 64) : PATCH(8, 32);
     return g.bn == 64 ? PATCH(4, 64) : PATCH(4, 32);
@@ -658,3 +729,33 @@
     }
     return bytes;
 }
+
+int conv_i8_split_tile_rows(const mhip_conv_i8_t *p) {
+    patch_geom_t g;
+    for (int th : {16, 8, 4})
+        if (patch_geom(p, th, &g)) return th;
+    return 0;
+}
+extern "C" int mhip_conv_i8_split_ok(const mhip_conv_i8_t *p) {
+    if (!p || !p->split_w || p->pre_w || p->post_w || p->add || p->nseg > 1 || p->out_nchw) return 0;
+    return conv_i8_split_tile_rows(p) != 0;
+}
+extern "C" int mhip_conv_i8_split_row(int side, int oc) {
+    const int g = oc >> 3, rem = oc & 7;
+    return side * 32 + (rem >> 2) * 16 + g * 4 + (rem & 3);
+}
+extern "C" size_t mhip_conv_i8_split_pack(const int8_t *packed0, const int32_t *bias0, const int8_t *packed1, const int32_t *bias1, int8_t *out) {
+    const size_t bytes = (size_t)64 * BK + (size_t)64 * 4;
+    if (!packed0 || !packed1 || !out) return bytes;
+    memset(out, 0, bytes);
+    for (int side = 0; side < 2; side++) {
+        const int8_t *packed = side ? packed1 : packed0;
+        const int32_t *bias = side ? bias1 : bias0;
+        for (int oc = 0; oc < 32; oc++) {
+            const int R = mhip_conv_i8_split_row(side, oc), src = mhip_conv_i8_oc_row(oc, 32);
+            for (int k = 0; k < 64; k++) out[(size_t)R * BK + ((((k >> 4) ^ ((R >> 1) & 2))) << 4) + (k & 15)] = packed[(size_t)src * 64 + k];
+            ((int32_t *)(out + (size_t)64 * BK))[R] = bias ? bias[src] : 0;
+        }
+    }
+    return bytes;
+}
diff --git a/thingino-accel_amd/csrc/host/mars_internal.h b/thingino-accel_amd/csrc/host/mars_internal.h
--- a/thingino-accel_amd/csrc/host/mars_internal.h
+++ b/thingino-accel_amd/csrc/host/mars_internal.h
@@ -79,6 +79,8 @@
     float pre_cs;
     int post_next;
     size_t post_w_off;
+    int split_next;
+    size_t split_w_off;
     size_t w2_off;
     int w2_rows;
     int w2_planes;
@@ -98,7 +100,7 @@
 typedef struct {
     int fusion;
     unsigned no_fuse_lut : 1, no_nhwc_internal : 1, no_vconcat_q : 1, no_pair_f32 : 1, no_rec : 1, no_zero_tail : 1, no_vconcat_f32 : 1,
-        no_rowpad : 1, no_post : 1;
+        no_rowpad : 1, no_post : 1, no_split : 1;
     size_t rec_limit;
     size_t vconcat_limit;
     size_t bottleneck_limit;
@@ -113,6 +115,7 @@
     int no_download;
     int no_bottleneck;
     int no_post;
+    int no_split;
     int rec_frames;
     int rec_skipped;
     size_t rec_max_frames;
@@ -217,6 +220,7 @@
 MARS_INTERNAL void conv_i8_geometry(const mars_op_t *op, int frames, mhip_conv_i8_t *p);
 MARS_INTERNAL int conv_i8_pre_fits(const mars_op_t *op, int frames, size_t in_stride, size_t out_stride);
 MARS_INTERNAL int conv_i8_post_fits(const mars_model_ext_t *m, const mars_op_t *a, const mars_op_t *b, int frames);
+MARS_INTERNAL int conv_i8_split_fits(const mars_model_ext_t *m, const mars_op_t *a, const mars_op_t *b, const mars_op_t *c, int frames);
 MARS_INTERNAL void plan_layer(mars_model_ext_t *m, int li);
 MARS_INTERNAL void fold_silu(mars_model_ext_t *m, int f32);
 MARS_INTERNAL void fuse_lut(mars_model_ext_t *m);
@@ -229,6 +233,7 @@
 MARS_INTERNAL void pair_convs(mars_model_ext_t *m);
 MARS_INTERNAL void fuse_bottleneck(mars_model_ext_t *m);
 MARS_INTERNAL void fuse_post(mars_model_ext_t *m);
+MARS_INTERNAL void fuse_split(mars_model_ext_t *m);
 MARS_INTERNAL void pad_output_rows(mars_model_ext_t *m);
 MARS_INTERNAL void virtual_concat_q(mars_model_ext_t *m);
 MARS_INTERNAL void f32_policy(mars_model_ext_t *m);
diff --git a/thingino-accel_amd/csrc/host/mars_model.c b/thingino-accel_amd/csrc/host/mars_model.c
--- a/thingino-accel_amd/csrc/host/mars_model.c
+++ b/thingino-accel_amd/csrc/host/mars_model.c
@@ -27,6 +27,7 @@
     sw->no_vconcat_f32 = getenv("MARS_HIP_NO_VCONCAT_F32") != NULL;
     sw->no_rowpad = getenv("MARS_HIP_NO_ROWPAD") != NULL;
     sw->no_post = getenv("MARS_HIP_NO_POST") != NULL;
+    sw->no_split = getenv("MARS_HIP_NO_SPLIT") != NULL;
     sw->rec_limit = (e = getenv("MARS_HIP_REC_LIMIT")) ? (size_t)strtoull(e, NULL, 0) : (size_t)0xfffffff0u;
     sw->vconcat_limit = (e = getenv("MARS_HIP_VCONCAT_LIMIT")) ? (size_t)strtoull(e, NULL, 0) : (size_t)0x7fffffffu;
     sw->bottleneck_limit = (e = getenv("MARS_HIP_BOTTLENECK_LIMIT")) ? (size_t)strtoull(e, NULL, 0) : 0;
@@ -161,6 +162,7 @@
         pair_convs(m);
         if (m->sw.fusion >= 2 && !m->no_bottleneck) fuse_bottleneck(m);
         fuse_post(m);
+        fuse_split(m);
         pad_output_rows(m);
         virtual_concat_q(m);
     } else {
@@ -202,8 +204,8 @@
     const size_t vlim = m->sw.vconcat_limit, blim = m->sw.bottleneck_limit;
     const int rec_replan = (size_t)n > m->rec_max_frames || (m->rec_skipped && n < m->rec_frames);
     m->rec_frames = n;
-    if (m->no_vconcat || m->no_bottleneck || m->no_post || rec_replan) {
-        m->no_vconcat = m->no_bottleneck = m->no_post = 0;
+    if (m->no_vconcat || m->no_bottleneck || m->no_post || m->no_split || rec_replan) {
+        m->no_vconcat = m->no_bottleneck = m->no_post = m->no_split = 0;
         mars_error_t e = build_plan(m);
         if (e == MARS_OK) e = upload_params(m);
         if (e != MARS_OK) return e;
@@ -239,6 +241,18 @@
             if (op->kind != OP_CONV_I8 || !op->post_next) continue;
             if (!conv_i8_post_fits(m, op, op + 1, n)) {
                 m->no_post = 1;
+                mars_error_t e = build_plan(m);
+                if (e == MARS_OK) e = upload_params(m);
+                if (e != MARS_OK) return e;
+                break;
+            }
+        }
+    if (!m->no_split)
+        for (int i = 0; i + 2 < m->n_ops; i++) {
+            const mars_op_t *op = &m->ops[i];
+            if (op->kind != OP_CONV_I8 || !op->split_next) continue;
+            if (!conv_i8_split_fits(m, op, op + 1, op + 2, n)) {
+                m->no_split = 1;
                 mars_error_t e = build_plan(m);
                 if (e == MARS_OK) e = upload_params(m);
                 if (e != MARS_OK) return e;
@@ -397,6 +411,8 @@
         (ssize_t)o->w_blob_off[1]);
     ADD(" post_next %d", o->post_next);
     if (o->post_next) ADD(" %zd", (ssize_t)o->post_w_off);
+    ADD(" split_next %d", o->split_next);
+    if (o->split_next) ADD(" %zd", (ssize_t)o->split_w_off);
     ADD(" pre %d", o->pre);
     if (o->pre) ADD(" %zd %zd %zd %a", (ssize_t)o->pre_w_off, (ssize_t)o->pre_b_off, (ssize_t)o->pre_lut2_off, (double)o->pre_cs);
     ADD(" macs %a bytes %a prof_kind %d", o->macs, o->bytes, o->prof_kind);
@@ -421,7 +437,7 @@
 #define FLAG(cond, ...) if (cond) k += snprintf(line + k, sizeof line - (size_t)k, __VA_ARGS__)
         FLAG(o->kind == OP_CONV_I8 || o->kind == OP_CONV_F32 || o->kind == OP_CONV_F32_VHEAD, " k%dx%d s%d c%d->%d", o->kh, o->kw, o->sw, o->in_c, o->out_c);
         FLAG(o->nchw, " relayout"); FLAG(o->out_nchw, " planar_store"); FLAG(o->lut_off != NO_OFF, " lut"); FLAG(o->add_t, " add=%d", o->add_t - 1);
-        FLAG(o->nseg, " seg=%d", o->nseg); FLAG(o->pair_next, " pair_next"); FLAG(o->post_next, " post_next"); FLAG(o->pre, " pre"); FLAG(o->silu_f32, " silu");
+        FLAG(o->nseg, " seg=%d", o->nseg); FLAG(o->pair_next, " pair_next"); FLAG(o->post_next, " post_next"); FLAG(o->split_next, " split_next"); FLAG(o->pre, " pre"); FLAG(o->silu_f32, " silu");
         FLAG(o->k_limit, " k_limit=%d", o->k_limit); FLAG(o->in_rec, " in_rec=%d", o->in_rec); FLAG(o->out_rec, " out_rec");
         FLAG(o->vc_shift, " view=-%d", o->vc_shift); FLAG(o->vc_n, " vcat=%dx%d", o->vc_n, o->vc_run);
         FLAG(o->rows_only, " rows_only=%d", o->rows_only); FLAG(o->out_byte_off, " out_off=%zu", o->out_byte_off); FLAG(o->chain_n, " chain=%d", o->chain_n);
@@ -447,10 +463,10 @@
     if (full) {
         const plan_switches_t *w = &m->sw;
         snprintf(line, sizeof line, "+plan n_ops %d arena_size %zu scratch_per_frame %zu blob_mirror_bytes %zu rec_max_frames %zu rec_skipped %d f32_mode %d | fusion %d"
-                 " no_fuse_lut %d no_nhwc_internal %d no_vconcat_q %d no_pair_f32 %d no_rec %d no_zero_tail %d no_vconcat_f32 %d no_rowpad %d no_post %d rec_limit %zu"
+                 " no_fuse_lut %d no_nhwc_internal %d no_vconcat_q %d no_pair_f32 %d no_rec %d no_zero_tail %d no_vconcat_f32 %d no_rowpad %d no_post %d no_split %d rec_limit %zu"
                  " vconcat_limit %zu bottleneck_limit %zu\n", m->n_ops, m->arena_size, m->scratch_per_frame, m->blob_mirror_bytes, m->rec_max_frames, m->rec_skipped,
                  m->plan_f32_mode, w->fusion, w->no_fuse_lut, w->no_nhwc_internal, w->no_vconcat_q, w->no_pair_f32, w->no_rec, w->no_zero_tail, w->no_vconcat_f32,
-                 w->no_rowpad, w->no_post, w->rec_limit, w->vconcat_limit, w->bottleneck_limit);
+                 w->no_rowpad, w->no_post, w->no_split, w->rec_limit, w->vconcat_limit, w->bottleneck_limit);
         EMIT();
     }
 #undef EMIT
diff --git a/thingino-accel_amd/csrc/host/mars_plan.c b/thingino-accel_amd/csrc/host/mars_plan.c
--- a/thingino-accel_amd/csrc/host/mars_plan.c
+++ b/thingino-accel_amd/csrc/host/mars_plan.c
@@ -630,6 +630,17 @@
     p.post_out_stride = planned_stride(&m->mt[b->t_out]);
     p.post_out_pix_stride = b->out_pix_stride; p.post_out_ch_off = b->out_ch_off;
     return mhip_conv_i8_post_ok(&p);
+}
+
+int conv_i8_split_fits(const mars_model_ext_t *m, const mars_op_t *a, const mars_op_t *b, const mars_op_t *c, int frames) {
+    mhip_conv_i8_t p;
+    if (a->t_in[0] < 0 || a->t_out < 0 || b->t_out < 0 || c->t_out < 0) return 0;
+    conv_i8_geometry(a, frames, &p);
+    p.in_stride = planned_stride(&m->mt[a->t_in[0]]); p.out_stride = planned_stride(&m->mt[a->t_out]);
+    p.lut = p.lut2 = p.split_lut2[0] = p.split_lut2[1] = (const uint8_t *)a;
+    p.split_w = (const int8_t *)a; p.split_out[0] = p.split_out[1] = (int8_t *)m;
+    p.split_out_stride[0] = planned_stride(&m->mt[b->t_out]); p.split_out_stride[1] = planned_stride(&m->mt[c->t_out]);
+    return mhip_conv_i8_split_ok(&p);
 }
 
 static int match_silu(const mars_model_ext_t *m, int i, int f32, const int *readers, const int *writers, int q[3], int *fwd) {
@@ -1104,6 +1115,46 @@
     free(readers);
 }
 
+static int split_mate_ok(const mars_op_t *b, const mars_op_t *a, int T) {
+    return b->kind == OP_CONV_I8 && b->kh == 1 && b->kw == 1 && b->sh == 1 && b->sw == 1 && !b->pt && !b->pl && b->safe && !b->nchw && !b->out_nchw && !b->add_t &&
+           !b->chain_n && !b->store_c && !b->in_byte_off && !b->out_byte_off && !b->out_pix_stride && !b->out_ch_off && b->lut_off != NO_OFF &&
+           b->lut2_off != NO_OFF && !b->nseg && !b->pre && !b->post_next && !b->split_next && b->n_in == 1 && b->t_in[0] == T && b->in_c == 64 &&
+           b->out_c == 32 && b->oc_pad == 32 && b->row_pad == 64 && b->in_h == a->out_h && b->in_w == a->out_w && b->out_h == a->out_h && b->out_w == a->out_w;
+}
+void fuse_split(mars_model_ext_t *m) {
+    if (m->sw.no_split || m->no_split) return;
+    int *readers, *writers;
+    if (!use_counts(m, &readers, &writers)) return;
+    for (int i = 0; i + 2 < m->n_ops; i++) {
+        mars_op_t *a = &m->ops[i], *b = &m->ops[i + 1], *c = &m->ops[i + 2];
+        if (a->kind != OP_CONV_I8 || a->pre || a->post_next || a->split_next || a->pair_next || !b->pair_next || c->pair_next ||
+            (i > 0 && (m->ops[i - 1].pair_next || m->ops[i - 1].post_next)))
+            continue;
+        const int T = a->t_out;
+        if (a->out_c != 64 || a->oc_pad != 64 || a->kh * a->kw < 2 || (a->sh != 1 && a->sh != 2) || a->sw != a->sh || !a->safe || a->nchw || a->out_nchw ||
+            a->nseg || a->out_pix_stride || a->out_ch_off || a->store_c || a->chain_n || a->in_byte_off || a->out_byte_off || a->add_t ||
+            a->lut_off == NO_OFF || a->lut2_off == NO_OFF || a->n_in != 1)
+            continue;
+        if (T < 0 || !split_mate_ok(b, a, T) || !split_mate_ok(c, a, T)) continue;
+        const int O0 = b->t_out, O1 = c->t_out;
+        if (O0 < 0 || O1 < 0 || O0 == O1 || O0 == T || O1 == T || readers[T] != 2 || writers[T] != 1 || m->mt[T].io_in || m->mt[T].io_out ||
+            m->mt[T].is_weight || m->mt[T].tail_read || m->mt[O0].pix_stride || m->mt[O1].pix_stride || op_reads(a, O0) || op_reads(a, O1))
+            continue;
+        if (!conv_i8_split_fits(m, a, b, c, 1)) continue;
+        const size_t bytes = mhip_conv_i8_split_pack(NULL, NULL, NULL, NULL, NULL);
+        const size_t off = arena_reserve(m, bytes);
+        if (off == NO_OFF) break;
+        mhip_conv_i8_split_pack((const int8_t *)(m->arena_host + b->w_off), b->b_off != NO_OFF ? (const int32_t *)(m->arena_host + b->b_off) : NULL,
+                                (const int8_t *)(m->arena_host + c->w_off), c->b_off != NO_OFF ? (const int32_t *)(m->arena_host + c->b_off) : NULL,
+                                (int8_t *)(m->arena_host + off));
+        a->split_next = 1;
+        a->split_w_off = off;
+        m->mt[T].needed = 0;
+        i += 2;
+    }
+    free(readers);
+}
+
 void pad_output_rows(mars_model_ext_t *m) {
     for (uint32_t i = 0; i < m->pub.header.num_tensors; i++) m->mt[i].pix_c = m->mt[i].pix_stride = 0;
     if (m->sw.no_rowpad) return;
@@ -1575,6 +1626,10 @@
         else if (o->post_next && (o->kind != OP_CONV_I8 || i + 1 >= m->n_ops || m->ops[i + 1].kind != OP_CONV_I8 || m->ops[i + 1].nseg != 2 ||
                                   m->ops[i + 1].seg_t[0] != o->t_out || !op_reads(o, m->ops[i + 1].seg_t[1])))
             why = "post_next without its 1x1 behind it, or y2 is not among t_in";
+        else if (o->split_next && (o->kind != OP_CONV_I8 || i + 2 >= m->n_ops || m->ops[i + 1].kind != OP_CONV_I8 || m->ops[i + 2].kind != OP_CONV_I8 ||
+                                   !m->ops[i + 1].pair_next || m->ops[i + 2].pair_next || m->ops[i + 1].n_in != 1 || m->ops[i + 2].n_in != 1 ||
+                                   m->ops[i + 1].t_in[0] != o->t_out || m->ops[i + 2].t_in[0] != o->t_out || o->post_next || o->pair_next || o->pre || o->add_t))
+            why = "split_next without its pair of 1x1s behind it";
         for (int k = 0; !why && k < o->nseg; k++)
             if (!op_reads(o, o->seg_t[k])) why = "a seg_t is not among t_in";
         for (int k = 0; !why && k < o->vc_n; k++)
diff --git a/thingino-accel_amd/csrc/host/mars_run.c b/thingino-accel_amd/csrc/host/mars_run.c
--- a/thingino-accel_amd/csrc/host/mars_run.c
+++ b/thingino-accel_amd/csrc/host/mars_run.c
@@ -38,7 +38,7 @@
     }
     p->cs = op->cs; p->relu = op->relu; p->out_nchw = op->out_nchw;
     p->variant = op->variant;
-    if (op->post_next && op->t_out >= 0) p->out_stride = planned_stride(&m->mt[op->t_out]);
+    if ((op->post_next || op->split_next) && op->t_out >= 0) p->out_stride = planned_stride(&m->mt[op->t_out]);
     if (op->add_t && tstride(m, op->add_t - 1) == p->out_stride) {
         p->add = (const int8_t *)tdev(m, op->add_t - 1);
         p->add_s_conv = op->add_s_conv; p->add_s_other = op->add_s_other; p->add_inv = op->add_inv;
@@ -69,6 +69,18 @@
     p->post_out = (int8_t *)tdev(m, cv3->t_out); p->post_out_stride = tstride(m, cv3->t_out);
     if (p->post_out) p->post_out += cv3->out_byte_off;
     p->post_out_pix_stride = cv3->out_pix_stride; p->post_out_ch_off = cv3->out_ch_off;
+}
+
+static void conv_i8_split_params(const mars_model_ext_t *m, const mars_op_t *op, const mars_op_t *cv1, const mars_op_t *cv2, mhip_conv_i8_t *p) {
+    uint8_t *A = m->arena_dev;
+    const mars_op_t *side[2] = {cv1, cv2};
+    conv_i8_params(m, op, p);
+    p->split_w = (const int8_t *)(A + op->split_w_off);
+    for (int k = 0; k < 2; k++) {
+        p->split_lut2[k] = A + side[k]->lut2_off;
+        p->split_cs[k] = side[k]->cs;
+        p->split_out[k] = (int8_t *)tdev(m, side[k]->t_out); p->split_out_stride[k] = tstride(m, side[k]->t_out);
+    }
 }
 
 static void conv_f32_params(mars_model_ext_t *m, mars_op_t *op, mhip_conv_f32_t *p) {
@@ -315,9 +327,11 @@
             fprintf(stderr, "Mars: Layer %d execution failed\n", op->layer);
             return (mars_error_t)op->err;
         }
-        mars_op_t *mate = (op->pair_next || op->post_next) && i + 1 < m->n_ops ? &m->ops[i + 1] : NULL;
+        mars_op_t *mate = (op->pair_next || op->post_next || op->split_next) && i + 1 < m->n_ops ? &m->ops[i + 1] : NULL;
+        mars_op_t *mate2 = op->split_next && i + 2 < m->n_ops ? &m->ops[i + 2] : NULL;
         if (wait_tail && ((op->t_out >= 0 && (m->mt[op->t_out].io_out || m->mt[op->t_out].tail_read)) ||
-                          (mate && mate->t_out >= 0 && (m->mt[mate->t_out].io_out || m->mt[mate->t_out].tail_read)))) {
+                          (mate && mate->t_out >= 0 && (m->mt[mate->t_out].io_out || m->mt[mate->t_out].tail_read)) ||
+                          (mate2 && mate2->t_out >= 0 && (m->mt[mate2->t_out].io_out || m->mt[mate2->t_out].tail_read)))) {
             mhip_stream_wait(sid, m->ev_tail_done);
             wait_tail = 0;
         }
@@ -331,7 +345,15 @@
             op->ev_start = prof_last;
         }
         int rc;
-        if (mate && op->post_next) {
+        if (op->split_next) {
+            mhip_conv_i8_t pa;
+            rc = -1;
+            if (mate && mate2) {
+                conv_i8_split_params(m, op, mate, mate2, &pa);
+                rc = mhip_conv_i8(&pa);
+            }
+            i += 2;
+        } else if (mate && op->post_next) {
             mhip_conv_i8_t pa;
             conv_i8_post_params(m, op, mate, &pa);
             rc = mhip_conv_i8(&pa);
@@ -360,8 +382,8 @@
             rc = launch_op(m, op);
         }
         {
-            const mars_op_t *w2[2] = {op, mate};
-            for (int q = 0; q < 2; q++)
+            const mars_op_t *w2[3] = {op, mate, mate2};
+            for (int q = 0; q < 3; q++)
                 if (w2[q] && op_writes(w2[q], m->scratch_t)) m->scratch_t = -1;
         }
         if (m->profiling) {
@@ -702,6 +724,7 @@
         if (op->kind != OP_CONV_I8 || op->nchw) continue;
         if (op->pair_next || (i > 0 && m->ops[i - 1].pair_next)) continue;
         if (op->post_next || (i > 0 && m->ops[i - 1].post_next)) continue;
+        if (op->split_next) continue;
         mhip_conv_i8_t p;
         conv_i8_params(m, op, &p);
         int codes[32];
diff --git a/thingino-accel_amd/csrc/mhip.h b/thingino-accel_amd/csrc/mhip.h
--- a/thingino-accel_amd/csrc/mhip.h
+++ b/thingino-accel_amd/csrc/mhip.h
@@ -79,7 +79,14 @@
     const int8_t *post_in;  size_t post_in_stride;
     int8_t *post_out;       size_t post_out_stride;
     int post_out_pix_stride, post_out_ch_off;
+    const int8_t *split_w;
+    const uint8_t *split_lut2[2];
+    float split_cs[2];
+    int8_t *split_out[2];   size_t split_out_stride[2];
 } mhip_conv_i8_t;
+int mhip_conv_i8_split_ok(const mhip_conv_i8_t *p);
+size_t mhip_conv_i8_split_pack(const int8_t *packed0, const int32_t *bias0, const int8_t *packed1, const int32_t *bias1, int8_t *out);
+int mhip_conv_i8_split_row(int side, int oc);
 int mhip_conv_i8_post_ok(const mhip_conv_i8_t *p);
 size_t mhip_conv_i8_post_pack(int c, const int8_t *packed, const int32_t *bias, int8_t *out);
 int mhip_conv_i8_post_k(int c, int k);
```

After: 60210, median of 6. 3.0% higher.
